# goruck/radar-ml

Measured on AMD Instinct MI355X. Metric: radar frames/s (3D-proj->SVM), higher is better.
Workload: dtype f32 volumes -> u8 codes, i8 MFMA (exact int32 dot), f64 epilogue; 1 GPU; configs[2]: max-projection + RBF-SVM decision_function, 3-class, 2562 SVs, batch 65536 frames/GPU of 64x64x128 f32 resident in HBM; parallelism=single GPU, global_frames=65536

## Files before the change

### include/radarml.h

```cpp
#ifndef RADARML_H
#define RADARML_H

#include <stdint.h>
#include <stddef.h>

#ifdef __cplusplus
extern "C" {
#endif

typedef enum rml_status {
    RML_OK = 0,
    RML_ERR_INVALID = -1,
    RML_ERR_UNSUPPORTED = -2,
    RML_ERR_HIP = -3,
    RML_ERR_NOMEM = -4,
    RML_ERR_STATE = -5
} rml_status;

typedef struct rml_ctx rml_ctx;
typedef struct rml_svm rml_svm;
typedef struct rml_linear rml_linear;

#define RML_MODE_MAX   0
#define RML_MODE_SLICE 1
#define RML_MODE_SUM   2
#define RML_MODE_MAX_NAN 3

#define RML_VOL_F32    0
#define RML_VOL_U8     1

#define RML_MASK_XZ 1u
#define RML_MASK_YZ 2u
#define RML_MASK_XY 4u
#define RML_MASK_ALL 7u

#define RML_KERNEL_RBF    0
#define RML_KERNEL_LINEAR 1

#define RML_PATH_AUTO  0
#define RML_PATH_F32   1
#define RML_PATH_I8    2
#define RML_PATH_F64   3
#define RML_PATH_DIGITS 4

const char* rml_version(void);
const char* rml_last_error(void);

int rml_ctx_create(int device, rml_ctx** out);
int rml_ctx_destroy(rml_ctx* ctx);
int rml_ctx_device(const rml_ctx* ctx);

#define RML_OPT_PROJECT_SHARE_CU 1
#define RML_OPT_WAVEFRAME 2
#define RML_OPT_LINPLANE 3
#define RML_OPT_STAGE_CODES 4
#define RML_OPT_SLICE_WAVE 5
#define RML_OPT_DERIVE_FUSED 6
#define RML_OPT_CODE_RMW 7
#define RML_OPT_GEMM_BIG 8
#define RML_OPT_CHUNK 9
#define RML_OPT_C1_PK 10
#define RML_OPT_SMO_LDS_ROWS 11
#define RML_SMO_LDS_ROWS_MAX 2768
#define RML_OPT_SGD_RESIDENT_D 12
#define RML_SGD_RESIDENT_D_MAX 10240
#define RML_OPT_CONV7 13
#define RML_CONV7_DEFAULT 3
#define RML_OPT_ZOOM_ROWS 14
#define RML_OPT_SPARSE_ROWS 15
int rml_ctx_set_option(rml_ctx* ctx, int option, int value);
int rml_ctx_get_option(const rml_ctx* ctx, int option, int* value);

int rml_ctx_reserve_workspace(rml_ctx* ctx, int64_t bytes);
int64_t rml_ctx_workspace_bytes(const rml_ctx* ctx);

int rml_profile_enable(rml_ctx* ctx, int on);
int rml_profile_read(rml_ctx* ctx, int64_t* launches, double* total_ms, int64_t* frames);
int rml_profile_read_gemm(rml_ctx* ctx, int64_t* launches, double* total_ms, double* ops);

int rml_probe_stream(rml_ctx* ctx, const void* buf, int64_t bytes, int reps, double* gb_per_s, void* stream);

int rml_code_rmw_default(int64_t D, int64_t frame_bytes, int derive, int u8);

int rml_svm_sv_occupancy(rml_ctx* ctx, const rml_svm* m, uint32_t* out, int64_t n_words);
int rml_project_occupancy(rml_ctx* ctx, const void* V, int vdtype, int64_t B, int X, int Y, int Z, int mode, float scale_div,
                          uint32_t mask, uint8_t* feat_q, int64_t ld_q, int32_t* row_isum, int64_t* row_isq, int32_t* row_flags,
                          uint32_t* occ, int occ_words, void* stream);
int64_t rml_ctx_sparse_gemm_launches(const rml_ctx* ctx);

int64_t rml_feature_len(int X, int Y, int Z, uint32_t mask);

int rml_project(rml_ctx* ctx, const void* V, int vdtype, int64_t B, int X, int Y, int Z, int mode,
                const int32_t* ijk, float scale_div, uint32_t mask,
                float* feat, int64_t ld_feat,
                uint8_t* feat_q, int64_t ld_q, int32_t* row_isum, int64_t* row_isq, int32_t* row_flags,
                void* stream);

int rml_project_slices(rml_ctx* ctx, const void* V, int vdtype, int64_t B, int X, int Y, int Z, int T,
                       const int32_t* ijk, float scale_div, uint32_t mask,
                       float* feat, int64_t ld_feat,
                       uint8_t* feat_q, int64_t ld_q, int32_t* row_isum, int64_t* row_isq, int32_t* row_flags,
                       void* stream);

int rml_project_planes(rml_ctx* ctx, const void* V, int vdtype, int64_t B, int X, int Y, int Z, int mode,
                       const int32_t* ijk, float* xz, float* yz, float* xy, void* stream);

int rml_derive_targets(rml_ctx* ctx, const void* V, int vdtype, int64_t B, int X, int Y, int Z,
                       int num_targets, int32_t* ijk, float* profiles, void* stream);

int rml_derive_slice(rml_ctx* ctx, const void* V, int vdtype, int64_t B, int X, int Y, int Z, int num_targets,
                     int32_t* ijk, float* profiles, float scale_div, uint32_t mask,
                     float* feat, int64_t ld_feat,
                     uint8_t* feat_q, int64_t ld_q, int32_t* row_isum, int64_t* row_isq, int32_t* row_flags,
                     void* stream);
int rml_derive_slice_supported(const rml_ctx* ctx, const void* V, int vdtype, int X, int Y, int Z, int num_targets);

int rml_assemble_features(rml_ctx* ctx, const float* xz, const float* yz, const float* xy,
                          int64_t B, int X, int Y, int Z, float scale_div, uint32_t mask,
                          float* feat, int64_t ld_feat, void* stream);

int rml_zoom_features(rml_ctx* ctx, const float* xz, const float* yz, const float* xy,
                      int64_t B, int X, int Y, int Z, const int32_t* out_shape,
                      float scale_div, uint32_t mask, float* feat, int64_t ld_feat, void* stream);

int rml_project_zoom(rml_ctx* ctx, const void* V, int vdtype, int64_t B, int X, int Y, int Z, int mode, const int32_t* ijk, int T,
                     const int32_t* out_shape, float scale_div, uint32_t mask, float* feat, int64_t ld_feat, void* stream);

int rml_quantize_rows(rml_ctx* ctx, const float* feat, int64_t N, int64_t D, int64_t ld_feat,
                      float scale_div, uint8_t* feat_q, int64_t ld_q,
                      int32_t* row_isum, int64_t* row_isq, int32_t* row_flags, void* stream);

int rml_svm_load(rml_ctx* ctx, const double* sv, int64_t M, int64_t D,
                 const double* dual_coef, const double* intercept, const int32_t* n_support,
                 int n_classes, int kernel, double gamma, double code_scale ,
                 const double* calib_a, const double* calib_b, rml_svm** out);
int rml_svm_free(rml_ctx* ctx, rml_svm* m);
int rml_svm_is_exact(const rml_svm* m);
int64_t rml_svm_num_sv(const rml_svm* m);
int64_t rml_svm_dim(const rml_svm* m);

int rml_svm_decision(rml_ctx* ctx, const rml_svm* m, int path,
                     const float* feat, int64_t ld_feat,
                     const uint8_t* feat_q, int64_t ld_q, const int32_t* row_isum, const int64_t* row_isq,
                     const int32_t* row_flags,
                     int64_t N,
                     double* dec_ovo, double* dec_ovr, double* proba,
                     int32_t* label_vote, int32_t* label_calib, void* stream);

int rml_svm_set_platt(rml_ctx* ctx, rml_svm* m, const double* probA, const double* probB);
int rml_svm_pairwise_proba(rml_ctx* ctx, const rml_svm* m, const double* dec_ovo, int64_t N, double* proba, void* stream);

#define RML_AUG_ROTATE 0
#define RML_AUG_ZOOM   1
#define RML_AUG_NOISE  2
int rml_augment(rml_ctx* ctx, int op, const float* src, int64_t B, int H, int W, const double* params, float* dst, void* stream);

#define RML_CHAIN_ROTATE 1
#define RML_CHAIN_ZOOM   2
#define RML_CHAIN_NOISE  4
int rml_augment_chain(rml_ctx* ctx, int stages, const float* src, int64_t in_stride, int64_t B, int H, int W, float sub, float div,
                      float lo, float hi, const double* params, float* dst, void* stream);

int rml_svm_kernel_matrix(rml_ctx* ctx, const rml_svm* m, int path, const float* feat, int64_t ld_feat, int64_t N,
                          double* kmat, int64_t ld_k, void* stream);

#define RML_GRAM_LINEAR 0
#define RML_GRAM_RBF    1
int rml_gram(rml_ctx* ctx, const float* feat, int64_t ld_feat, int64_t N, int64_t D,
             int nk, const int* kinds, const double* gammas,
             double* out, int64_t ld_out, int64_t stride_k, void* stream);

int rml_gram_segments(rml_ctx* ctx, const float* feat, int64_t ld_feat, int64_t N, int nseg, const int64_t* seg_len,
                      double* G, int64_t ld_g, int64_t stride_s, double* nsq, void* stream);
int rml_gram_compose(rml_ctx* ctx, const double* G, int64_t ld_g, int64_t stride_s, const double* nsq, int64_t N, int nseg,
                     int n_out, const int* seg_bits, const int* kinds, const double* gammas,
                     double* out, int64_t ld_out, int64_t stride_k, void* stream);

typedef struct rml_smo_problem {
    int32_t matrix;
    int32_t l;
    int32_t n_pos;
    int32_t shrinking;
    int32_t max_iter;
    int32_t reserved;
    int64_t rows_off;
    int64_t alpha_off;
    double Cp, Cn, eps;
} rml_smo_problem;
typedef struct rml_smo_fit {
    int32_t prob0;
    int32_t n_test;
    int64_t test_off;
} rml_smo_fit;
int rml_smo_solve(rml_ctx* ctx, const double* gram, int64_t N, int64_t ld, int64_t stride_k, int n_mats,
                  const rml_smo_problem* probs, int64_t n_probs, const int32_t* rows, int64_t n_rows_total,
                  double* alpha, int64_t n_alpha_total, double* rho, int32_t* n_iter, int32_t* stopped, void* stream);
int rml_smo_score(rml_ctx* ctx, const double* gram, int64_t N, int64_t ld, int64_t stride_k, int n_mats,
                  const rml_smo_problem* probs, int64_t n_probs, const int32_t* rows, int64_t n_rows_total,
                  const double* alpha, int64_t n_alpha_total, const double* rho, int n_classes,
                  const rml_smo_fit* fits, int64_t n_fits, const int32_t* test_rows, const int32_t* test_y,
                  int64_t n_test_total, double* dec, int32_t* labels, int32_t* correct, void* stream);

#define RML_SGD_L1 1
#define RML_SGD_L2 2
#define RML_SGD_ELASTICNET 3
#define RML_SGD_MAX_ROWS 8192
typedef struct rml_sgd_problem {
    int32_t n;
    int32_t penalty;
    int32_t average;
    int32_t max_iter;
    int32_t n_iter_no_change;
    int32_t shuffle;
    uint32_t seed;
    int32_t warm;
    int64_t rows_off;
    int64_t y_off;
    int64_t out;
    double alpha, l1_ratio, tol, weight_pos, weight_neg, t0;
} rml_sgd_problem;
typedef struct rml_sgd_fit {
    int32_t prob0;
    int32_t n_test;
    int64_t test_off;
} rml_sgd_fit;
int rml_sgd_solve(rml_ctx* ctx, const float* X, int64_t N, int64_t D, int64_t ld, const rml_sgd_problem* probs, int64_t n_probs,
                  const int32_t* rows, int64_t n_rows_total, const int32_t* y, int64_t n_y_total, int64_t n_out, double* coef,
                  double* avg_coef, double* intercept, double* avg_intercept, int32_t* n_iter, double* t, int32_t* status,
                  void* stream);
int rml_sgd_score(rml_ctx* ctx, const float* X, int64_t N, int64_t D, int64_t ld, const rml_sgd_problem* probs, int64_t n_probs,
                  int64_t n_out, const double* coef, const double* avg_coef, const double* intercept, const double* avg_intercept,
                  const double* t, int n_classes, const rml_sgd_fit* fits, int64_t n_fits, const int32_t* test_rows,
                  const int32_t* test_y, int64_t n_test_total, double* dec, int32_t* labels, int32_t* correct, void* stream);
int rml_sgd_shuffle(uint32_t seed, int64_t n, int32_t* perm_inout);

typedef struct rml_sgd_step {
    int64_t off;
    int32_t n;
    int32_t score;
    uint32_t seed[8];
} rml_sgd_step;
// ... 177 lines not shown
```

### radar-ml_amd/_lib.py

```python
import ctypes as C
import os
import threading

HERE = os.path.dirname(os.path.abspath(__file__))
LIB_PATH = os.environ.get("RML_LIB") or os.path.join(HERE, "libradarml_hip.so")


class RadarMLError(RuntimeError):
    pass


_lib = None
_lock = threading.RLock()
_ctx = {}

c_void_p, c_int, c_int64, c_uint32, c_uint64, c_float, c_double = (
    C.c_void_p, C.c_int, C.c_int64, C.c_uint32, C.c_uint64, C.c_float, C.c_double)

SIGNATURES = {
    "rml_version": (C.c_char_p, []),
    "rml_last_error": (C.c_char_p, []),
    "rml_ctx_create": (c_int, [c_int, C.POINTER(c_void_p)]),
    "rml_ctx_destroy": (c_int, [c_void_p]),
    "rml_ctx_device": (c_int, [c_void_p]),
# ... 6 lines not shown
    "rml_profile_read_gemm": (c_int, [c_void_p, C.POINTER(c_int64), C.POINTER(c_double), C.POINTER(c_double)]),
    "rml_feature_len": (c_int64, [c_int, c_int, c_int, c_uint32]),
    "rml_project": (c_int, [c_void_p, c_void_p, c_int, c_int64, c_int, c_int, c_int, c_int, c_void_p, c_float, c_uint32,
                            c_void_p, c_int64, c_void_p, c_int64, c_void_p, c_void_p, c_void_p, c_void_p]),
    "rml_project_slices": (c_int, [c_void_p, c_void_p, c_int, c_int64, c_int, c_int, c_int, c_int, c_void_p, c_float, c_uint32,
                                   c_void_p, c_int64, c_void_p, c_int64, c_void_p, c_void_p, c_void_p, c_void_p]),
    "rml_project_planes": (c_int, [c_void_p, c_void_p, c_int, c_int64, c_int, c_int, c_int, c_int, c_void_p,
                                   c_void_p, c_void_p, c_void_p, c_void_p]),
    "rml_derive_targets": (c_int, [c_void_p, c_void_p, c_int, c_int64, c_int, c_int, c_int, c_int, c_void_p, c_void_p, c_void_p]),
    "rml_derive_slice": (c_int, [c_void_p, c_void_p, c_int, c_int64, c_int, c_int, c_int, c_int, c_void_p, c_void_p, c_float, c_uint32,
                                 c_void_p, c_int64, c_void_p, c_int64, c_void_p, c_void_p, c_void_p, c_void_p]),
    "rml_derive_slice_supported": (c_int, [c_void_p, c_void_p, c_int, c_int, c_int, c_int, c_int]),
    "rml_assemble_features": (c_int, [c_void_p, c_void_p, c_void_p, c_void_p, c_int64, c_int, c_int, c_int, c_float,
                                      c_uint32, c_void_p, c_int64, c_void_p]),
    "rml_zoom_features": (c_int, [c_void_p, c_void_p, c_void_p, c_void_p, c_int64, c_int, c_int, c_int, c_void_p, c_float,
                                  c_uint32, c_void_p, c_int64, c_void_p]),
    "rml_project_zoom": (c_int, [c_void_p, c_void_p, c_int, c_int64, c_int, c_int, c_int, c_int, c_void_p, c_int, c_void_p, c_float,
                                 c_uint32, c_void_p, c_int64, c_void_p]),
    "rml_project_zoom_svm": (c_int, [c_void_p, c_void_p, c_void_p, c_int, c_int64, c_int, c_int, c_int, c_int, c_void_p, c_void_p, c_float,
                                     c_uint32, c_void_p, c_void_p, c_void_p, c_void_p, c_void_p, c_void_p]),
    "rml_quantize_rows": (c_int, [c_void_p, c_void_p, c_int64, c_int64, c_int64, c_float, c_void_p, c_int64,
                                  c_void_p, c_void_p, c_void_p, c_void_p]),
    "rml_svm_load": (c_int, [c_void_p, c_void_p, c_int64, c_int64, c_void_p, c_void_p, c_void_p, c_int, c_int,
                             c_double, c_double, c_void_p, c_void_p, C.POINTER(c_void_p)]),
    "rml_svm_free": (c_int, [c_void_p, c_void_p]),
    "rml_svm_is_exact": (c_int, [c_void_p]),
    "rml_svm_num_sv": (c_int64, [c_void_p]),
    "rml_svm_dim": (c_int64, [c_void_p]),
    "rml_svm_decision": (c_int, [c_void_p, c_void_p, c_int, c_void_p, c_int64, c_void_p, c_int64, c_void_p, c_void_p,
                                 c_void_p, c_int64, c_void_p, c_void_p, c_void_p, c_void_p, c_void_p, c_void_p]),
    "rml_svm_set_platt": (c_int, [c_void_p, c_void_p, c_void_p, c_void_p]),
    "rml_svm_pairwise_proba": (c_int, [c_void_p, c_void_p, c_void_p, c_int64, c_void_p, c_void_p]),
    "rml_svm_kernel_matrix": (c_int, [c_void_p, c_void_p, c_int, c_void_p, c_int64, c_int64, c_void_p, c_int64, c_void_p]),
    "rml_gram": (c_int, [c_void_p, c_void_p, c_int64, c_int64, c_int64, c_int, c_void_p, c_void_p, c_void_p, c_int64, c_int64,
                         c_void_p]),
    "rml_gram_segments": (c_int, [c_void_p, c_void_p, c_int64, c_int64, c_int, c_void_p, c_void_p, c_int64, c_int64, c_void_p, c_void_p]),
    "rml_gram_compose": (c_int, [c_void_p, c_void_p, c_int64, c_int64, c_void_p, c_int64, c_int, c_int, c_void_p, c_void_p, c_void_p,
                                 c_void_p, c_int64, c_int64, c_void_p]),
    "rml_smo_solve": (c_int, [c_void_p, c_void_p, c_int64, c_int64, c_int64, c_int, c_void_p, c_int64, c_void_p, c_int64, c_void_p, c_int64,
                              c_void_p, c_void_p, c_void_p, c_void_p]),
    "rml_smo_score": (c_int, [c_void_p, c_void_p, c_int64, c_int64, c_int64, c_int, c_void_p, c_int64, c_void_p, c_int64, c_void_p, c_int64,
                              c_void_p, c_int, c_void_p, c_int64, c_void_p, c_void_p, c_int64, c_void_p, c_void_p, c_void_p, c_void_p]),
    "rml_sgd_solve": (c_int, [c_void_p, c_void_p, c_int64, c_int64, c_int64, c_void_p, c_int64, c_void_p, c_int64, c_void_p, c_int64, c_int64,
                              c_void_p, c_void_p, c_void_p, c_void_p, c_void_p, c_void_p, c_void_p, c_void_p]),
    "rml_sgd_score": (c_int, [c_void_p, c_void_p, c_int64, c_int64, c_int64, c_void_p, c_int64, c_int64, c_void_p, c_void_p, c_void_p,
                              c_void_p, c_void_p, c_int, c_void_p, c_int64, c_void_p, c_void_p, c_int64, c_void_p, c_void_p, c_void_p,
                              c_void_p]),
    "rml_sgd_shuffle": (c_int, [c_uint32, c_int64, c_void_p]),
    "rml_sgd_online": (c_int, [c_void_p, c_void_p, c_int64, c_int64, c_int64, c_void_p, c_int, c_void_p, c_int64, c_void_p, c_void_p, c_int64,
                               c_void_p, c_void_p, c_int64, c_int64, c_void_p, c_void_p, c_void_p, c_void_p, c_void_p, c_void_p, c_void_p,
                               c_void_p, c_void_p, c_void_p, c_void_p, c_void_p]),
    "rml_libsvm_shuffle": (c_int, [c_uint32, c_int64, c_void_p]),
    "rml_platt_fit": (c_int, [c_void_p, c_void_p, c_int64, C.POINTER(c_double), C.POINTER(c_double), C.POINTER(c_int)]),
    "rml_project_svm": (c_int, [c_void_p, c_void_p, c_void_p, c_int, c_int64, c_int, c_int, c_int, c_int, c_void_p, c_float,
                                c_uint32, c_void_p, c_void_p, c_void_p, c_void_p, c_void_p, c_void_p]),
    "rml_derive_project_svm": (c_int, [c_void_p, c_void_p, c_void_p, c_int, c_int64, c_int, c_int, c_int, c_float, c_uint32, c_void_p,
                                       c_void_p, c_void_p, c_void_p, c_void_p, c_void_p, c_void_p]),
    "rml_linear_load": (c_int, [c_void_p, c_void_p, c_void_p, c_int, c_int64, c_void_p, c_void_p, C.POINTER(c_void_p)]),
    "rml_linear_free": (c_int, [c_void_p, c_void_p]),
    "rml_linear_decision": (c_int, [c_void_p, c_void_p, c_void_p, c_int64, c_int64, c_void_p, c_void_p, c_void_p,
                                    c_void_p, c_void_p]),
    "rml_resize_bicubic": (c_int, [c_void_p, c_void_p, c_int64, c_int64, c_int, c_int, c_int, c_int, c_float, c_float,
                                   c_void_p, c_int, c_void_p]),
    "rml_dnn_preprocess_supported": (c_int, [c_int, c_int, c_int, c_int, c_int]),
    "rml_dnn_preprocess_rows": (c_int, [c_void_p, c_void_p, c_int64, c_void_p, c_int64, c_void_p, c_int64, c_int, c_int, c_int, c_int,
                                        c_int, c_void_p, c_void_p, c_void_p, c_void_p]),
    "rml_dnn_preprocess_volumes": (c_int, [c_void_p, c_void_p, c_int, c_int64, c_int, c_int, c_int, c_int, c_void_p, c_void_p, c_int64,
                                           c_void_p, c_void_p, c_int64, c_int, c_int, c_void_p, c_void_p, c_void_p, c_void_p]),
    "rml_dnn_preprocess_slices": (c_int, [c_void_p, c_void_p, c_int, c_int64, c_int, c_int, c_int, c_void_p, c_int, c_int, c_int,
                                          c_void_p, c_void_p, c_void_p, c_void_p]),
    "rml_dnn_trunk": (c_int, [c_void_p, c_void_p, c_void_p, c_void_p, c_int, c_int64, c_int, c_int, c_void_p, c_void_p, c_void_p,
                              c_void_p, c_void_p, c_void_p]),
    "rml_dnn_trunk_kblock": (c_int, [c_void_p, c_void_p, c_void_p, c_void_p, c_int, c_int64, c_int, c_int, c_void_p, c_void_p, c_void_p,
                                     c_void_p, c_void_p, c_void_p]),
    "rml_dnn_trunk_kblock_supported": (c_int, [c_int, c_int]),
    "rml_dnn_trunk_x3_supported": (c_int, [c_int, c_int]),
    "rml_dnn_trunk_x3": (c_int, [c_void_p, c_void_p, c_void_p, c_void_p, c_int64, c_int, c_int, c_void_p, c_void_p, c_void_p,
                                 c_void_p, c_int, c_void_p, c_void_p]),
    "rml_dnn_exact_features_scratch_bytes": (c_int64, [c_int, c_int64, c_int, c_int, c_int, c_int, c_int, c_int]),
    "rml_dnn_exact_features": (c_int, [c_void_p, c_void_p, c_int, c_void_p, c_int64, c_int, c_int, c_int, c_int, c_int, c_int, c_void_p,
                                       c_void_p, c_void_p, c_void_p, c_int, c_void_p, c_int64, c_void_p, c_void_p]),
    "rml_dnn_top2_gap": (c_int, [c_void_p, c_void_p, c_int64, c_int64, c_int, c_void_p, c_void_p]),
    "rml_dnn_guard_apply": (c_int, [c_void_p, c_void_p, c_int64, c_int, c_void_p, c_int64, c_void_p, c_float, c_void_p, c_void_p, c_void_p,
                                    c_void_p]),
    "rml_dnn_dense_workspace_bytes": (c_int64, [c_void_p, c_int64, c_int64]),
    "rml_dnn_dense_tail": (c_int, [c_void_p, c_void_p, c_int64, c_int, c_int64, c_int64, c_void_p, c_void_p, c_void_p, c_void_p, c_void_p,
                                   c_void_p, c_int, c_void_p, c_int64, c_void_p, c_void_p]),
    "rml_dnn_dense_tail_f32_workspace_bytes": (c_int64, [c_int64, c_int64]),
    "rml_dnn_dense_tail_f32": (c_int, [c_void_p, c_void_p, c_int64, c_int64, c_int64, c_void_p, c_void_p, c_void_p, c_void_p, c_void_p,
                                       c_void_p, c_int, c_void_p, c_int64, c_void_p, c_void_p]),
    "rml_sgan_trunk_supported": (c_int, [c_int, c_int]),
    "rml_sgan_trunk_workspace_bytes": (c_int64, [c_int64, c_int, c_int]),
    "rml_sgan_trunk": (c_int, [c_void_p, c_void_p, c_void_p, c_void_p, c_int, c_int64, c_int, c_int, c_void_p, c_void_p, c_void_p,
                               c_void_p, c_void_p, c_void_p, c_float, c_void_p, c_void_p, c_int64, c_void_p]),
    "rml_dense_tail_lrelu": (c_int, [c_void_p, c_void_p, c_int64, c_int64, c_int64, c_void_p, c_void_p, c_void_p, c_void_p, c_void_p,
                                     c_void_p, c_int, c_float, c_void_p, c_int64, c_void_p, c_void_p]),
    "rml_sgan_trunk_x3_supported": (c_int, [c_int, c_int]),
    "rml_sgan_trunk_x3_workspace_bytes": (c_int64, [c_int64, c_int, c_int]),
    "rml_sgan_trunk_x3": (c_int, [c_void_p, c_void_p, c_void_p, c_void_p, c_int64, c_int, c_int, c_void_p, c_void_p, c_void_p, c_void_p,
                                  c_void_p, c_void_p, c_float, c_int, c_void_p, c_void_p, c_int64, c_void_p]),
    "rml_dense_tail_lrelu_f32": (c_int, [c_void_p, c_void_p, c_int64, c_int64, c_int64, c_void_p, c_void_p, c_void_p, c_void_p, c_void_p,
                                         c_void_p, c_int, c_float, c_void_p, c_int64, c_void_p, c_void_p]),
    "rml_dnn_train_supported":(c_int, [c_int, c_int, c_int]),
    "rml_dnn_train_workspace_bytes": (c_int64, [c_int, c_int, c_int, c_int]),
    "rml_dnn_train_step": (c_int, [c_void_p, c_void_p, c_void_p, c_void_p, c_void_p, c_void_p, c_int, c_int64, c_int, c_int, c_void_p, c_int,
                                   c_void_p, c_void_p, c_int, c_uint64, c_int64, c_float, c_int, c_void_p, c_int64, c_void_p, c_void_p,
                                   c_void_p, c_void_p]),
    "rml_dnn_dropout_mask": (c_int, [c_uint64, c_int64, c_int, c_int, c_int, c_float, c_void_p]),
    "rml_bn_workspace_floats": (c_int64, [c_void_p, c_int]),
    "rml_bn_lrelu_pad_forward": (c_int, [c_void_p, c_void_p, c_int, c_int64, c_int, c_int, c_int, c_int, c_int, c_void_p, c_void_p,
                                         c_float, c_float, c_float, c_void_p, c_void_p, c_void_p, c_void_p, c_void_p, c_void_p, c_void_p]),
    "rml_bn_lrelu_pad_backward": (c_int, [c_void_p, c_void_p, c_void_p, c_int, c_int64, c_int, c_int, c_int, c_int, c_int, c_void_p,
                                          c_void_p, c_void_p, c_void_p, c_float, c_void_p, c_void_p, c_void_p, c_void_p, c_void_p]),
    "rml_conv1_bn_lrelu_pad_forward": (c_int, [c_void_p, c_void_p, c_void_p, c_int, c_int64, c_int, c_int, c_int, c_int, c_int, c_void_p,
                                               c_void_p, c_float, c_float, c_float, c_void_p, c_void_p, c_void_p, c_void_p, c_void_p,
                                               c_void_p, c_void_p, c_void_p]),
    "rml_conv1_bn_lrelu_pad_backward": (c_int, [c_void_p, c_void_p, c_void_p, c_void_p, c_int, c_int64, c_int, c_int, c_int, c_int, c_int,
                                                c_void_p, c_void_p, c_void_p, c_void_p, c_void_p, c_float, c_void_p, c_void_p, c_void_p,
                                                c_void_p, c_void_p]),
    "rml_conv7_tanh_supported": (c_int, [c_int, c_int, c_int]),
    "rml_conv7_workspace_floats": (c_int64, [c_void_p, c_int64, c_int, c_int, c_int]),
    "rml_conv7_tanh_forward": (c_int, [c_void_p, c_void_p, c_int, c_int64, c_int, c_int, c_int, c_void_p, c_void_p, c_void_p, c_void_p]),
    "rml_conv7_tanh_backward": (c_int, [c_void_p, c_void_p, c_void_p, c_void_p, c_int, c_int64, c_int, c_int, c_int, c_void_p, c_void_p,
                                        c_void_p, c_void_p, c_void_p, c_void_p]),
    "rml_gen_up_supported": (c_int, [c_int, c_int, c_int]),
    "rml_gen_up_forward": (c_int, [c_void_p, c_void_p, c_int, c_int64, c_int, c_int, c_int, c_void_p, c_void_p, c_void_p, c_void_p]),
    "rml_sgan_generate_workspace_bytes": (c_int64, [c_int64, c_int, c_int, c_int]),
    "rml_sgan_generate": (c_int, [c_void_p, c_void_p, c_int64, c_int, c_int, c_int, c_int, c_int, c_void_p, c_void_p, c_void_p, c_void_p,
                                  c_void_p, c_void_p, c_void_p, c_void_p, c_void_p, c_void_p, c_int64, c_void_p]),
    "rml_conv3s2_supported": (c_int, [c_int, c_int, c_int, c_int]),
    "rml_conv3s2_workspace_bytes": (c_int64, [c_void_p, c_int64, c_int, c_int, c_int, c_int, c_int]),
    "rml_conv3s2_forward": (c_int, [c_void_p, c_void_p, c_void_p, c_int, c_int64, c_int, c_int, c_int, c_int, c_void_p, c_void_p, c_int64,
                                    c_void_p]),
    "rml_conv3s2_dgrad": (c_int, [c_void_p, c_void_p, c_void_p, c_int, c_int64, c_int, c_int, c_int, c_int, c_void_p, c_void_p, c_int64,
                                  c_void_p]),
    "rml_conv3s2_wgrad": (c_int, [c_void_p, c_void_p, c_void_p, c_int, c_int64, c_int, c_int, c_int, c_int, c_void_p, c_void_p, c_int64,
                                  c_void_p]),
    "rml_convt4s2_supported": (c_int, [c_int, c_int, c_int, c_int]),
    "rml_convt4s2_workspace_bytes": (c_int64, [c_void_p, c_int64, c_int, c_int, c_int, c_int, c_int]),
    "rml_convt4s2_forward": (c_int, [c_void_p, c_void_p, c_void_p, c_int, c_int64, c_int, c_int, c_int, c_int, c_void_p, c_void_p, c_int64,
                                     c_void_p]),
    "rml_convt4s2_dgrad": (c_int, [c_void_p, c_void_p, c_void_p, c_int, c_int64, c_int, c_int, c_int, c_int, c_void_p, c_void_p, c_int64,
                                   c_void_p]),
    "rml_convt4s2_wgrad": (c_int, [c_void_p, c_void_p, c_void_p, c_int, c_int64, c_int, c_int, c_int, c_int, c_void_p, c_void_p, c_int64,
                                   c_void_p]),
    "rml_adam_entry_bytes": (c_int, []),
    "rml_adam_step": (c_int, [c_void_p, c_void_p, c_int, c_int64, c_float, c_float, c_float, c_float, c_void_p, c_void_p, c_void_p,
                              c_void_p, c_int, c_float, c_float, c_int, c_void_p]),
    "rml_augment": (c_int, [c_void_p, c_int, c_void_p, c_int64, c_int, c_int, c_void_p, c_void_p, c_void_p]),
    "rml_augment_chain": (c_int, [c_void_p, c_int, c_void_p, c_int64, c_int64, c_int, c_int, c_float, c_float, c_float, c_float, c_void_p,
                                  c_void_p, c_void_p]),
    "rml_code_rmw_default": (c_int, [c_int64, c_int64, c_int, c_int]),
    "rml_ctx_sparse_gemm_launches": (c_int64, [c_void_p]),
    "rml_svm_sv_occupancy": (c_int, [c_void_p, c_void_p, c_void_p, c_int64]),
    "rml_project_occupancy": (c_int, [c_void_p, c_void_p, c_int, c_int64, c_int, c_int, c_int, c_int, c_float, c_uint32, c_void_p, c_int64,
                                      c_void_p, c_void_p, c_void_p, c_void_p, c_int, c_void_p]),
    "rml_probe_stream": (c_int, [c_void_p, c_void_p, c_int64, c_int, c_void_p, c_void_p]),
    "rml_synth_volumes": (c_int, [c_void_p, c_uint64, c_int64, c_int64, c_int, c_int, c_int, c_int, c_void_p, c_void_p,
                                  c_void_p]),
}

MODE_MAX, MODE_SLICE, MODE_SUM, MODE_MAX_NAN = 0, 1, 2, 3
OPT_PROJECT_SHARE_CU, OPT_WAVEFRAME, OPT_LINPLANE, OPT_STAGE_CODES, OPT_SLICE_WAVE, OPT_DERIVE_FUSED, OPT_CODE_RMW, OPT_GEMM_BIG, OPT_CHUNK, OPT_C1_PK, OPT_SMO_LDS_ROWS, OPT_SGD_RESIDENT_D, OPT_CONV7, OPT_ZOOM_ROWS, OPT_SPARSE_ROWS = range(1, 16)
OPTIONS = {"project_share_cu": OPT_PROJECT_SHARE_CU, "waveframe": OPT_WAVEFRAME, "linplane": OPT_LINPLANE, "stage_codes": OPT_STAGE_CODES,
           "slice_wave": OPT_SLICE_WAVE, "derive_fused": OPT_DERIVE_FUSED, "code_rmw": OPT_CODE_RMW, "gemm_big": OPT_GEMM_BIG,
           "chunk": OPT_CHUNK, "c1_pk": OPT_C1_PK}
SOLVER_OPTIONS = {"smo_lds_rows": OPT_SMO_LDS_ROWS, "sgd_resident_d": OPT_SGD_RESIDENT_D}
NN_OPTIONS = {"conv7": OPT_CONV7}
ZOOM_OPTIONS = {"zoom_rows": OPT_ZOOM_ROWS}
SVM_OPTIONS = {"sparse_rows": OPT_SPARSE_ROWS}
SMO_LDS_ROWS_MAX = 2768
SGD_RESIDENT_D_MAX = 10240
SGD_MAX_ROWS = 8192
SGD_L1, SGD_L2, SGD_ELASTICNET = 1, 2, 3
DNN_TRAIN, DNN_EVAL = 0, 1
DNN_TRAIN_MAX_BATCH = 64
ENV_OPTIONS = {"RML_WAVE_SHARE": "project_share_cu", "RML_WAVEFRAME": "waveframe", "RML_LINPLANE": "linplane", "RML_STAGE_CODES": "stage_codes",
               "RML_SLICE_WAVE": "slice_wave", "RML_DERIVE_FUSED": "derive_fused", "RML_CODE_RMW": "code_rmw", "RML_GEMM_BIG": "gemm_big",
               "RML_CHUNK": "chunk", "RML_C1_PK": "c1_pk", "RML_SMO_LDS_ROWS": "smo_lds_rows", "RML_SGD_RESIDENT_D": "sgd_resident_d",
               "RML_CONV7": "conv7", "RML_SPARSE_ROWS": "sparse_rows"}
AUG_ROTATE, AUG_ZOOM, AUG_NOISE = 0, 1, 2
CHAIN_ROTATE, CHAIN_ZOOM, CHAIN_NOISE = 1, 2, 4
VOL_F32, VOL_U8 = 0, 1
MODES = {"max": MODE_MAX, "slice": MODE_SLICE, "sum": MODE_SUM, "max_nan": MODE_MAX_NAN}
KERNEL_RBF, KERNEL_LINEAR = 0, 1
PATH_AUTO, PATH_F32, PATH_I8, PATH_F64, PATH_DIGITS = 0, 1, 2, 3, 4
GRAM_LINEAR, GRAM_RBF = 0, 1
PATHS = {"auto": PATH_AUTO, "f32": PATH_F32, "i8": PATH_I8, "f64": PATH_F64, "digits": PATH_DIGITS}


def option_id(name):
    name = name.lower()
    for table in (OPTIONS, SOLVER_OPTIONS, ZOOM_OPTIONS, SVM_OPTIONS):
        if name in table:
            return table[name]
    return NN_OPTIONS[name]


def load():
    global _lib
    with _lock:
        if _lib is not None:
            return _lib
        if not os.path.exists(LIB_PATH):
            raise RadarMLError(
                "libradarml_hip.so is not built (%s missing): run `python radar-ml_amd/build.py`; "
                "there is no CPU fallback for the HIP path" % LIB_PATH)
        try:
            import torch
        except Exception:
            pass
        try:
            lib = C.CDLL(LIB_PATH, mode=C.RTLD_GLOBAL)
        except OSError as e:
            raise RadarMLError("cannot load %s: %s" % (LIB_PATH, e))
        for name, (res, args) in SIGNATURES.items():
            try:
                fn = getattr(lib, name)
            except AttributeError:
                raise RadarMLError("libradarml_hip.so does not export %s" % name)
            fn.restype = res
            fn.argtypes = args
        _lib = lib
        return lib


def check(rc, what=""):
    if rc != 0:
        msg = load().rml_last_error()
        raise RadarMLError("%s failed (status %d): %s" % (what or "radarml call", rc, msg.decode() if msg else ""))


def context(device=None):
    import torch
    if not torch.cuda.is_available():
        raise RadarMLError("no HIP device is visible: the radar-ml HIP path needs an MI355X (no CPU fallback)")
    if device is None:
        device = torch.cuda.current_device()
    elif isinstance(device, torch.device):
        device = device.index if device.index is not None else torch.cuda.current_device()
    index = int(device)
    lib = load()
    with _lock:
        h = _ctx.get(device)
    if h is None:
        new = c_void_p()
        check(lib.rml_ctx_create(index, C.byref(new)), "rml_ctx_create")
        for var, name in ENV_OPTIONS.items():
            val = os.environ.get(var)
            if val not in (None, ""):
                check(lib.rml_ctx_set_option(new, option_id(name), int(val)), "rml_ctx_set_option(%s from $%s)" % (name, var))
        with _lock:
            h = _ctx.setdefault(device, new)
        if h is not new:
            lib.rml_ctx_destroy(new)
    return h


def set_option(name, value, device=None):
    lib, ctx = load(), context(device)
    old = C.c_int()
    check(lib.rml_ctx_get_option(ctx, option_id(name), C.byref(old)), "rml_ctx_get_option")
    check(lib.rml_ctx_set_option(ctx, option_id(name), int(value)), "rml_ctx_set_option")
    return old.value


def get_option(name, device=None):
    v = C.c_int()
    check(load().rml_ctx_get_option(context(device), option_id(name), C.byref(v)), "rml_ctx_get_option")
    return v.value


class options:

    def __init__(self, device=None, **kv):
        self.device, self.kv, self.old = device, kv, {}

    def __enter__(self):
        for k, v in self.kv.items():
            self.old[k] = set_option(k, v, self.device)
        return self

    def __exit__(self, *exc):
        for k, v in self.old.items():
            set_option(k, v, self.device)
        return False


def device_of(device=None):
    import torch
    if device is None:
        return torch.device("cuda", torch.cuda.current_device())
    d = torch.device(device) if not isinstance(device, int) else torch.device("cuda", device)
    if d.type != "cuda":
        raise RadarMLError("the radar-ml HIP path runs on a HIP device, not %r" % (device,))
    return d if d.index is not None else torch.device("cuda", torch.cuda.current_device())


def ptr(t):
    if t is None:
        return None
    return c_void_p(t.data_ptr())


def stream_ptr(device=None):
    import torch
    return c_void_p(torch.cuda.current_stream(device).cuda_stream)
```

### radar-ml_amd/csrc/context.hip

```cpp
#include "rml_internal.h"
#include <stdarg.h>
#include <stdio.h>
#include <stdlib.h>
#include <new>

namespace {
thread_local char g_err[512] = "";
}

void rml_set_error(const char* fmt, ...) {
    va_list ap;
    va_start(ap, fmt);
    vsnprintf(g_err, sizeof(g_err), fmt, ap);
    va_end(ap);
}

int rml_hip_fail(hipError_t e, const char* what, const char* file, int line) {
    rml_set_error("HIP error %d (%s) in %s at %s:%d", (int)e, hipGetErrorString(e), what, file, line);
    return RML_ERR_HIP;
}

static void ws_release_retired(rml_ctx* ctx, bool all) {
    size_t k = 0;
    for (size_t i = 0; i < ctx->ws_retired.size(); ++i) {
// ... 114 lines not shown
    RML_REQUIRE(device >= 0 && device < n, RML_ERR_INVALID, "rml_ctx_create: device %d out of range (%d devices)", device, n);
    struct restore_device {
        int prev = -1;
        restore_device() { if (hipGetDevice(&prev) != hipSuccess) { (void)hipGetLastError(); prev = -1; } }
        ~restore_device() { if (prev >= 0) (void)hipSetDevice(prev); }
    } restore;
    RML_HIP(hipSetDevice(device));
    hipDeviceProp_t prop;
    RML_HIP(hipGetDeviceProperties(&prop, device));
    rml_ctx* c = new (std::nothrow) rml_ctx();
    RML_REQUIRE(c != nullptr, RML_ERR_NOMEM, "rml_ctx_create: out of host memory");
    c->device = device;
    c->num_cu = prop.multiProcessorCount;
    hipError_t e = hipStreamCreateWithFlags(&c->aux_stream, hipStreamNonBlocking);
    if (e == hipSuccess) e = hipEventCreateWithFlags(&c->ev_fork, hipEventDisableTiming);
    if (e == hipSuccess) e = hipEventCreateWithFlags(&c->ev_join, hipEventDisableTiming);
    if (e == hipSuccess) e = hipEventCreateWithFlags(&c->ev_last, hipEventDisableTiming);
    for (int i = 0; i < 2 && e == hipSuccess; ++i) {
        e = hipEventCreateWithFlags(&c->ev_proj[i], hipEventDisableTiming);
        if (e == hipSuccess) e = hipEventCreateWithFlags(&c->ev_done[i], hipEventDisableTiming);
    }
    if (e == hipSuccess) e = hipMalloc(reinterpret_cast<void**>(&c->bg_line), 128);
    if (e == hipSuccess) e = hipMemset(c->bg_line, 0x80, 128);
    if (e != hipSuccess) {
        if (c->bg_line) (void)hipFree(c->bg_line);
        delete c;
        return rml_hip_fail(e, "stream/event creation", __FILE__, __LINE__);
    }
    *out = c;
    return RML_OK;
}

extern "C" int rml_ctx_destroy(rml_ctx* ctx) {
    if (!ctx) return RML_OK;
    int prev = -1;
    if (hipGetDevice(&prev) != hipSuccess) { (void)hipGetLastError(); prev = -1; }
    (void)hipSetDevice(ctx->device);
    (void)hipDeviceSynchronize();
    ws_release_retired(ctx, true);
    if (ctx->ws) (void)hipFree(ctx->ws);
    if (ctx->ev_fork) (void)hipEventDestroy(ctx->ev_fork);
    if (ctx->ev_join) (void)hipEventDestroy(ctx->ev_join);
    if (ctx->ev_last) (void)hipEventDestroy(ctx->ev_last);
    if (ctx->ev_stage) (void)hipEventDestroy(ctx->ev_stage);
    if (ctx->stage) (void)hipHostFree(ctx->stage);
    for (int i = 0; i < 2; ++i) {
        if (ctx->ev_proj[i]) (void)hipEventDestroy(ctx->ev_proj[i]);
        if (ctx->ev_done[i]) (void)hipEventDestroy(ctx->ev_done[i]);
    }
    for (hipEvent_t e : ctx->prof_ev) (void)hipEventDestroy(e);
    for (hipEvent_t e : ctx->prof_ev_g) (void)hipEventDestroy(e);
    for (const rml_resize_tab& t : ctx->resize_tabs) (void)hipFree(const_cast<double*>(t.kk));
    for (const rml_pre_tab& t : ctx->pre_tabs) (void)hipFree(t.dev);
    if (ctx->aux_stream) (void)hipStreamDestroy(ctx->aux_stream);
    if (ctx->bg_line) (void)hipFree(ctx->bg_line);
    delete ctx;
    if (prev >= 0) (void)hipSetDevice(prev);
    return RML_OK;
}

static bool stream_is_capturing(hipStream_t st) {
    hipStreamCaptureStatus cs = hipStreamCaptureStatusNone;
    if (hipStreamIsCapturing(st, &cs) != hipSuccess) (void)hipGetLastError();
    return cs != hipStreamCaptureStatusNone;
}

void rml_prof_mark(rml_ctx* ctx, hipStream_t st) {
    if (!ctx->profiling || stream_is_capturing(st)) return;
    if (ctx->prof_used == ctx->prof_ev.size()) {
        hipEvent_t e;
        if (hipEventCreate(&e) != hipSuccess) { (void)hipGetLastError(); return; }
        ctx->prof_ev.push_back(e);
    }
    (void)hipEventRecord(ctx->prof_ev[ctx->prof_used++], st);
}

void rml_prof_mark_gemm(rml_ctx* ctx, hipStream_t st) {
    if (!ctx->profiling || stream_is_capturing(st)) return;
    if (ctx->prof_used_g == ctx->prof_ev_g.size()) {
        hipEvent_t e;
        if (hipEventCreate(&e) != hipSuccess) { (void)hipGetLastError(); return; }
        ctx->prof_ev_g.push_back(e);
    }
    (void)hipEventRecord(ctx->prof_ev_g[ctx->prof_used_g++], st);
}

extern "C" int rml_profile_read_gemm(rml_ctx* ctx, int64_t* launches, double* total_ms, double* ops) {
    RML_REQUIRE(ctx != nullptr, RML_ERR_INVALID, "rml_profile_read_gemm: ctx is NULL");
    std::lock_guard<std::recursive_mutex> lk(ctx->mu);
    RML_HIP(hipSetDevice(ctx->device));
    double tot = 0.0;
    int64_t n = 0;
    for (size_t i = 0; i + 1 < ctx->prof_used_g; i += 2) {
        RML_HIP(hipEventSynchronize(ctx->prof_ev_g[i + 1]));
        float ms = 0.0f;
        RML_HIP(hipEventElapsedTime(&ms, ctx->prof_ev_g[i], ctx->prof_ev_g[i + 1]));
        tot += ms;
        ++n;
    }
    if (launches) *launches = n;
    if (total_ms) *total_ms = tot;
    if (ops) *ops = ctx->prof_ops_g;
    ctx->prof_used_g = 0;
    ctx->prof_ops_g = 0.0;
    return RML_OK;
}

extern "C" int rml_profile_enable(rml_ctx* ctx, int on) {
    RML_REQUIRE(ctx != nullptr, RML_ERR_INVALID, "rml_profile_enable: ctx is NULL");
    std::lock_guard<std::recursive_mutex> lk(ctx->mu);
    ctx->profiling = on != 0;
    ctx->prof_used = 0;
    ctx->prof_frames = 0;
    ctx->prof_used_g = 0;
    ctx->prof_ops_g = 0.0;
    return RML_OK;
}

extern "C" int rml_profile_read(rml_ctx* ctx, int64_t* launches, double* total_ms, int64_t* frames) {
    RML_REQUIRE(ctx != nullptr, RML_ERR_INVALID, "rml_profile_read: ctx is NULL");
    std::lock_guard<std::recursive_mutex> lk(ctx->mu);
    RML_HIP(hipSetDevice(ctx->device));
    double tot = 0.0;
    int64_t n = 0;
    for (size_t i = 0; i + 1 < ctx->prof_used; i += 2) {
        RML_HIP(hipEventSynchronize(ctx->prof_ev[i + 1]));
        float ms = 0.0f;
        RML_HIP(hipEventElapsedTime(&ms, ctx->prof_ev[i], ctx->prof_ev[i + 1]));
        tot += ms;
        ++n;
    }
    if (launches) *launches = n;
    if (total_ms) *total_ms = tot;
    if (frames) *frames = ctx->prof_frames;
    ctx->prof_used = 0;
    ctx->prof_frames = 0;
    return RML_OK;
}

extern "C" int rml_ctx_device(const rml_ctx* ctx) { return ctx ? ctx->device : RML_ERR_INVALID; }

static int* opt_slot(rml_opts& o, int option) {
    switch (option) {
        case RML_OPT_PROJECT_SHARE_CU: return &o.project_share_cu;
        case RML_OPT_WAVEFRAME: return &o.waveframe;
        case RML_OPT_LINPLANE: return &o.linplane;
        case RML_OPT_STAGE_CODES: return &o.stage_codes;
        case RML_OPT_SLICE_WAVE: return &o.slice_wave;
        case RML_OPT_DERIVE_FUSED: return &o.derive_fused;
        case RML_OPT_CODE_RMW: return &o.code_rmw;
        case RML_OPT_GEMM_BIG: return &o.gemm_big;
        case RML_OPT_C1_PK: return &o.c1_pk;
        case RML_OPT_SPARSE_ROWS: return &o.sparse_rows;
        default: return nullptr;
    }
}

extern "C" int rml_ctx_set_option(rml_ctx* ctx, int option, int value) {
    RML_REQUIRE(ctx != nullptr, RML_ERR_INVALID, "rml_ctx_set_option: ctx is NULL");
    std::lock_guard<std::recursive_mutex> lk(ctx->mu);
    if (option == RML_OPT_SMO_LDS_ROWS) {
        RML_REQUIRE(value >= 0 && value <= RML_SMO_LDS_ROWS_MAX, RML_ERR_INVALID, "rml_ctx_set_option: RML_OPT_SMO_LDS_ROWS is 0..%d rows",
                    RML_SMO_LDS_ROWS_MAX);
        ctx->opt.smo_lds_rows = value;
        return RML_OK;
    }
    if (option == RML_OPT_SGD_RESIDENT_D) {
        RML_REQUIRE(value >= 0 && value <= RML_SGD_RESIDENT_D_MAX, RML_ERR_INVALID, "rml_ctx_set_option: RML_OPT_SGD_RESIDENT_D is 0..%d "
                    "features", RML_SGD_RESIDENT_D_MAX);
        ctx->opt.sgd_resident_d = value;
        return RML_OK;
    }
    if (option == RML_OPT_CONV7) {
        RML_REQUIRE(value >= 0 && value <= 3, RML_ERR_INVALID, "rml_ctx_set_option: RML_OPT_CONV7 is 0..3 (bit 0 forward, bit 1 backward)");
        ctx->opt.conv7 = value;
        return RML_OK;
    }
    if (option == RML_OPT_ZOOM_ROWS) {
        RML_REQUIRE(value >= 0 && value <= 2, RML_ERR_INVALID, "rml_ctx_set_option: RML_OPT_ZOOM_ROWS is 0 (by LDS size), 1 (whole row) or 2 (plane by plane)");
        ctx->opt.zoom_rows = value;
        return RML_OK;
    }
    if (option == RML_OPT_CHUNK) {
        RML_REQUIRE(value == 0 || value >= 128, RML_ERR_INVALID, "rml_ctx_set_option: RML_OPT_CHUNK is 0 (automatic) or >= 128 rows");
        ctx->opt.chunk = value;
        return RML_OK;
    }
    int* slot = opt_slot(ctx->opt, option);
    RML_REQUIRE(slot != nullptr, RML_ERR_INVALID, "rml_ctx_set_option: unknown option %d", option);
    switch (option) {
        case RML_OPT_WAVEFRAME: RML_REQUIRE(value >= 0 && value <= 3, RML_ERR_INVALID, "rml_ctx_set_option: RML_OPT_WAVEFRAME is 0..3"); *slot = value; break;
        case RML_OPT_CODE_RMW: case RML_OPT_GEMM_BIG: case RML_OPT_SPARSE_ROWS: *slot = value < 0 ? -1 : (value ? 1 : 0); break;
        default: *slot = value ? 1 : 0;
    }
    return RML_OK;
}

extern "C" int rml_ctx_get_option(const rml_ctx* ctx, int option, int* value) {
    RML_REQUIRE(ctx != nullptr && value != nullptr, RML_ERR_INVALID, "rml_ctx_get_option: NULL argument");
    rml_ctx* c = const_cast<rml_ctx*>(ctx);
    std::lock_guard<std::recursive_mutex> lk(c->mu);
    if (option == RML_OPT_CHUNK) { *value = (int)c->opt.chunk; return RML_OK; }
    if (option == RML_OPT_SMO_LDS_ROWS) { *value = c->opt.smo_lds_rows; return RML_OK; }
    if (option == RML_OPT_SGD_RESIDENT_D) { *value = c->opt.sgd_resident_d; return RML_OK; }
    if (option == RML_OPT_CONV7) { *value = c->opt.conv7; return RML_OK; }
    if (option == RML_OPT_ZOOM_ROWS) { *value = c->opt.zoom_rows; return RML_OK; }
    const int* slot = opt_slot(c->opt, option);
    RML_REQUIRE(slot != nullptr, RML_ERR_INVALID, "rml_ctx_get_option: unknown option %d", option);
    *value = *slot;
    return RML_OK;
}

namespace {
typedef float probe_v4 __attribute__((ext_vector_type(4)));
__global__ __launch_bounds__(256) void k_probe_stream(const probe_v4* __restrict__ src, int64_t n16, float* sink) {
    constexpr int PF = 16;
    const int64_t piece = (int64_t)256 * PF;
    probe_v4 m = {-INFINITY, -INFINITY, -INFINITY, -INFINITY};
    for (int64_t base = (int64_t)blockIdx.x * piece; base < n16; base += (int64_t)gridDim.x * piece) {
        probe_v4 v[PF];
#pragma unroll
        for (int u = 0; u < PF; ++u) {
            int64_t q = base + (int64_t)u * 256 + threadIdx.x;
            q = q < n16 ? q : n16 - 1;
            v[u] = __builtin_nontemporal_load(src + q);
        }
#pragma unroll
        for (int u = 0; u < PF; ++u) {
            m.x = fmaxf(m.x, v[u].x); m.y = fmaxf(m.y, v[u].y); m.z = fmaxf(m.z, v[u].z); m.w = fmaxf(m.w, v[u].w);
        }
    }
    const float r = fmaxf(fmaxf(m.x, m.y), fmaxf(m.z, m.w));
    if (r == 12345.678f) sink[blockIdx.x] = r;
}
}

extern "C" int rml_probe_stream(rml_ctx* ctx, const void* buf, int64_t bytes, int reps, double* gb_per_s, void* stream) {
    RML_REQUIRE(ctx && buf && gb_per_s, RML_ERR_INVALID, "rml_probe_stream: NULL argument");
    RML_REQUIRE(bytes >= (1 << 20) && reps >= 1 && (reinterpret_cast<uintptr_t>(buf) & 15) == 0, RML_ERR_INVALID,
                "rml_probe_stream: needs a 16-byte aligned buffer of at least 1 MiB and reps >= 1");
    RML_HIP(hipSetDevice(ctx->device));
    hipStream_t st = static_cast<hipStream_t>(stream);
    rml_ctx_guard guard(ctx, st);
    void* sink = nullptr;
    int rc = rml_ws_reserve(ctx, (size_t)4 * 2 * ctx->num_cu, &sink, st);
    if (rc) return rc;
    const int64_t n16 = bytes / 16;
    hipEvent_t e0 = nullptr, e1 = nullptr;
    RML_HIP(hipEventCreate(&e0));
    {
        const hipError_t ec = hipEventCreate(&e1);
        if (ec != hipSuccess) { (void)hipEventDestroy(e0); RML_HIP(ec); }
    }
    const dim3 grid((unsigned)(2 * ctx->num_cu)), block(256);
    for (int i = 0; i < 2; ++i)
        hipLaunchKernelGGL(k_probe_stream, grid, block, 0, st, static_cast<const probe_v4*>(buf), n16, static_cast<float*>(sink));
    hipError_t e = hipGetLastError();
    if (e == hipSuccess) e = hipEventRecord(e0, st);
    for (int i = 0; i < reps && e == hipSuccess; ++i)
        hipLaunchKernelGGL(k_probe_stream, grid, block, 0, st, static_cast<const probe_v4*>(buf), n16, static_cast<float*>(sink));
    if (e == hipSuccess) e = hipGetLastError();
    if (e == hipSuccess) e = hipEventRecord(e1, st);
    if (e == hipSuccess) e = hipEventSynchronize(e1);
    float ms = 0.0f;
    if (e == hipSuccess) e = hipEventElapsedTime(&ms, e0, e1);
    (void)hipEventDestroy(e0);
    (void)hipEventDestroy(e1);
    RML_HIP(e);
    RML_HIP(hipGetLastError());
    *gb_per_s = ms > 0.0f ? (double)reps * (double)(n16 * 16) / ((double)ms * 1e-3) / 1e9 : 0.0;
    return RML_OK;
}

extern "C" int rml_code_rmw_default(int64_t D, int64_t frame_bytes, int derive, int u8) {
    return rml_code_rmw(D, frame_bytes, derive != 0, u8 != 0);
}
```

### radar-ml_amd/csrc/project.hip

```cpp
#include "project_shared.h"

namespace {

using namespace rmlproj;

template <typename VT, int MODE, int LPR, int NM, bool FULL, bool PRED>
__global__ __launch_bounds__(kThreads) void k_project_fast(ProjParams a) {
    extern __shared__ __align__(16) float lds[];
    if constexpr (PRED) { if (*a.o.skip_if_set) return; }
    const int X = a.X, Y = a.Y, Z = a.Z, ZQ = a.ZQ;
    float* xz_lds = lds;
    float* xy_lds = lds + (size_t)X * Z;
    int64_t* red = reinterpret_cast<int64_t*>(xy_lds + (((size_t)X * Y + 3) & ~(size_t)3));

    constexpr int RPW = 64 / LPR;
    constexpr int NSLOT = 4 * RPW;
    const int tid = threadIdx.x, lane = tid & 63, wave = tid >> 6;
    const int slot = wave * RPW + lane / LPR;
    const int kq = lane % LPR;
    const bool act = FULL || (kq < ZQ);
    const int64_t b = blockIdx.x;
    typedef typename Quad<VT>::T QT;
    const QT* __restrict__ Vb = reinterpret_cast<const QT*>(static_cast<const VT*>(a.V) + b * (int64_t)X * Y * Z);

// ... 125 lines not shown
#pragma unroll
        for (int m = 0; m < NM; ++m) {
            yz[m] = op4<MODE>(yz[m], cur[m]);
            p = op4<MODE>(p, cur[m]);
            float r = Op<MODE>::f(Op<MODE>::f(cur[m].x, cur[m].y), Op<MODE>::f(cur[m].z, cur[m].w));
#pragma unroll
            for (int s = 0; s < 6; ++s) {
                const float o = __shfl_down(r, 1 << s);
                r = ((same >> s) & 1u) ? Op<MODE>::f(r, o) : r;
            }
            if (head && rv[m]) Op<MODE>::lds_atomic(xy_lds + i * Y + slot + R * m, r);
        }
        float* dst = xz_lds + i * Z + 4 * kq;
        Op<MODE>::lds_atomic(dst + 0, p.x);
        Op<MODE>::lds_atomic(dst + 1, p.y);
        Op<MODE>::lds_atomic(dst + 2, p.z);
        Op<MODE>::lds_atomic(dst + 3, p.w);
    }

    Emitter em(a, b);
    em.rmw = false;
#pragma unroll
    for (int m = 0; m < NM; ++m) {
        const int j = slot + R * m;
        if (rv[m]) em.put4(1, (int64_t)j * Z + 4 * kq, yz[m]);
    }
    __syncthreads();
    auto val4 = [](const float4& q) { return make_float4(Op<MODE>::lds_value(q.x), Op<MODE>::lds_value(q.y), Op<MODE>::lds_value(q.z), Op<MODE>::lds_value(q.w)); };
    const int nxz4 = (X * Z) >> 2;
    for (int idx = tid; idx < nxz4; idx += T)
        em.put4(0, (int64_t)idx * 4, val4(*reinterpret_cast<const float4*>(xz_lds + idx * 4)));
    const int nxy = X * Y;
    const int nxy4 = nxy >> 2;
    for (int idx = tid; idx < nxy4; idx += T)
        em.put4(2, (int64_t)idx * 4, val4(*reinterpret_cast<const float4*>(xy_lds + idx * 4)));
    for (int idx = nxy4 * 4 + tid; idx < nxy; idx += T) em.put1(2, idx, Op<MODE>::lds_value(xy_lds[idx]));
    em.finish(red);
}

template <typename VT, int MODE, int NY, int G, bool PRED>
__global__ __launch_bounds__(256, (NY + 2 * G) * 4 + 40 > 256 ? 1 : 2) void k_project_wave(ProjParams a) {
    if constexpr (PRED) { if (*a.o.skip_if_set) return; }
    constexpr int NG = (NY + G - 1) / G;
    static_assert(NG == 1 || NG % 2 == 0, "the two row buffers must alternate statically");
    constexpr int U = NG == 1 ? 2 : NG;
    const int X = a.X, Yr = a.Y, Zr = a.Z, ZQr = a.ZQ;
    const int RPL = a.rpl;
    const int Y = Yr / RPL, Z = Zr * RPL, ZQ = ZQr * RPL;
    const int lane = threadIdx.x & 63;
    const int wave = __builtin_amdgcn_readfirstlane(threadIdx.x >> 6);
    const int64_t stride = (int64_t)gridDim.x * 4;
    int64_t cf = (int64_t)blockIdx.x * 4 + wave;
    if (cf >= a.B) return;
    typedef typename Quad<VT>::T QT;
    const QT* __restrict__ Vall = reinterpret_cast<const QT*>(a.V);
    const int64_t fq = (int64_t)X * Y * ZQ;
    const int pq = Y * ZQ;
    const bool act = lane < ZQ;
    const uint32_t kqc = (uint32_t)(act ? lane : ZQ - 1);
    const float id = Op<MODE>::ident();
    const float4 id4 = make_float4(id, id, id, id);

    int64_t lf = cf;
    int li = 0;
    const QT* __restrict__ lV = Vall + lf * fq;
    auto next_plane = [&]() {
        ++li;
        lV += pq;
        if (li == X) {
            li = 0;
            const int64_t nf = lf + stride;
            lf = nf < a.B ? nf : lf;
            lV = Vall + lf * fq;
        }
    };
    float4 buf[2][G];
    constexpr int kXyStride = 68;
    __shared__ __align__(16) float xy_stage[4][NY * kXyStride];
    float* xyl = xy_stage[wave];
    const uint32_t rowb = (uint32_t)ZQ * sizeof(QT);
    auto fetch = [&](float4 (&dst)[G], auto gc) {
        constexpr int g = decltype(gc)::value;
        const char* __restrict__ base = reinterpret_cast<const char*>(lV);
        uint32_t rowb_t = rowb;
        asm volatile("" : "+s"(rowb_t));
        static_for<G>([&](auto rc) {
            constexpr int r = decltype(rc)::value;
            constexpr int j = g * G + r;
            if constexpr (j < NY) {
                const uint32_t ro = (uint32_t)(NY == 31 || j < Y ? j : Y - 1) * rowb_t;
                dst[r] = ld_stream(reinterpret_cast<const QT*>(base + ro) + kqc);
            }
        });
    };
    constexpr int PPT = NG == 1 ? 2 : 1;
    Emitter em(a, cf);
    em.rmw = false;
    extern __shared__ __align__(16) unsigned char wave_dyn[];
    if (a.stage_bytes) em.set_stage(wave_dyn + wave * a.stage_bytes, (X * Zr + 15) & ~15);
    fetch(buf[0], std::integral_constant<int, 0>{});
    for (; cf < a.B; cf += stride) {
        em.reset(cf);
        float4 yz[NY];
        static_for<NY>([&](auto jc) { yz[decltype(jc)::value] = id4; });
        float4 xz = id4;
        for (int ci = 0; ci < X; ci += PPT) {
            static_for<U>([&](auto uc) {
                constexpr int u = decltype(uc)::value;
                constexpr int g = NG == 1 ? 0 : u;
                constexpr int gn = NG == 1 ? 0 : (u + 1) % NG;
                if constexpr (gn == 0) next_plane();
                fetch(buf[(u + 1) & 1], std::integral_constant<int, gn>{});
                __builtin_amdgcn_sched_barrier(0);
                static_for<G>([&](auto rc) {
                    constexpr int r = decltype(rc)::value;
                    constexpr int j = g * G + r;
                    if constexpr (j < NY) {
                        float4 v = buf[u & 1][r];
                        if constexpr (MODE == RML_MODE_SUM) v = (act && j < Y) ? v : id4;
                        yz[j] = op4_raw<MODE>(yz[j], v);
                        asm volatile("" : "+v"(yz[j].x), "+v"(yz[j].y), "+v"(yz[j].z), "+v"(yz[j].w));
                        xz = op4_raw<MODE>(xz, v);
                        xyl[j * kXyStride + lane] = op_raw<MODE>(op_raw<MODE>(v.x, v.y), op_raw<MODE>(v.z, v.w));
                    }
                });
                asm volatile("" : "+v"(xz.x), "+v"(xz.y), "+v"(xz.z), "+v"(xz.w));
                __builtin_amdgcn_sched_barrier(0);
                if constexpr (g == NG - 1) {
                    const int i = ci + (NG == 1 ? u : 0);
                    int lane_e = lane;
                    asm volatile("" : "+v"(lane_e));
                    for (int off = ZQr; off < ZQ; off <<= 1) {
                        float4 o;
                        o.x = __shfl_xor(xz.x, off); o.y = __shfl_xor(xz.y, off); o.z = __shfl_xor(xz.z, off); o.w = __shfl_xor(xz.w, off);
                        xz = op4<MODE>(xz, o);
                    }
                    if (lane_e < ZQr) em.put4(0, (int64_t)i * Zr + 4 * lane_e, xz);
                    for (int jr = lane_e; jr < Yr; jr += 64) {
                        const float* rowp = xyl + (jr / RPL) * kXyStride + (jr % RPL) * ZQr;
                        float m = id;
                        for (int q = 0; q < ZQr; q += 4) {
                            const float4 t = *reinterpret_cast<const float4*>(rowp + q);
                            m = Op<MODE>::f(m, Op<MODE>::f(Op<MODE>::f(t.x, t.y), Op<MODE>::f(t.z, t.w)));
                        }
                        em.put1(2, (int64_t)i * Yr + jr, m);
                    }
                    xz = id4;
                }
            });
        }
        int lane_f = lane, Y_f = Y;
        asm volatile("" : "+v"(lane_f), "+s"(Y_f));
        const bool act_f = lane_f < ZQ;
        static_for<NY>([&](auto jc) {
            constexpr int j = decltype(jc)::value;
            if (j < Y_f && act_f) em.put4(1, (int64_t)j * Z + 4 * lane_f, yz[j]);
        });
        em.flush_wave(lane_f);
        em.finish_wave(lane_f);
    }
}

template <typename VT, int MODE, int NY, int G>
void launch_wave(const ProjParams& pp_in, int num_cu, hipStream_t st) {
    ProjParams pp = pp_in;
    constexpr int per_cu_max = (NY + 2 * G) * 4 + 40 > 256 ? 1 : 2;
    const size_t mine = (size_t)4 * NY * 68 * sizeof(float);
    pp.stage_bytes = code_stage_bytes(pp, sizeof(VT));
    if (mine + (size_t)4 * pp.stage_bytes > 160 * 1024) pp.stage_bytes = 0;
    if (!pp.stage_bytes) pp.o.occ = nullptr;
    else if (pp.o.occ && pp.occ_done) *pp.occ_done = 1;
    const size_t stage = (size_t)4 * pp.stage_bytes;
    int per_cu = pp.o.share_cu ? 1 : per_cu_max;
    if (per_cu * (mine + stage) > 160 * 1024) per_cu = 1;
    const int64_t want = (pp.B + 3) / 4;
    const int64_t cap = (int64_t)num_cu * per_cu;
    dim3 grid((unsigned)(want < cap ? want : cap)), block(kThreads);
    size_t pad = stage;
    if (pp.o.share_cu && per_cu == 1 && !pp.o.no_pad && mine + stage < 81 * 1024) pad = 81 * 1024 - mine;
    if (pp.o.skip_if_set) {
        RML_MAX_DYN_LDS(160 * 1024 - (int)mine, &k_project_wave<VT, MODE, NY, G, true>);
        hipLaunchKernelGGL((k_project_wave<VT, MODE, NY, G, true>), grid, block, pad, st, pp);
    } else {
        RML_MAX_DYN_LDS(160 * 1024 - (int)mine, &k_project_wave<VT, MODE, NY, G, false>);
        hipLaunchKernelGGL((k_project_wave<VT, MODE, NY, G, false>), grid, block, pad, st, pp);
    }
}

int wave_kernel_rpl(int ZQ, int Y) {
    if (ZQ > 32 && ZQ <= 64) return Y <= 32 ? 1 : 0;
    if (ZQ == 32 || ZQ == 16) {
        const int rpl = 64 / ZQ;
        return (Y % rpl == 0 && Y / rpl <= 32) ? rpl : 0;
    }
    return 0;
}

bool wave_kernel_wanted(int ZQ, int Y, bool share_cu, int64_t B, int num_cu, int knob) {
    if (B < 2 * (int64_t)num_cu) return false;
    const int rpl = wave_kernel_rpl(ZQ, Y);
    if (knob == 0 || rpl == 0) return false;
    return rpl == 1 || share_cu || knob == 3;
}

template <typename VT, int MODE>
bool try_launch_wave(const ProjParams& pp_in, int num_cu, hipStream_t st) {
    const int knob = pp_in.k_waveframe;
    if (!wave_kernel_wanted(pp_in.ZQ, pp_in.Y, pp_in.o.share_cu != 0, pp_in.B, num_cu, knob)) return false;
    ProjParams pp = pp_in;
    pp.rpl = wave_kernel_rpl(pp.ZQ, pp.Y);
    const int Y = pp.Y / wave_kernel_rpl(pp.ZQ, pp.Y);
    const bool quarter = knob == 2 || (pp.X & 1) || pp.o.share_cu;
#define RML_WAVE_CASE(NYV)                                                                     \
    { if (quarter) launch_wave<VT, MODE, NYV, (NYV + 3) / 4>(pp, num_cu, st);                 \
      else launch_wave<VT, MODE, NYV, NYV>(pp, num_cu, st); return true; }
    if (Y <= 8) RML_WAVE_CASE(8)
    if (Y <= 16) RML_WAVE_CASE(16)
    if (Y <= 24) RML_WAVE_CASE(24)
    if (Y == 31) RML_WAVE_CASE(31)
    RML_WAVE_CASE(32)
#undef RML_WAVE_CASE
}

template <typename VT, int MODE>
__global__ __launch_bounds__(kThreads) void k_project_generic(ProjParams a) {
    __shared__ int64_t red[64];
    if (a.o.skip_if_set && *a.o.skip_if_set) return;
    const int X = a.X, Y = a.Y, Z = a.Z;
    const int64_t b = blockIdx.x;
    const VT* __restrict__ Vb = static_cast<const VT*>(a.V) + b * (int64_t)X * Y * Z;
    const int tid = threadIdx.x, lane = tid & 63, wave = tid >> 6;
    Emitter em(a, b);
    const float id = Op<MODE>::ident();
    for (int idx = tid; idx < X * Z; idx += kThreads) {
        int i = idx / Z, k = idx - i * Z;
        float r = id;
        for (int j = 0; j < Y; ++j) r = Op<MODE>::f(r, (float)Vb[((int64_t)i * Y + j) * Z + k]);
        em.put1(0, idx, r);
    }
    for (int idx = tid; idx < Y * Z; idx += kThreads) {
        float r = id;
        for (int i = 0; i < X; ++i) r = Op<MODE>::f(r, (float)Vb[(int64_t)i * Y * Z + idx]);
        em.put1(1, idx, r);
    }
    for (int row = wave; row < X * Y; row += kThreads / 64) {
        float r = id;
        for (int k = lane; k < Z; k += 64) r = Op<MODE>::f(r, (float)Vb[(int64_t)row * Z + k]);
        r = row_reduce<MODE, 64>(r);
        if (lane == 0) em.put1(2, row, r);
    }
    em.finish(red);
}

template <typename VT>
__global__ __launch_bounds__(kThreads) void k_project_slice(ProjParams a) {
    __shared__ int64_t red[64];
    if (a.o.skip_if_set && *a.o.skip_if_set) return;
    const int X = a.X, Y = a.Y, Z = a.Z;
    const int64_t b = blockIdx.x;
    const VT* __restrict__ Vb = static_cast<const VT*>(a.V) + (b / a.tpf) * (int64_t)X * Y * Z;
    int i = a.ijk[b * 3 + 0], j = a.ijk[b * 3 + 1], k = a.ijk[b * 3 + 2];
    i = i < 0 ? i + X : i; j = j < 0 ? j + Y : j; k = k < 0 ? k + Z : k;
    i = min(max(i, 0), X - 1); j = min(max(j, 0), Y - 1); k = min(max(k, 0), Z - 1);
    const int tid = threadIdx.x;
    Emitter em(a, b);
    for (int idx = tid; idx < X * Z; idx += kThreads) {
        int ii = idx / Z, kk = idx - ii * Z;
        em.put1(0, idx, (float)Vb[((int64_t)ii * Y + j) * Z + kk]);
    }
    for (int idx = tid; idx < Y * Z; idx += kThreads)
        em.put1(1, idx, (float)Vb[(int64_t)i * Y * Z + idx]);
    for (int idx = tid; idx < X * Y; idx += kThreads)
        em.put1(2, idx, (float)Vb[(int64_t)idx * Z + k]);
    em.finish(red);
}

__global__ __launch_bounds__(kThreads) void k_assemble(const float* xz, const float* yz, const float* xy, ProjParams a) {
    __shared__ int64_t red[64];
    const int X = a.X, Y = a.Y, Z = a.Z;
    const int64_t b = blockIdx.x;
    const int tid = threadIdx.x;
    Emitter em(a, b);
    if (xz) for (int idx = tid; idx < X * Z; idx += kThreads) em.put1(0, idx, xz[b * (int64_t)X * Z + idx]);
    if (yz) for (int idx = tid; idx < Y * Z; idx += kThreads) em.put1(1, idx, yz[b * (int64_t)Y * Z + idx]);
    if (xy) for (int idx = tid; idx < X * Y; idx += kThreads) em.put1(2, idx, xy[b * (int64_t)X * Y + idx]);
    em.finish(red);
}

__global__ __launch_bounds__(kThreads) void k_quantize_rows(const float* feat, int64_t D, int64_t ld, float scale_div, ProjParams a) {
    __shared__ int64_t red[64];
    const int64_t b = blockIdx.x;
    Emitter em(a, b);
    const bool scaled = scale_div > 1.0f;
    for (int64_t idx = threadIdx.x; idx < D; idx += kThreads) {
        float v = feat[b * ld + idx];
        float c = rintf(scaled ? v * scale_div : v);
        float back = scaled ? __fdiv_rn(c, scale_div) : c;
        bool good = (back == v) && c >= 0.0f && c <= 255.0f;
        em.put_code1(0, idx, good ? (int)c : 0, good);
    }
    em.finish(red);
}

__global__ __launch_bounds__(64) void k_profiles_topk(const float* xzs, const float* yzs, int X, int Y, int Z,
                                                      int ntgt, int32_t* ijk, float* profiles) {
    extern __shared__ float prof[];
    const int64_t b = blockIdx.x;
    const float* xz = xzs + b * (int64_t)X * Z;
    const float* yz = yzs + b * (int64_t)Y * Z;
// ... 16 lines not shown
                if (best < 0 || v >= bv) { bv = v; best = q; }
            }
            ijk[(b * ntgt + (ntgt - 1 - t)) * 3 + lane] = best;
            s[best] = -INFINITY;
        }
    }
}

int next_pow2(int v) { int p = 1; while (p < v) p <<= 1; return p; }

template <typename VT, int MODE, int LPR, int NM, bool FULL>
void launch_fast_pred(const ProjParams& pp, size_t lds_bytes, hipStream_t st) {
    dim3 grid((unsigned)pp.B), block(kThreads);
    if (pp.o.skip_if_set) {
        RML_MAX_DYN_LDS(160 * 1024, &k_project_fast<VT, MODE, LPR, NM, FULL, true>);
        hipLaunchKernelGGL((k_project_fast<VT, MODE, LPR, NM, FULL, true>), grid, block, lds_bytes, st, pp);
    } else {
        RML_MAX_DYN_LDS(160 * 1024, &k_project_fast<VT, MODE, LPR, NM, FULL, false>);
        hipLaunchKernelGGL((k_project_fast<VT, MODE, LPR, NM, FULL, false>), grid, block, lds_bytes, st, pp);
    }
}

template <typename VT, int MODE, int LPR>
int launch_fast_nm(const ProjParams& pp, int nm, size_t lds_bytes, hipStream_t st) {
    constexpr int NSLOT = 4 * (64 / LPR);
    if (nm > (LPR == 64 ? 16 : 8)) return 1;
    const int NMr = nm <= 4 ? 4 : (nm <= 8 ? 8 : 16);
    const bool full = (pp.ZQ == LPR) && (pp.Y == NMr * NSLOT);
    if (NMr == 4) { if (full) launch_fast_pred<VT, MODE, LPR, 4, true>(pp, lds_bytes, st); else launch_fast_pred<VT, MODE, LPR, 4, false>(pp, lds_bytes, st); }
    else if (NMr == 8) { if (full) launch_fast_pred<VT, MODE, LPR, 8, true>(pp, lds_bytes, st); else launch_fast_pred<VT, MODE, LPR, 8, false>(pp, lds_bytes, st); }
    else if constexpr (LPR == 64) { if (full) launch_fast_pred<VT, MODE, LPR, 16, true>(pp, lds_bytes, st); else launch_fast_pred<VT, MODE, LPR, 16, false>(pp, lds_bytes, st); }
    return 0;
}

template <typename VT, int MODE, int NM>
void launch_rowgroup(const ProjParams& pp, int R, size_t lds_bytes, hipStream_t st) {
    dim3 grid((unsigned)pp.B), block((unsigned)(R * pp.ZQ));
    if (pp.o.skip_if_set) {
        RML_MAX_DYN_LDS(160 * 1024, &k_project_rowgroup<VT, MODE, NM, true>);
        hipLaunchKernelGGL((k_project_rowgroup<VT, MODE, NM, true>), grid, block, lds_bytes, st, pp, R);
    } else {
        RML_MAX_DYN_LDS(160 * 1024, &k_project_rowgroup<VT, MODE, NM, false>);
        hipLaunchKernelGGL((k_project_rowgroup<VT, MODE, NM, false>), grid, block, lds_bytes, st, pp, R);
    }
}

int gcd_int(int a, int b) { while (b) { int t = a % b; a = b; b = t; } return a; }

template <typename VT, int MODE>
int launch_mode(const ProjParams& pp, int num_cu, hipStream_t st, bool* used_fast) {
    const int X = pp.X, Y = pp.Y, Z = pp.Z;
    *used_fast = false;
    if constexpr (sizeof(VT) == 1 && MODE == RML_MODE_MAX) {
        if (try_launch_u8_max(pp, st)) { *used_fast = true; return 0; }
    }
    bool fast_ok = (Z % 4 == 0) && (Z / 4 <= 64) && ((reinterpret_cast<uintptr_t>(pp.V) & (4 * sizeof(VT) - 1)) == 0);
    size_t lds_bytes = ((size_t)X * Z + (((size_t)X * Y + 3) & ~(size_t)3)) * 4 + 64 * 8;
    if (lds_bytes > 150 * 1024) fast_ok = false;
    if constexpr (sizeof(VT) == 4) {
        if (fast_ok && wave_kernel_wanted(pp.ZQ, pp.Y, pp.o.share_cu != 0, pp.B, num_cu, pp.k_waveframe) && try_launch_lin(pp, MODE, num_cu, st)) {
            *used_fast = true;
            return 0;
        }
    }
    if (fast_ok && try_launch_wave<VT, MODE>(pp, num_cu, st)) { *used_fast = true; return 0; }
    if (fast_ok && (Z / 4) != next_pow2(Z / 4) && (Z / 4) >= 8) {
        const int zq = Z / 4;
        int R = 64 / gcd_int(zq, 64);
        while (R * zq < 512 && 2 * R * zq <= 1024 && 2 * R <= Y) R *= 2;
        if (R * zq <= 1024) {
            const int nm = (Y + R - 1) / R;
            if (nm <= 2) { launch_rowgroup<VT, MODE, 2>(pp, R, lds_bytes, st); *used_fast = true; return 0; }
            if (nm <= 4) { launch_rowgroup<VT, MODE, 4>(pp, R, lds_bytes, st); *used_fast = true; return 0; }
            if (nm <= 8) { launch_rowgroup<VT, MODE, 8>(pp, R, lds_bytes, st); *used_fast = true; return 0; }
        }
    }
    if (fast_ok) {
        int zq = Z / 4;
        int lpr = next_pow2(zq); if (lpr < 16) lpr = 16;
        int nslot = 4 * (64 / lpr);
        int nm = (Y + nslot - 1) / nslot;
        int rc = 1;
        if (lpr == 16) rc = launch_fast_nm<VT, MODE, 16>(pp, nm, lds_bytes, st);
        else if (lpr == 32) rc = launch_fast_nm<VT, MODE, 32>(pp, nm, lds_bytes, st);
        else rc = launch_fast_nm<VT, MODE, 64>(pp, nm, lds_bytes, st);
        if (rc == 0) { *used_fast = true; return 0; }
    }
    hipLaunchKernelGGL((k_project_generic<VT, MODE>), dim3((unsigned)pp.B), dim3(kThreads), 0, st, pp);
    return 0;
}

void fill_params(ProjParams& pp, const rml_ctx* ctx, const void* V, int64_t B, int X, int Y, int Z, const int32_t* ijk, const ProjOut& o) {
    pp.V = V; pp.B = B; pp.X = X; pp.Y = Y; pp.Z = Z; pp.ZQ = Z / 4; pp.ijk = ijk; pp.tpf = 1; pp.rpl = 1; pp.o = o;
    pp.ntgt = 1; pp.ijk_out = nullptr; pp.profiles = nullptr; pp.wave_lds = 0; pp.stage_bytes = 0; pp.occ_done = nullptr;
    const rml_opts def;
    const rml_opts& op = ctx ? ctx->opt : def;
    pp.k_waveframe = op.waveframe; pp.k_linplane = op.linplane; pp.k_stage_codes = op.stage_codes; pp.k_slice_wave = op.slice_wave;
    pp.k_derive_fused = op.derive_fused;
    if (op.project_share_cu) pp.o.share_cu = 1;
    for (int pl = 0; pl < 3; ++pl)
        pp.vec_ok[pl] = o.p[pl] && ((reinterpret_cast<uintptr_t>(o.p[pl]) & 15) == 0) && (o.stride[pl] % 4 == 0);
}

}

namespace {
template <typename VT>
int launch_project_t(const ProjParams& pp, int mode, int num_cu, hipStream_t st) {
    bool fast = false;
    if (mode == RML_MODE_MAX) launch_mode<VT, RML_MODE_MAX>(pp, num_cu, st, &fast);
    else if (mode == RML_MODE_SUM) launch_mode<VT, RML_MODE_SUM>(pp, num_cu, st, &fast);
    else if (mode == RML_MODE_SLICE) {
        RML_REQUIRE(pp.ijk != nullptr, RML_ERR_INVALID, "rml_project: mode SLICE needs ijk");
        if (!try_launch_slice(pp, (int)sizeof(VT), st))
            hipLaunchKernelGGL(k_project_slice<VT>, dim3((unsigned)pp.B), dim3(kThreads), 0, st, pp);
    } else {
        RML_REQUIRE(false, RML_ERR_INVALID, "rml_project: unknown mode %d", mode);
    }
    return RML_OK;
}
}

namespace {
__global__ __launch_bounds__(256) void k_fill_u32(uint32_t* p, int64_t n, uint32_t v) {
    const int64_t i = (int64_t)blockIdx.x * 256 + threadIdx.x;
    if (i < n) p[i] = v;
}
}

bool rml_project_uses_wave_kernel(const rml_ctx* ctx, int vdtype, int mode, int X, int Y, int Z, bool share_cu, int64_t B) {
    (void)X;
    const int num_cu = ctx ? ctx->num_cu : 256, knob = ctx ? ctx->opt.waveframe : 1;
    if (mode != RML_MODE_MAX && mode != RML_MODE_SUM) return false;
    if (vdtype == RML_VOL_U8 && mode == RML_MODE_MAX && Z % 16 == 0) return false;
    return Z % 4 == 0 && wave_kernel_wanted(Z / 4, Y, share_cu, B, num_cu, knob);
}

int rml_launch_project(rml_ctx* ctx, const void* V, int vdtype, int64_t B, int X, int Y, int Z, int mode,
                       const int32_t* ijk, const ProjOut& o, hipStream_t st, int targets_per_frame) {
    if (B == 0) return RML_OK;
    RML_REQUIRE(vdtype == RML_VOL_F32 || vdtype == RML_VOL_U8, RML_ERR_INVALID, "rml_project: unknown volume dtype %d", vdtype);
    if (mode == RML_MODE_MAX_NAN) mode = RML_MODE_MAX;
    RML_REQUIRE(targets_per_frame == 1 || mode == RML_MODE_SLICE, RML_ERR_INVALID, "rml_project: several targets per frame only in mode SLICE");
    RML_REQUIRE(!o.occ || (o.qrow && (int64_t)o.occ_words * 32 >= (o.qD + 127) / 128), RML_ERR_INVALID,
                "rml_project: occupancy words need code rows and a bit per 128-byte line");
    ProjParams pp;
    fill_params(pp, ctx, V, B, X, Y, Z, ijk, o);
    pp.tpf = targets_per_frame;
    int occ_done = 0;
    pp.occ_done = &occ_done;
    const int num_cu = !ctx ? 256 : ctx->num_cu;
    const int rc = vdtype == RML_VOL_U8 ? launch_project_t<uint8_t>(pp, mode, num_cu, st) : launch_project_t<float>(pp, mode, num_cu, st);
    if (rc) return rc;
    if (o.occ && !occ_done) {
        const int64_t n = B * o.occ_words;
        hipLaunchKernelGGL(k_fill_u32, dim3((unsigned)((n + 255) / 256)), dim3(256), 0, st, o.occ, n, 0xFFFFFFFFu);
    }
    RML_HIP(hipGetLastError());
    return RML_OK;
}

namespace {
constexpr int kFinalThreads = 1024;
__global__ __launch_bounds__(kFinalThreads) void k_project_finalize(ProjParams a, const float* __restrict__ scr, int S, int Xs, int64_t ldv) {
    __shared__ int64_t red[64];
    const int X = a.X, Y = a.Y, Z = a.Z;
    const int64_t b = blockIdx.x;
    const float* __restrict__ fr = scr + b * S * ldv;
    const int64_t oyz = (int64_t)Xs * Z, oxy = oyz + (int64_t)Y * Z;
    Emitter em(a, b);
    em.rmw = false;
    const int tid = threadIdx.x;
    for (int idx = tid; idx < (X * Z) >> 2; idx += kFinalThreads) {
        const int i = (idx * 4) / Z, k = idx * 4 - i * Z, s = i / Xs;
        em.put4(0, (int64_t)idx * 4, *reinterpret_cast<const float4*>(fr + s * ldv + (int64_t)(i - s * Xs) * Z + k));
    }
    for (int idx = tid; idx < (Y * Z) >> 2; idx += kFinalThreads) {
        const float* __restrict__ q0 = fr + oyz + (int64_t)idx * 4;
        float4 v = *reinterpret_cast<const float4*>(q0);
        for (int s0 = 1; s0 < S; s0 += 8) {
            float4 t[8];
#pragma unroll
            for (int u = 0; u < 8; ++u) t[u] = *reinterpret_cast<const float4*>(q0 + (int64_t)(s0 + u < S ? s0 + u : 0) * ldv);
#pragma unroll
            for (int u = 0; u < 8; ++u) v = op4<RML_MODE_MAX>(v, t[u]);
        }
        em.put4(1, (int64_t)idx * 4, v);
    }
    const int nxy = X * Y;
    if ((Y & 3) == 0) {
        for (int idx = tid; idx < nxy >> 2; idx += kFinalThreads) {
            const int i = (idx * 4) / Y, j = idx * 4 - i * Y, s = i / Xs;
            em.put4(2, (int64_t)idx * 4, *reinterpret_cast<const float4*>(fr + s * ldv + oxy + (int64_t)(i - s * Xs) * Y + j));
        }
    } else {
        for (int idx = tid; idx < nxy >> 2; idx += kFinalThreads) {
            float v[4];
#pragma unroll
            for (int e = 0; e < 4; ++e) {
                const int t = idx * 4 + e, i = t / Y, j = t - i * Y, s = i / Xs;
                v[e] = fr[s * ldv + oxy + (int64_t)(i - s * Xs) * Y + j];
            }
            em.put4(2, (int64_t)idx * 4, make_float4(v[0], v[1], v[2], v[3]));
        }
        for (int t = (nxy & ~3) + tid; t < nxy; t += kFinalThreads) {
            const int i = t / Y, j = t - i * Y, s = i / Xs;
            em.put1(2, t, fr[s * ldv + oxy + (int64_t)(i - s * Xs) * Y + j]);
        }
    }
    em.finish(red);
}
}

int rml_project_split_pieces(int X, int Y, int Z) {
    if (Z % 4 != 0 || X < 2 || Y < 1) return 0;
    int best = 0;
    for (int s = 2; s <= X && s <= 16; ++s)
        if (X % s == 0) best = s;
    return best;
}
int64_t rml_project_split_ld(int X, int Y, int Z, int S) {
    const int Xs = X / S;
    return (((int64_t)Xs * Z + (int64_t)Y * Z + (int64_t)Xs * Y) + 3) & ~(int64_t)3;
}
size_t rml_project_split_scratch_bytes(int64_t B, int X, int Y, int Z, int S) {
    return (size_t)B * S * rml_project_split_ld(X, Y, Z, S) * sizeof(float);
}

int rml_launch_project_split(rml_ctx* ctx, const void* V, int vdtype, int64_t B, int X, int Y, int Z, const ProjOut& o, float* scratch, int S,
                             hipStream_t st) {
    RML_REQUIRE(S >= 2 && X % S == 0 && Z % 4 == 0 && scratch, RML_ERR_INVALID, "rml_launch_project_split: bad split");
    const int Xs = X / S;
    const int64_t ldv = rml_project_split_ld(X, Y, Z, S);
    ProjOut os{};
    os.p[0] = scratch; os.p[1] = scratch + (int64_t)Xs * Z; os.p[2] = os.p[1] + (int64_t)Y * Z;
    os.stride[0] = os.stride[1] = os.stride[2] = ldv;
    os.sel = RML_MASK_ALL;
    int rc = rml_launch_project(ctx, V, vdtype, B * S, Xs, Y, Z, RML_MODE_MAX, nullptr, os, st);
    if (rc) return rc;
    ProjParams pp;
    fill_params(pp, ctx, V, B, X, Y, Z, nullptr, o);
    hipLaunchKernelGGL(k_project_finalize, dim3((unsigned)B), dim3(kFinalThreads), 0, st, pp, (const float*)scratch, S, Xs, ldv);
    RML_HIP(hipGetLastError());
    return RML_OK;
}

int rml_launch_derive_slice(rml_ctx* ctx, const void* V, int vdtype, int64_t B, int X, int Y, int Z, int num_targets,
                            int32_t* ijk_out, float* profiles, const ProjOut& o, hipStream_t st) {
    if (B == 0) return RML_OK;
    ProjParams pp;
    fill_params(pp, ctx, V, B, X, Y, Z, nullptr, o);
    pp.ntgt = num_targets; pp.ijk_out = ijk_out; pp.profiles = profiles;
    const int num_cu = !ctx ? 256 : ctx->num_cu;
    if (!try_launch_derive_slice(pp, vdtype == RML_VOL_U8 ? 1 : 4, num_cu, st)) return RML_ERR_UNSUPPORTED;
    RML_HIP(hipGetLastError());
    return RML_OK;
}

static int plane_len(int pl, int X, int Y, int Z) { return pl == 0 ? X * Z : (pl == 1 ? Y * Z : X * Y); }

extern "C" int64_t rml_feature_len(int X, int Y, int Z, uint32_t mask) {
    int64_t d = 0;
    for (int pl = 0; pl < 3; ++pl) if (mask & (1u << pl)) d += plane_len(pl, X, Y, Z);
    return d;
}

static int project_rows(rml_ctx* ctx, const void* V, int vdtype, int64_t B, int X, int Y, int Z, int mode, int tpf,
                        const int32_t* ijk, float scale_div, uint32_t mask,
                        float* feat, int64_t ld_feat, uint8_t* feat_q, int64_t ld_q,
                        int32_t* row_isum, int64_t* row_isq, int32_t* row_flags, void* stream);

extern "C" int rml_project(rml_ctx* ctx, const void* V, int vdtype, int64_t B, int X, int Y, int Z, int mode,
                           const int32_t* ijk, float scale_div, uint32_t mask,
                           float* feat, int64_t ld_feat, uint8_t* feat_q, int64_t ld_q,
                           int32_t* row_isum, int64_t* row_isq, int32_t* row_flags, void* stream) {
    return project_rows(ctx, V, vdtype, B, X, Y, Z, mode, 1, ijk, scale_div, mask, feat, ld_feat, feat_q, ld_q, row_isum, row_isq,
                        row_flags, stream);
}

extern "C" int rml_project_slices(rml_ctx* ctx, const void* V, int vdtype, int64_t B, int X, int Y, int Z, int T,
                                  const int32_t* ijk, float scale_div, uint32_t mask,
                                  float* feat, int64_t ld_feat, uint8_t* feat_q, int64_t ld_q,
                                  int32_t* row_isum, int64_t* row_isq, int32_t* row_flags, void* stream) {
    RML_REQUIRE(T >= 1 && B >= 0 && B * (int64_t)T < (int64_t)1 << 31, RML_ERR_INVALID, "rml_project_slices: bad target count");
    RML_REQUIRE(B == 0 || ijk != nullptr, RML_ERR_INVALID, "rml_project_slices: ijk is NULL");
    return project_rows(ctx, V, vdtype, B * T, X, Y, Z, RML_MODE_SLICE, T, ijk, scale_div, mask, feat, ld_feat, feat_q, ld_q, row_isum,
                        row_isq, row_flags, stream);
}

static void rows_out(ProjOut& o, int X, int Y, int Z, uint32_t mask, float scale_div, float* feat, int64_t ld_feat, uint8_t* feat_q,
                     int64_t ld_q, int32_t* row_isum, int64_t* row_isq, int32_t* row_flags) {
    int64_t off = 0;
    for (int pl = 0; pl < 3; ++pl) {
        if (mask & (1u << pl)) {
            o.p[pl] = feat ? feat + off : nullptr;
            o.stride[pl] = ld_feat;
            o.q[pl] = feat_q ? feat_q + off : nullptr;
            off += plane_len(pl, X, Y, Z);
        }
    }
    o.sel = mask & RML_MASK_ALL;
    o.qstride = ld_q;
    o.qrow = feat_q; o.qD = rml_feature_len(X, Y, Z, mask);
    o.row_isum = row_isum; o.row_isq = row_isq; o.row_flags = row_flags;
    o.scale_div = scale_div;
}

static int derive_two_kernels(rml_ctx* ctx, const void* V, int vdtype, int64_t B, int X, int Y, int Z, int num_targets, int32_t* ijk,
                              float* profiles, hipStream_t st);
static int derive_two_kernels_at(rml_ctx* ctx, const void* V, int vdtype, int64_t B, int X, int Y, int Z, int num_targets, int32_t* ijk,
                                 float* profiles, float* xzs, hipStream_t st);

int rml_launch_derive(rml_ctx* ctx, const void* V, int vdtype, int64_t B, int X, int Y, int Z, int num_targets, int32_t* ijk,
                      float* sums, hipStream_t st) {
    ProjOut none{};
    const int rc = rml_launch_derive_slice(ctx, V, vdtype, B, X, Y, Z, num_targets, ijk, nullptr, none, st);
    return rc != RML_ERR_UNSUPPORTED ? rc : derive_two_kernels_at(ctx, V, vdtype, B, X, Y, Z, num_targets, ijk, nullptr, sums, st);
}

extern "C" int rml_derive_slice_supported(const rml_ctx* ctx, const void* V, int vdtype, int X, int Y, int Z, int num_targets) {
    if (X <= 0 || Y <= 0 || Z <= 0 || (vdtype != RML_VOL_F32 && vdtype != RML_VOL_U8)) return 0;
    if (ctx && !ctx->opt.derive_fused) return 0;
    const size_t quad = vdtype == RML_VOL_U8 ? 4 : 16;
    if (V && (reinterpret_cast<uintptr_t>(V) & (quad - 1))) return 0;
    return derive_slice_shape_ok(X, Y, Z, num_targets) ? 1 : 0;
}

extern "C" int rml_derive_slice(rml_ctx* ctx, const void* V, int vdtype, int64_t B, int X, int Y, int Z, int num_targets,
                                int32_t* ijk, float* profiles, float scale_div, uint32_t mask,
                                float* feat, int64_t ld_feat, uint8_t* feat_q, int64_t ld_q,
                                int32_t* row_isum, int64_t* row_isq, int32_t* row_flags, void* stream) {
    RML_REQUIRE(ctx && B >= 0 && X > 0 && Y > 0 && Z > 0, RML_ERR_INVALID, "rml_derive_slice: bad arguments");
    if (B == 0) return RML_OK;
    RML_REQUIRE(V != nullptr, RML_ERR_INVALID, "rml_derive_slice: V is NULL");
    RML_REQUIRE(vdtype == RML_VOL_F32 || vdtype == RML_VOL_U8, RML_ERR_INVALID, "rml_derive_slice: unknown volume dtype %d", vdtype);
    RML_REQUIRE((mask & RML_MASK_ALL) != 0, RML_ERR_INVALID, "rml_derive_slice: empty projection mask");
    RML_REQUIRE(num_targets >= 1 && num_targets <= X && num_targets <= Y && num_targets <= Z, RML_ERR_INVALID,
                "rml_derive_slice: num_targets out of range");
    RML_REQUIRE(B * (int64_t)num_targets < (int64_t)1 << 31, RML_ERR_UNSUPPORTED, "rml_derive_slice: too many rows for one launch");
    const int64_t D = rml_feature_len(X, Y, Z, mask);
    RML_REQUIRE(!feat || ld_feat >= D, RML_ERR_INVALID, "rml_derive_slice: ld_feat < D");
    RML_REQUIRE(!feat_q || (ld_q >= D && ld_q % 4 == 0 && (reinterpret_cast<uintptr_t>(feat_q) & 3) == 0),
                RML_ERR_INVALID, "rml_derive_slice: feat_q needs ld_q >= D, ld_q %% 4 == 0 and 4-byte alignment");
    RML_HIP(hipSetDevice(ctx->device));
    hipStream_t st = static_cast<hipStream_t>(stream);
    ProjOut o{};
    rows_out(o, X, Y, Z, mask, scale_div, feat, ld_feat, feat_q, ld_q, row_isum, row_isq, row_flags);
    int rc = rml_launch_derive_slice(ctx, V, vdtype, B, X, Y, Z, num_targets, ijk, profiles, o, st);
    if (rc != RML_ERR_UNSUPPORTED) return rc;
    rml_ctx_guard guard(ctx, st);
    int32_t* ijk_w = ijk;
    if (!ijk_w) {
        const size_t planes = (size_t)B * ((size_t)X * Z + (size_t)Y * Z) * sizeof(float);
        void* ws = nullptr;
        rc = rml_ws_reserve(ctx, planes + (size_t)B * num_targets * 3 * sizeof(int32_t), &ws, st);
        if (rc) return rc;
        ijk_w = reinterpret_cast<int32_t*>(static_cast<unsigned char*>(ws) + planes);
    }
    rc = derive_two_kernels(ctx, V, vdtype, B, X, Y, Z, num_targets, ijk_w, profiles, st);
    if (rc) return rc;
    return rml_launch_project(ctx, V, vdtype, B * num_targets, X, Y, Z, RML_MODE_SLICE, ijk_w, o, st, num_targets);
}

static int project_rows(rml_ctx* ctx, const void* V, int vdtype, int64_t B, int X, int Y, int Z, int mode, int tpf,
                        const int32_t* ijk, float scale_div, uint32_t mask,
                        float* feat, int64_t ld_feat, uint8_t* feat_q, int64_t ld_q,
                        int32_t* row_isum, int64_t* row_isq, int32_t* row_flags, void* stream) {
    RML_REQUIRE(ctx && B >= 0 && X > 0 && Y > 0 && Z > 0, RML_ERR_INVALID, "rml_project: bad arguments");
    if (B == 0) return RML_OK;
    RML_REQUIRE(V != nullptr, RML_ERR_INVALID, "rml_project: V is NULL");
    RML_REQUIRE((mask & RML_MASK_ALL) != 0, RML_ERR_INVALID, "rml_project: empty projection mask");
    RML_REQUIRE(B < (int64_t)1 << 31, RML_ERR_UNSUPPORTED, "rml_project: B too large for one launch");
    const int64_t D = rml_feature_len(X, Y, Z, mask);
    RML_REQUIRE(!feat || ld_feat >= D, RML_ERR_INVALID, "rml_project: ld_feat < D");
    RML_REQUIRE(!feat_q || (ld_q >= D && ld_q % 4 == 0 && (reinterpret_cast<uintptr_t>(feat_q) & 3) == 0),
                RML_ERR_INVALID, "rml_project: feat_q needs ld_q >= D, ld_q %% 4 == 0 and 4-byte alignment");
    RML_HIP(hipSetDevice(ctx->device));
    ProjOut o{};
    int64_t off = 0;
    for (int pl = 0; pl < 3; ++pl) {
        if (mask & (1u << pl)) {
            o.p[pl] = feat ? feat + off : nullptr;
            o.stride[pl] = ld_feat;
            o.q[pl] = feat_q ? feat_q + off : nullptr;
            off += plane_len(pl, X, Y, Z);
        }
    }
    o.sel = mask & RML_MASK_ALL;
    o.qstride = ld_q;
    o.qrow = feat_q; o.qD = D;
    o.row_isum = row_isum; o.row_isq = row_isq; o.row_flags = row_flags;
    o.scale_div = scale_div;
    return rml_launch_project(ctx, V, vdtype, B, X, Y, Z, mode, ijk, o, static_cast<hipStream_t>(stream), tpf);
}

extern "C" int rml_project_occupancy(rml_ctx* ctx, const void* V, int vdtype, int64_t B, int X, int Y, int Z, int mode, float scale_div,
                                     uint32_t mask, uint8_t* feat_q, int64_t ld_q, int32_t* row_isum, int64_t* row_isq, int32_t* row_flags,
                                     uint32_t* occ, int occ_words, void* stream) {
    RML_REQUIRE(ctx && B >= 0 && X > 0 && Y > 0 && Z > 0, RML_ERR_INVALID, "rml_project_occupancy: bad arguments");
    if (B == 0) return RML_OK;
    RML_REQUIRE(V && feat_q && occ, RML_ERR_INVALID, "rml_project_occupancy: NULL argument");
    RML_REQUIRE(mode == RML_MODE_MAX || mode == RML_MODE_SUM || mode == RML_MODE_MAX_NAN, RML_ERR_INVALID, "rml_project_occupancy: mode MAX or SUM");
    RML_REQUIRE((mask & RML_MASK_ALL) != 0, RML_ERR_INVALID, "rml_project_occupancy: empty projection mask");
    RML_REQUIRE(B < (int64_t)1 << 31, RML_ERR_UNSUPPORTED, "rml_project_occupancy: B too large for one launch");
    const int64_t D = rml_feature_len(X, Y, Z, mask);
    RML_REQUIRE(ld_q >= D && ld_q % 128 == 0 && (reinterpret_cast<uintptr_t>(feat_q) & 127) == 0, RML_ERR_INVALID,
                "rml_project_occupancy: code rows need ld_q >= D, ld_q %% 128 == 0 and 128-byte alignment");
    RML_REQUIRE(occ_words == (int)(((D + 127) / 128 + 31) / 32), RML_ERR_INVALID, "rml_project_occupancy: occ_words must be ceil(ceil(D / 128) / 32)");
    RML_HIP(hipSetDevice(ctx->device));
    ProjOut o{};
    rows_out(o, X, Y, Z, mask, scale_div, nullptr, 0, feat_q, ld_q, row_isum, row_isq, row_flags);
    o.occ = occ; o.occ_words = occ_words;
    return rml_launch_project(ctx, V, vdtype, B, X, Y, Z, mode, nullptr, o, static_cast<hipStream_t>(stream));
}

extern "C" int rml_project_planes(rml_ctx* ctx, const void* V, int vdtype, int64_t B, int X, int Y, int Z, int mode,
                                  const int32_t* ijk, float* xz, float* yz, float* xy, void* stream) {
    RML_REQUIRE(ctx && B >= 0 && X > 0 && Y > 0 && Z > 0, RML_ERR_INVALID, "rml_project_planes: bad arguments");
    if (B == 0) return RML_OK;
    RML_REQUIRE(V != nullptr, RML_ERR_INVALID, "rml_project_planes: V is NULL");
    RML_REQUIRE(B < (int64_t)1 << 31, RML_ERR_UNSUPPORTED, "rml_project_planes: B too large for one launch");
    RML_HIP(hipSetDevice(ctx->device));
    ProjOut o{};
    o.p[0] = xz; o.stride[0] = (int64_t)X * Z;
    o.p[1] = yz; o.stride[1] = (int64_t)Y * Z;
    o.p[2] = xy; o.stride[2] = (int64_t)X * Y;
    o.sel = (xz ? 1u : 0u) | (yz ? 2u : 0u) | (xy ? 4u : 0u);
    o.scale_div = 0.0f;
    return rml_launch_project(ctx, V, vdtype, B, X, Y, Z, mode, ijk, o, static_cast<hipStream_t>(stream));
}

extern "C" int rml_derive_targets(rml_ctx* ctx, const void* V, int vdtype, int64_t B, int X, int Y, int Z,
                                  int num_targets, int32_t* ijk, float* profiles, void* stream) {
    RML_REQUIRE(ctx && B >= 0 && X > 0 && Y > 0 && Z > 0, RML_ERR_INVALID, "rml_derive_targets: bad arguments");
    if (B == 0) return RML_OK;
    RML_REQUIRE(V && ijk, RML_ERR_INVALID, "rml_derive_targets: NULL argument");
    RML_REQUIRE(num_targets >= 1 && num_targets <= X && num_targets <= Y && num_targets <= Z, RML_ERR_INVALID,
                "rml_derive_targets: num_targets out of range");
    RML_HIP(hipSetDevice(ctx->device));
    if (B == 0) return RML_OK;
    hipStream_t st = static_cast<hipStream_t>(stream);
    ProjOut none{};
    int rc1 = rml_launch_derive_slice(ctx, V, vdtype, B, X, Y, Z, num_targets, ijk, profiles, none, st);
    if (rc1 != RML_ERR_UNSUPPORTED) return rc1;
    rml_ctx_guard guard(ctx, st);
    return derive_two_kernels(ctx, V, vdtype, B, X, Y, Z, num_targets, ijk, profiles, st);
}

static int derive_two_kernels(rml_ctx* ctx, const void* V, int vdtype, int64_t B, int X, int Y, int Z, int num_targets, int32_t* ijk,
                              float* profiles, hipStream_t st) {
    size_t need = (size_t)B * ((size_t)X * Z + (size_t)Y * Z) * sizeof(float);
    void* ws = nullptr;
    int rc = rml_ws_reserve(ctx, need, &ws, st);
    if (rc) return rc;
    return derive_two_kernels_at(ctx, V, vdtype, B, X, Y, Z, num_targets, ijk, profiles, static_cast<float*>(ws), st);
}

static int derive_two_kernels_at(rml_ctx* ctx, const void* V, int vdtype, int64_t B, int X, int Y, int Z, int num_targets, int32_t* ijk,
                                 float* profiles, float* xzs, hipStream_t st) {
    int rc;
    float* yzs = xzs + (size_t)B * X * Z;
    ProjOut o{};
    o.p[0] = xzs; o.stride[0] = (int64_t)X * Z;
    o.p[1] = yzs; o.stride[1] = (int64_t)Y * Z;
    o.sel = 3u;
    o.scale_div = 0.0f;
    rc = rml_launch_project(ctx, V, vdtype, B, X, Y, Z, RML_MODE_SUM, nullptr, o, st);
    if (rc) return rc;
    hipLaunchKernelGGL(k_profiles_topk, dim3((unsigned)B), dim3(64), (size_t)(X + Y + Z) * sizeof(float), st,
                       xzs, yzs, X, Y, Z, num_targets, ijk, profiles);
    RML_HIP(hipGetLastError());
    return RML_OK;
}

extern "C" int rml_assemble_features(rml_ctx* ctx, const float* xz, const float* yz, const float* xy,
                                     int64_t B, int X, int Y, int Z, float scale_div, uint32_t mask,
                                     float* feat, int64_t ld_feat, void* stream) {
    RML_REQUIRE(ctx && B >= 0 && X > 0 && Y > 0 && Z > 0, RML_ERR_INVALID, "rml_assemble_features: bad arguments");
    if (B == 0) return RML_OK;
    RML_REQUIRE(feat != nullptr, RML_ERR_INVALID, "rml_assemble_features: feat is NULL");
    RML_REQUIRE((mask & RML_MASK_ALL) != 0, RML_ERR_INVALID, "rml_assemble_features: empty mask");
    const float* src[3] = {xz, yz, xy};
    for (int pl = 0; pl < 3; ++pl)
        RML_REQUIRE(!(mask & (1u << pl)) || src[pl], RML_ERR_INVALID, "rml_assemble_features: selected plane %d is NULL", pl);
    const int64_t D = rml_feature_len(X, Y, Z, mask);
    RML_REQUIRE(ld_feat >= D, RML_ERR_INVALID, "rml_assemble_features: ld_feat < D");
    RML_HIP(hipSetDevice(ctx->device));
    if (B == 0) return RML_OK;
    ProjOut o{};
    int64_t off = 0;
    for (int pl = 0; pl < 3; ++pl)
        if (mask & (1u << pl)) { o.p[pl] = feat + off; o.stride[pl] = ld_feat; off += plane_len(pl, X, Y, Z); }
    o.sel = mask & RML_MASK_ALL;
    o.scale_div = scale_div;
    ProjParams pp;
    fill_params(pp, ctx, nullptr, B, X, Y, Z, nullptr, o);
    hipLaunchKernelGGL(k_assemble, dim3((unsigned)B), dim3(kThreads), 0, static_cast<hipStream_t>(stream),
                       (mask & 1u) ? xz : nullptr, (mask & 2u) ? yz : nullptr, (mask & 4u) ? xy : nullptr, pp);
    RML_HIP(hipGetLastError());
    return RML_OK;
}

extern "C" int rml_quantize_rows(rml_ctx* ctx, const float* feat, int64_t N, int64_t D, int64_t ld_feat,
                                 float scale_div, uint8_t* feat_q, int64_t ld_q,
                                 int32_t* row_isum, int64_t* row_isq, int32_t* row_flags, void* stream) {
    RML_REQUIRE(ctx && N >= 0 && D > 0 && ld_feat >= D && ld_q >= D, RML_ERR_INVALID, "rml_quantize_rows: bad arguments");
    if (N == 0) return RML_OK;
    RML_REQUIRE(feat && feat_q, RML_ERR_INVALID, "rml_quantize_rows: NULL argument");
    RML_HIP(hipSetDevice(ctx->device));
    if (N == 0) return RML_OK;
    ProjOut o{};
    o.q[0] = feat_q; o.qstride = ld_q; o.qrow = feat_q; o.qD = D; o.sel = 1u;
    o.row_isum = row_isum; o.row_isq = row_isq; o.row_flags = row_flags;
    o.scale_div = 0.0f;
    ProjParams pp;
    fill_params(pp, ctx, nullptr, N, 1, 1, 1, nullptr, o);
    hipLaunchKernelGGL(k_quantize_rows, dim3((unsigned)N), dim3(kThreads), 0, static_cast<hipStream_t>(stream),
                       feat, D, ld_feat, scale_div, pp);
    RML_HIP(hipGetLastError());
    return RML_OK;
}
```

### radar-ml_amd/csrc/project_shared.h

```cpp
#pragma once
#include "rml_internal.h"
#include <math.h>
#include <stdlib.h>
#include <type_traits>

namespace rmlproj {

constexpr int kThreads = 256;

struct ProjParams {
    const void* V;
    int64_t B;
    int X, Y, Z, ZQ;
    const int32_t* ijk;
    int tpf;
    int rpl;
    ProjOut o;
    int vec_ok[3];
    int ntgt;
    int32_t* ijk_out;
    float* profiles;
    int wave_lds;
    int stage_bytes;
    int k_waveframe, k_linplane, k_stage_codes, k_slice_wave, k_derive_fused;
    int* occ_done;
};

template <int MODE> struct Op;
template <> struct Op<RML_MODE_MAX> {
    static __device__ __forceinline__ float ident() { return -INFINITY; }
    static __device__ __forceinline__ float f(float a, float b) { return __builtin_elementwise_maximum(a, b); }
    static __device__ __forceinline__ uint32_t key(float v) {
        const uint32_t b = __float_as_uint(v);
        const uint32_t k = b ^ ((uint32_t)((int32_t)b >> 31) | 0x80000000u);
        return v != v ? 0xFFFFFFFFu : k;
    }
    static __device__ __forceinline__ float lds_ident() { return __uint_as_float(key(-INFINITY)); }
    static __device__ __forceinline__ float lds_value(float stored) {
        const uint32_t k = __float_as_uint(stored);
        const uint32_t b = (k & 0x80000000u) ? (k ^ 0x80000000u) : ~k;
        return k == 0xFFFFFFFFu ? __uint_as_float(0x7FC00000u) : __uint_as_float(b);
    }
    static __device__ __forceinline__ void lds_atomic(float* p, float v) {
        __hip_atomic_fetch_max(reinterpret_cast<uint32_t*>(p), key(v), __ATOMIC_RELAXED, __HIP_MEMORY_SCOPE_WORKGROUP);
    }
};
template <> struct Op<RML_MODE_SUM> {
    static __device__ __forceinline__ float ident() { return 0.0f; }
    static __device__ __forceinline__ float f(float a, float b) { return a + b; }
    static __device__ __forceinline__ float lds_ident() { return 0.0f; }
    static __device__ __forceinline__ float lds_value(float stored) { return stored; }
    static __device__ __forceinline__ void lds_atomic(float* p, float v) {
        __hip_atomic_fetch_add(p, v, __ATOMIC_RELAXED, __HIP_MEMORY_SCOPE_WORKGROUP);
    }
};

template <int MODE> __device__ __forceinline__ float4 op4(float4 a, float4 b) {
    return make_float4(Op<MODE>::f(a.x, b.x), Op<MODE>::f(a.y, b.y), Op<MODE>::f(a.z, b.z), Op<MODE>::f(a.w, b.w));
}

__device__ __forceinline__ float4 bytes_to_float4(uint32_t w) {
    return make_float4((float)(w & 0xFFu), (float)((w >> 8) & 0xFFu), (float)((w >> 16) & 0xFFu), (float)(w >> 24));
}

struct Emitter {
    const ProjParams& a;
    int64_t b;
    __device__ __forceinline__ int64_t qb() const { return b; }
    int32_t isum = 0;
    uint32_t isq = 0;
    int ok = 1;
    double nsq = 0.0;
    bool want_stats;
    bool rmw;
    typedef __attribute__((address_space(3))) uint8_t lds_u8;
    typedef __attribute__((address_space(3))) uint32_t lds_u32;
    typedef uint32_t u32x4 __attribute__((ext_vector_type(4)));
    typedef __attribute__((address_space(3))) u32x4 lds_u128;
    lds_u8* stage = nullptr;
    int staged = 0;
    int stage_xy = 0;
    int occ_on = 0;
    int occ_off = 0;
    __device__ __forceinline__ void set_stage(unsigned char* p, int xy_off) {
        stage = (lds_u8*)p; staged = 1; stage_xy = xy_off;
        if (a.o.occ) {
            occ_on = 1; occ_off = xy_off + ((a.X * a.Y + 15) & ~15);
            for (int w = threadIdx.x & 63; w < a.o.occ_words; w += 64) *(lds_u32*)(stage + occ_off + 4 * w) = 0u;
        }
    }
    __device__ __forceinline__ void occ_mark(int at) {
        const int k = at >> 7;
        __hip_atomic_fetch_or((lds_u32*)(stage + occ_off + 4 * (k >> 5)), 1u << (k & 31), __ATOMIC_RELAXED, __HIP_MEMORY_SCOPE_WAVEFRONT);
    }
    __device__ __forceinline__ int plane_at(int pl) const { return (int)(a.o.q[pl] - a.o.qrow); }

    __device__ Emitter(const ProjParams& a_, int64_t b_) : a(a_), b(b_) {
        want_stats = a.o.row_isum || a.o.row_isq || a.o.row_flags || a.o.q[0] || a.o.q[1] || a.o.q[2];
        rmw = a.o.q_rmw != 0;
    }
    __device__ __forceinline__ float scaled(float v) const {
        return (a.o.scale_div > 1.0f) ? __fdiv_rn(v, a.o.scale_div) : v;
    }
    __device__ __forceinline__ uint32_t code(float v) {
        int c = (int)v;
        bool good = ((float)c == v) && c >= 0 && c <= 255;
        ok &= good ? 1 : 0;
        c = good ? c : 0;
        isum += c;
        isq += (uint32_t)(c * c);
        return (uint32_t)(c ^ 0x80);
    }
    __device__ __forceinline__ void put_code1(int pl, int64_t idx, int c, bool good) {
        ok &= good ? 1 : 0;
        c = good ? c : 0;
        isum += c;
        isq += (uint32_t)(c * c);
        if (a.o.q[pl]) a.o.q[pl][b * a.o.qstride + idx] = (uint8_t)(c ^ 0x80);
    }
    __device__ __forceinline__ void put1(int pl, int64_t idx, float v) {
        if (!((a.o.sel >> pl) & 1u)) return;
        if (a.o.p[pl]) a.o.p[pl][b * a.o.stride[pl] + idx] = scaled(v);
        if (a.o.row_nsq) { double t = (double)scaled(v); nsq += t * t; }
        if (want_stats) {
            uint32_t c = code(v);
            if (a.o.q[pl]) {
                if (staged && pl != 1) stage[(pl == 2 ? stage_xy : 0) + idx] = (uint8_t)c;
                else {
                    a.o.q[pl][b * a.o.qstride + idx] = (uint8_t)c;
                    if (occ_on && c != 0x80u) occ_mark(plane_at(pl) + (int)idx);
                }
            }
        }
    }
    __device__ __forceinline__ uint32_t old_word(int pl, int64_t idx) const {
        if (!(rmw && a.o.q[pl] && ((a.o.sel >> pl) & 1u))) return 0u;
        return *reinterpret_cast<const uint32_t*>(a.o.q[pl] + qb() * a.o.qstride + idx);
    }
    __device__ __forceinline__ uint32_t old_word_nocheck(int pl, int64_t idx) const {
        return *reinterpret_cast<const uint32_t*>(a.o.q[pl] + qb() * a.o.qstride + idx);
    }
    __device__ __forceinline__ void put_bytes4(int pl, int64_t idx, uint32_t w, bool have_old = false, uint32_t old = 0u) {
        if (!((a.o.sel >> pl) & 1u)) return;
        if (a.o.p[pl] || a.o.row_nsq) { put4(pl, idx, bytes_to_float4(w), have_old, old); return; }
        if (want_stats) {
            isum += (int32_t)__builtin_amdgcn_udot4(w, 0x01010101u, 0u, false);
            isq = __builtin_amdgcn_udot4(w, w, isq, false);
            if (a.o.q[pl]) {
                uint32_t* dq = reinterpret_cast<uint32_t*>(a.o.q[pl] + qb() * a.o.qstride + idx);
                const uint32_t nv = w ^ 0x80808080u;
                if (!rmw || (have_old ? old : *dq) != nv) *dq = nv;
            }
        }
    }
    __device__ __forceinline__ void put4(int pl, int64_t idx, float4 v, bool have_old = false, uint32_t old = 0u) {
        if (!((a.o.sel >> pl) & 1u)) return;
        if (a.o.p[pl]) {
            float* dst = a.o.p[pl] + b * a.o.stride[pl] + idx;
            float4 s = make_float4(scaled(v.x), scaled(v.y), scaled(v.z), scaled(v.w));
            if (a.o.row_nsq) {
                nsq += (double)s.x * (double)s.x + (double)s.y * (double)s.y;
                nsq += (double)s.z * (double)s.z + (double)s.w * (double)s.w;
            }
            if (a.vec_ok[pl]) {
                *reinterpret_cast<float4*>(dst) = s;
            } else {
                typedef float f32x4u __attribute__((ext_vector_type(4), aligned(4)));
                *reinterpret_cast<f32x4u*>(dst) = f32x4u{s.x, s.y, s.z, s.w};
            }
        }
        if (want_stats) {
            uint32_t c0 = code(v.x), c1 = code(v.y), c2 = code(v.z), c3 = code(v.w);
            if (a.o.q[pl]) {
                uint32_t packed = c0 | (c1 << 8) | (c2 << 16) | (c3 << 24);
                if (staged && pl != 1) *(lds_u32*)(stage + (pl == 2 ? stage_xy : 0) + idx) = packed;
                else {
                    uint32_t* dq = reinterpret_cast<uint32_t*>(a.o.q[pl] + qb() * a.o.qstride + idx);
                    if (!rmw || (have_old ? old : *dq) != packed) *dq = packed;
                    if (occ_on && packed != 0x80808080u) occ_mark(plane_at(pl) + (int)idx);
                }
            }
        }
    }
    __device__ __forceinline__ void reset(int64_t b_) { b = b_; isum = 0; isq = 0; ok = 1; nsq = 0.0; }
    __device__ void flush_wave(int lane) {
        if (!staged) return;
        __builtin_amdgcn_fence(__ATOMIC_ACQ_REL, "wavefront");
        const int len[2] = {a.X * a.Z, a.X * a.Y};
        lds_u8* src[2] = {stage, stage + stage_xy};
        uint8_t* dst[2] = {a.o.q[0] + qb() * a.o.qstride, a.o.q[2] + qb() * a.o.qstride};
        const int at[2] = {occ_on ? plane_at(0) : 0, occ_on ? plane_at(2) : 0};
#pragma unroll
        for (int r = 0; r < 2; ++r) {
            int done = 0;
            if ((reinterpret_cast<uintptr_t>(dst[r]) & 15) == 0) {
                for (int i = lane; i < (len[r] >> 4); i += 64) {
                    const u32x4 v = ((lds_u128*)src[r])[i];
                    reinterpret_cast<u32x4*>(dst[r])[i] = v;
                    if (occ_on && ((v.x ^ 0x80808080u) | (v.y ^ 0x80808080u) | (v.z ^ 0x80808080u) | (v.w ^ 0x80808080u))) occ_mark(at[r] + 16 * i);
                }
                done = len[r] & ~15;
            }
            for (int i = done + 4 * lane; i + 4 <= len[r]; i += 256) {
                const uint32_t v = *(lds_u32*)(src[r] + i);
                *reinterpret_cast<uint32_t*>(dst[r] + i) = v;
                if (occ_on && v != 0x80808080u) occ_mark(at[r] + i);
            }
            for (int i = (len[r] & ~3) + lane; i < len[r]; i += 64) {
                const uint8_t v = src[r][i];
                dst[r][i] = v;
                if (occ_on && v != 0x80u) occ_mark(at[r] + i);
            }
        }
        __builtin_amdgcn_fence(__ATOMIC_ACQ_REL, "wavefront");
        if (occ_on) {
            const int kpad = (int)(a.o.qD >> 7);
            for (int w = lane; w < a.o.occ_words; w += 64) {
                lds_u32* lw = (lds_u32*)(stage + occ_off + 4 * w);
                uint32_t v = *lw;
                if ((a.o.qD & 127) && (kpad >> 5) == w) v |= 1u << (kpad & 31);
                a.o.occ[qb() * a.o.occ_words + w] = v;
                *lw = 0u;
            }
            __builtin_amdgcn_fence(__ATOMIC_ACQ_REL, "wavefront");
        }
    }
    __device__ void finish_wave(int lane) {
        if (a.o.qrow) {
            for (int64_t c = a.o.qD + lane; c < a.o.qstride; c += 64) a.o.qrow[b * a.o.qstride + c] = 0;
        }
        if (a.o.prow) {
            for (int64_t c = a.o.pD + lane; c < a.o.pstride; c += 64) a.o.prow[b * a.o.pstride + c] = 0.0f;
        }
        if (!(a.o.row_isum || a.o.row_isq || a.o.row_flags || a.o.row_nsq)) return;
        int64_t s = isum, q = isq;
        int g = ok;
        double nn = nsq;
#pragma unroll
        for (int off = 32; off >= 1; off >>= 1) {
            s += __shfl_xor(s, off);
            q += __shfl_xor(q, off);
            g &= __shfl_xor(g, off);
            nn += __shfl_xor(nn, off);
        }
        if (lane == 0) {
            if (a.o.row_isum) a.o.row_isum[b] = (int32_t)s;
            if (a.o.row_isq) a.o.row_isq[b] = q;
            if (a.o.row_flags) a.o.row_flags[b] = (int32_t)g;
            if (a.o.row_nsq) a.o.row_nsq[b] = nn;
        }
    }
    __device__ void finish(int64_t* red) {
        if (a.o.qrow) {
            for (int64_t c = a.o.qD + threadIdx.x; c < a.o.qstride; c += blockDim.x) a.o.qrow[b * a.o.qstride + c] = 0;
        }
        if (a.o.prow) {
            for (int64_t c = a.o.pD + threadIdx.x; c < a.o.pstride; c += blockDim.x) a.o.prow[b * a.o.pstride + c] = 0.0f;
        }
        if (!(a.o.row_isum || a.o.row_isq || a.o.row_flags || a.o.row_nsq)) return;
        int64_t s = isum, q = isq;
        int g = ok;
        double nn = nsq;
#pragma unroll
        for (int off = 32; off >= 1; off >>= 1) {
            s += __shfl_xor(s, off);
            q += __shfl_xor(q, off);
            g &= __shfl_xor(g, off);
            nn += __shfl_xor(nn, off);
        }
        int lane = threadIdx.x & 63, wave = threadIdx.x >> 6;
        double* redd = reinterpret_cast<double*>(red + 48);
        __syncthreads();
        if (lane == 0) { red[wave * 3 + 0] = s; red[wave * 3 + 1] = q; red[wave * 3 + 2] = g; redd[wave] = nn; }
        __syncthreads();
        if (threadIdx.x == 0) {
            int64_t S = 0, Q = 0, G = 1;
            double NN = 0.0;
            for (int w = 0; w < (int)(blockDim.x + 63) / 64; ++w) { S += red[w * 3]; Q += red[w * 3 + 1]; G &= red[w * 3 + 2]; NN += redd[w]; }
            if (a.o.row_isum) a.o.row_isum[b] = (int32_t)S;
            if (a.o.row_isq) a.o.row_isq[b] = Q;
            if (a.o.row_flags) a.o.row_flags[b] = (int32_t)G;
            if (a.o.row_nsq) a.o.row_nsq[b] = NN;
        }
    }
};

__device__ __forceinline__ float4 ld_stream(const float4* p) {
    typedef float v4f_t __attribute__((ext_vector_type(4)));
    v4f_t v = __builtin_nontemporal_load(reinterpret_cast<const v4f_t*>(p));
    return make_float4(v.x, v.y, v.z, v.w);
}

__device__ __forceinline__ float4 ld_stream(const uint32_t* p) {
    const uint32_t w = __builtin_nontemporal_load(p);
    return make_float4((float)(w & 0xFFu), (float)((w >> 8) & 0xFFu), (float)((w >> 16) & 0xFFu), (float)(w >> 24));
}
template <typename VT> struct Quad;
template <> struct Quad<float> { typedef float4 T; };
template <> struct Quad<uint8_t> { typedef uint32_t T; };

template <int MODE, int LPR> __device__ __forceinline__ float row_reduce(float r) {
#pragma unroll
    for (int off = LPR / 2; off >= 1; off >>= 1) r = Op<MODE>::f(r, __shfl_xor(r, off));
    return r;
}

template <int CTRL, int ROW_MASK, bool BOUND>
__device__ __forceinline__ float dpp_mov(float old, float v) {
    return __int_as_float(__builtin_amdgcn_update_dpp(__float_as_int(old), __float_as_int(v), CTRL, ROW_MASK, 0xF, BOUND));
}
template <int MODE> __device__ __forceinline__ float wave_reduce_uniform(float r) {
    const float id = Op<MODE>::ident();
    r = Op<MODE>::f(r, dpp_mov<0xB1, 0xF, true>(id, r));
    r = Op<MODE>::f(r, dpp_mov<0x4E, 0xF, true>(id, r));
    r = Op<MODE>::f(r, dpp_mov<0x141, 0xF, true>(id, r));
    r = Op<MODE>::f(r, dpp_mov<0x140, 0xF, true>(id, r));
    r = Op<MODE>::f(r, dpp_mov<0x142, 0xA, false>(id, r));
    r = Op<MODE>::f(r, dpp_mov<0x143, 0xC, false>(id, r));
    return __int_as_float(__builtin_amdgcn_readlane(__float_as_int(r), 63));
}

template <int N, typename F> __device__ __forceinline__ void static_for(F&& f) {
    if constexpr (N > 0) {
        static_for<N - 1>(f);
        f(std::integral_constant<int, N - 1>{});
    }
}
template <int J> __device__ __forceinline__ float park_lane(float acc, float uniform_val) {
    asm("v_writelane_b32 %0, %1, %2" : "+v"(acc) : "s"(uniform_val), "n"(J));
    return acc;
}

template <int MODE> __device__ __forceinline__ float op_raw(float a, float b) {
    if constexpr (MODE == RML_MODE_MAX) {
        float r;
        asm("v_maximum3_f32 %0, %1, %2, %2" : "=v"(r) : "v"(a), "v"(b));
        return r;
    } else
    {
        return Op<MODE>::f(a, b);
    }
}
template <int MODE> __device__ __forceinline__ float4 op4_raw(float4 a, float4 b) {
    return make_float4(op_raw<MODE>(a.x, b.x), op_raw<MODE>(a.y, b.y), op_raw<MODE>(a.z, b.z), op_raw<MODE>(a.w, b.w));
}

inline int code_stage_bytes(const ProjParams& pp, size_t voxel_bytes) {
    const ProjOut& o = pp.o;
    if (voxel_bytes != 4 || o.p[0] || o.p[1] || o.p[2] || o.row_nsq || !o.q[0] || !o.q[2] || o.skip_if_set) return 0;
    if (!pp.k_stage_codes) return 0;
    const int bytes = ((pp.X * pp.Z + 15) & ~15) + ((pp.X * pp.Y + 15) & ~15) + (o.occ ? (4 * o.occ_words + 15) & ~15 : 0);
    return bytes <= 16 * 1024 ? bytes : 0;
// ... 12 lines not shown
```

### radar-ml_amd/csrc/rml_internal.h

```cpp
#pragma once
#include <hip/hip_runtime.h>
#include <stdint.h>
#include <cstdlib>
#include <atomic>
#include <mutex>
#include <string>
#include <vector>
#include "../../include/radarml.h"

struct rml_resize_tab {
    int in, out, ksize;
    const int* bounds;
    const double* kk;
};

struct rml_pre_tab {
    int X, Y, Z, OH, OW;
    void* dev;
    size_t off[6];
};

struct rml_opts {
    int project_share_cu = 0;
    int waveframe = 1;
    int linplane = 1;
    int stage_codes = 1;
    int slice_wave = 1;
    int derive_fused = 1;
    int code_rmw = -1;
    int gemm_big = -1;
    int c1_pk = 1;
    int64_t chunk = 0;
    int smo_lds_rows = RML_SMO_LDS_ROWS_MAX;
    int conv7 = RML_CONV7_DEFAULT;
    int sgd_resident_d = RML_SGD_RESIDENT_D_MAX;
    int sparse_rows = -1;
    int zoom_rows = 0;
};

struct rml_ws_retired {
    void* p;
    hipEvent_t ev;
};

struct rml_ctx {
    int device = 0;
    int num_cu = 256;
    void* ws = nullptr;
    size_t ws_bytes = 0;
    std::vector<rml_ws_retired> ws_retired;
    rml_opts opt;
    hipEvent_t ev_fork = nullptr, ev_join = nullptr;
    hipEvent_t ev_proj[2] = {nullptr, nullptr}, ev_done[2] = {nullptr, nullptr};
    hipStream_t aux_stream = nullptr;
    mutable int64_t sparse_gemm_launches = 0;
    uint8_t* bg_line = nullptr;
    bool profiling = false;
    std::vector<hipEvent_t> prof_ev;
    size_t prof_used = 0;
    int64_t prof_frames = 0;
    std::vector<hipEvent_t> prof_ev_g;
    size_t prof_used_g = 0;
    double prof_ops_g = 0.0;
    std::vector<rml_resize_tab> resize_tabs;
    std::vector<rml_pre_tab> pre_tabs;
    std::recursive_mutex mu;
    hipEvent_t ev_last = nullptr;
    bool ev_last_valid = false;
    void* stage = nullptr;
    size_t stage_bytes = 0;
    hipEvent_t ev_stage = nullptr;
    bool ev_stage_valid = false;
};

struct rml_ctx_guard {
    rml_ctx* ctx;
    hipStream_t st;
    bool capturing = false;
    explicit rml_ctx_guard(rml_ctx* c, hipStream_t stream) : ctx(c), st(stream) {
        ctx->mu.lock();
        hipStreamCaptureStatus cs = hipStreamCaptureStatusNone;
        if (hipStreamIsCapturing(st, &cs) != hipSuccess) (void)hipGetLastError();
        capturing = cs != hipStreamCaptureStatusNone;
        if (!capturing && ctx->ev_last_valid) (void)hipStreamWaitEvent(st, ctx->ev_last, 0);
    }
    ~rml_ctx_guard() {
        if (!capturing && ctx->ev_last && hipEventRecord(ctx->ev_last, st) == hipSuccess) ctx->ev_last_valid = true;
        ctx->mu.unlock();
    }
    rml_ctx_guard(const rml_ctx_guard&) = delete;
    rml_ctx_guard& operator=(const rml_ctx_guard&) = delete;
};

void rml_prof_mark(rml_ctx* ctx, hipStream_t st);
void rml_prof_mark_gemm(rml_ctx* ctx, hipStream_t st);

struct rml_once_per_device {
    std::atomic<uint64_t> mask{0};
    bool first(int dev) { const uint64_t bit = 1ull << (dev & 63); return !(mask.fetch_or(bit) & bit); }
};
#define RML_MAX_DYN_LDS(bytes, ...)                                                                                     \
    do {                                                                                                                \
        static rml_once_per_device _once;                                                                               \
        int _dev = 0;                                                                                                   \
        (void)hipGetDevice(&_dev);                                                                                      \
        if (_once.first(_dev))                                                                                          \
            (void)hipFuncSetAttribute(reinterpret_cast<const void*>(__VA_ARGS__), hipFuncAttributeMaxDynamicSharedMemorySize, (bytes)); \
    } while (0)

void rml_set_error(const char* fmt, ...);
int rml_hip_fail(hipError_t e, const char* what, const char* file, int line);

#define RML_HIP(call)                                                        \
    do {                                                                     \
        hipError_t _e = (call);                                              \
        if (_e != hipSuccess) return rml_hip_fail(_e, #call, __FILE__, __LINE__); \
    } while (0)

#define RML_REQUIRE(cond, status, ...)      \
    do {                                    \
        if (!(cond)) {                      \
            rml_set_error(__VA_ARGS__);     \
            return (status);                \
        }                                   \
    } while (0)

int rml_ws_reserve(rml_ctx* ctx, size_t bytes, void** out, hipStream_t st);

int rml_stage_reserve(rml_ctx* ctx, size_t bytes, void** host);
int rml_stage_upload(rml_ctx* ctx, void* dst, size_t bytes, hipStream_t st);

struct ProjOut {
    float* p[3];
    int64_t stride[3];
    uint32_t sel;
    uint8_t* q[3];
    int64_t qstride;
    uint8_t* qrow;
    int64_t qD;
    int32_t* row_isum;
    int64_t* row_isq;
    int32_t* row_flags;
    float scale_div;
    float* prow;
    int64_t pD, pstride;
    double* row_nsq;
    const int32_t* skip_if_set;
    int share_cu;
    int no_pad;
    int q_rmw;
    uint32_t* occ;
    int occ_words;
};
inline int rml_code_rmw(int64_t D, int64_t frame_bytes, bool derive, bool u8) {
    if (derive) return 0;
    return u8 && D * 64 >= frame_bytes && D * 16 <= frame_bytes;
}

inline int rml_sparse_rows(int X, int Y, int Z) {
    return (Z % 128 == 0 || 128 % Z == 0) && ((int64_t)X * Z) % 128 == 0 && ((int64_t)Y * Z) % 128 == 0;
}

bool rml_project_uses_wave_kernel(const rml_ctx* ctx, int vdtype, int mode, int X, int Y, int Z, bool share_cu, int64_t B);

int rml_launch_project(rml_ctx* ctx, const void* V, int vdtype, int64_t B, int X, int Y, int Z, int mode,
                       const int32_t* ijk, const ProjOut& o, hipStream_t st, int targets_per_frame = 1);

constexpr int RML_SMALL_FRAMES = 8;
int rml_project_split_pieces(int X, int Y, int Z);
size_t rml_project_split_scratch_bytes(int64_t B, int X, int Y, int Z, int S);
int rml_launch_project_split(rml_ctx* ctx, const void* V, int vdtype, int64_t B, int X, int Y, int Z, const ProjOut& o, float* scratch, int S,
                             hipStream_t st);

int rml_launch_derive_slice(rml_ctx* ctx, const void* V, int vdtype, int64_t B, int X, int Y, int Z, int num_targets,
                            int32_t* ijk_out, float* profiles, const ProjOut& o, hipStream_t st);

int rml_launch_derive(rml_ctx* ctx, const void* V, int vdtype, int64_t B, int X, int Y, int Z, int num_targets, int32_t* ijk,
                      float* sums, hipStream_t st);

struct rml_zoom_plan {
    int vdtype, X, Y, Z, T; uint32_t mask; int32_t out_shape[6];
    bool codes;
    bool derive;
    int64_t Dsrc, Dout, ld_src;
    size_t lds; int by_plane;
};
int rml_zoom_plan_make(const rml_ctx* ctx, const char* who, int vdtype, int mode, int X, int Y, int Z, int T, bool derive, const int32_t* out_shape,
                       uint32_t mask, rml_zoom_plan* zp);
size_t rml_zoom_stage_bytes(const rml_zoom_plan& zp, int64_t frames);
int rml_zoom_stage_run(rml_ctx* ctx, const rml_zoom_plan& zp, void* scratch, const void* V, int64_t frames, int mode, const int32_t* ijk,
                       float scale_div, float* feat, int64_t ld_feat, int64_t pad_to, double* row_nsq, int32_t* row_flags, hipStream_t st);

struct rml_svm {
    int64_t M = 0, Mpad = 0, D = 0;
    int64_t Kq = 0;
    int64_t Kf = 0;
    int64_t Dq = 0;
    int64_t Df = 0;
    int C = 0, P = 0, PT = 0, kernel = 0;
    double gamma = 0, code_scale = 1;
    bool exact = false, has_calib = false;
    float* sv_f32 = nullptr;
    double* sv_nsq = nullptr;
    uint8_t* sv_q = nullptr;
    double* sv_term_q = nullptr;
    double* W = nullptr;
    double* intercept = nullptr;
    double* calib = nullptr;
    double* platt = nullptr;
    bool dig_ok = false;
    double dig_c0 = 0, dig_s = 1;
    int8_t* sv_dig = nullptr;
    double* sv_dig_nsq = nullptr;
    uint32_t mask_hint = 0;
    uint32_t* sv_occ = nullptr;
    int occ_words = 0;
};

struct rml_svm_pack {
    std::vector<double> W, nsq, term, dnsq;
    std::vector<float> svf;
    std::vector<uint8_t> svq;
    std::vector<int8_t> svd;
    std::vector<uint32_t> occ;
};
int rml_svm_pack_host(const double* sv, int64_t M, int64_t D, const double* dual_coef, const int32_t* n_support,
                      int n_classes, int kernel, double gamma, double code_scale, bool has_calib, rml_svm* m, rml_svm_pack* pk);
size_t rml_svm_ws_bytes(const rml_svm* m, int64_t CH, unsigned needs);

struct rml_linear {
    int64_t D = 0;
    int C = 0;
    bool has_calib = false;
    double* coef = nullptr;
    double* intercept = nullptr;
    double* calib = nullptr;
};
```

### radar-ml_amd/csrc/svm.hip

```cpp
#include "rml_internal.h"
#include "svm_tile.h"
#include "svm_ring.h"
#include "svm_small.h"
#include "svm_rows.h"
#include "svm_finish.h"
#include <math.h>
#include <vector>
#include <stdlib.h>
#include <type_traits>
#include <algorithm>
#include <new>

namespace {

inline bool use_dig_gemm(const rml_svm* m, int policy, int64_t n, int num_cu) {
    if (!m->dig_ok) return false;
    if (policy == RML_PATH_DIGITS) return true;
    if (policy != RML_PATH_AUTO) return false;
    const int64_t wgs = ((n + kBig - 1) / kBig) * ((m->Mpad + kBig - 1) / kBig);
    return wgs * 2 >= (int64_t)num_cu;
}

inline bool use_big_gemm(const rml_svm* m, int64_t n, int num_cu, int knob) {
    if (knob == 0 || m->PT > 6) return false;
    if (knob == 1) return n >= 256;
    const int64_t wgs = ((n + kBig - 1) / kBig) * ((m->Mpad + kBig - 1) / kBig);
    const int64_t rounds = (wgs + num_cu - 1) / num_cu;
    return wgs * 4 >= (int64_t)num_cu * 3 && wgs * 4 >= rounds * num_cu * 3;
}

inline int64_t round_up(int64_t v, int64_t m) { return (v + m - 1) / m * m; }

template <typename T> int dev_upload(T** dst, const std::vector<T>& h) {
    RML_HIP(hipMalloc(reinterpret_cast<void**>(dst), h.size() * sizeof(T)));
    RML_HIP(hipMemcpy(*dst, h.data(), h.size() * sizeof(T), hipMemcpyHostToDevice));
    return RML_OK;
}

RingArgs ring_args_from(const GemmArgs& ga) {
    RingArgs ra{};
    ra.sv = ga.sv; ra.x = ga.x; ra.ld_sv = ga.ld_sv; ra.ld_x = ga.ld_x; ra.KT = ga.KT;
    ra.N = ga.N; ra.Mpad = ga.Mpad; ra.sv_rows = ga.sv_rows; ra.ST = ga.ST; ra.FT = ga.FT;
    ra.tile_exact = ga.tile_exact; ra.want = ga.want; ra.x_isum = ga.x_isum; ra.x_isq = ga.x_isq;
    ra.sv_term = ga.sv_term; ra.W = ga.W; ra.gs = ga.gs; ra.kernel = ga.kernel; ra.partial = ga.partial; ra.Npart = ga.Npart;
    return ra;
}
int launch_gemm_big(const rml_svm* m, const GemmArgs& ga, hipStream_t st) { return launch_gemm_ring<0>(m, ring_args_from(ga), st); }
SmallArgs small_args_from(const GemmArgs& ga, int32_t* G, int64_t g_sm, int64_t g_sn) {
    SmallArgs sa{};
    sa.N = (int)ga.N; sa.Mpad = ga.Mpad; sa.tile_exact = ga.tile_exact; sa.G = G; sa.g_sm = g_sm; sa.g_sn = g_sn;
    sa.x_isum = ga.x_isum; sa.x_isq = ga.x_isq; sa.sv_term = ga.sv_term; sa.W = ga.W; sa.gs = ga.gs; sa.kernel = ga.kernel;
    sa.partial = ga.partial; sa.Npart = ga.Npart;
    return sa;
}
inline bool ring_takes(const rml_ctx* ctx, const rml_svm* m, int64_t n) { return use_big_gemm(m, n, ctx->num_cu, ctx->opt.gemm_big); }

int64_t pick_chunk_opt(const rml_ctx* ctx, int64_t fallback) { return ctx->opt.chunk >= 128 ? round_up(ctx->opt.chunk, kTile) : fallback; }
int64_t pick_chunk(const rml_ctx* ctx, const rml_svm* m, int64_t rows, int64_t fallback, bool dig) {
    const int64_t env = pick_chunk_opt(ctx, 0);
    const int num_cu = ctx->num_cu;
    int64_t ch = fallback;
    if (env) ch = env;
    else if (dig || (m->exact && ring_takes(ctx, m, 32768))) {
        const int64_t st2 = (m->Mpad + kBig - 1) / kBig;
        auto rounds = [&](int64_t n) { return n <= 0 ? (int64_t)0 : (((n + kBig - 1) / kBig) * st2 + num_cu - 1) / num_cu; };
        const int64_t total = round_up(rows, kBig);
        int64_t best = -1;
        const int64_t cmax = dig ? std::max<int64_t>(4096 / 4, std::min<int64_t>(32768, (2048 / st2) * kBig)) : 32768;
        for (int64_t c = std::min<int64_t>(4096, cmax); c <= cmax; c += kBig) {
            const int64_t nfull = total / c, rem = total % c;
            const int64_t cost = 20 * (nfull * rounds(c) + rounds(rem)) + 3 * (nfull + (rem ? 1 : 0));
            if (best < 0 || cost <= best) { best = cost; ch = c; }
            if (c >= total) break;
        }
    }
    return std::min<int64_t>(round_up(rows, kTile), ch);
}

struct ChunkWs {
    uint8_t* q; float* f32; int32_t* isum; int64_t* isq; double* nsq; int32_t* flags;
    int32_t* tile_exact; int32_t* all_exact; double* partial;
    int8_t* dig; int64_t dig_plane; double* dnsq; int32_t* dflags;
    int32_t* stash;
    int32_t* ijk;
    int32_t* gsmall;
    int32_t* gsplit;
    uint32_t* occ;
    size_t bytes;
};

struct ChunkNeeds { bool q, f32, dig, ijk, occ; };
constexpr int64_t kSplitRows = 2048;

ChunkWs carve(const rml_svm* m, int64_t CH, unsigned char* base, const ChunkNeeds& need) {
    ChunkWs w{}; size_t off = 0;
    auto take = [&](size_t bytes) { size_t o = off; off = (off + bytes + 255) & ~(size_t)255; return base && bytes ? base + o : (unsigned char*)nullptr; };
    w.q = (uint8_t*)take(need.q ? (size_t)CH * m->Dq : 0);
    w.f32 = (float*)take(need.f32 ? (size_t)CH * m->Df * 4 : 0);
    w.isum = (int32_t*)take((size_t)CH * 4); w.isq = (int64_t*)take((size_t)CH * 8);
    w.nsq = (double*)take((size_t)CH * 8); w.flags = (int32_t*)take((size_t)CH * 4);
    w.tile_exact = (int32_t*)take((size_t)(CH / kTile + 1) * 4); w.all_exact = (int32_t*)take(256);
    w.partial = (double*)take((size_t)(m->Mpad / kTile) * CH * m->PT * 8);
    w.dig_plane = CH * m->Dq;
    w.dig = (int8_t*)take(need.dig ? (size_t)4 * CH * m->Dq : 0);
    w.dnsq = (double*)take(need.dig ? (size_t)CH * 8 : 0); w.dflags = (int32_t*)take(need.dig ? (size_t)CH * 4 : 0);
    w.stash = (int32_t*)take(need.dig ? (size_t)ring_grid((int)((CH + kBig - 1) / kBig), (int)((m->Mpad + kBig - 1) / kBig)) * 2 * kDigStashBytes : 0);
    w.ijk = (int32_t*)take(need.ijk ? (size_t)CH * 12 : 0);
    w.gsmall = (int32_t*)take(need.q ? (size_t)RML_SMALL_FRAMES * m->Mpad * 4 : 0);
    w.gsplit = (int32_t*)take(need.q && CH <= kSplitRows ? (size_t)m->Mpad * CH * 4 : 0);
    w.occ = (uint32_t*)take(need.q && need.occ ? (size_t)CH * m->occ_words * 4 : 0);
    w.bytes = off;
    return w;
}

int reserve_chunks(rml_ctx* ctx, const rml_svm* m, int64_t CH, const ChunkNeeds& need, hipStream_t st, ChunkWs* w, int nbuf,
                   size_t extra = 0, void** extra_at = nullptr) {
    const size_t each = carve(m, CH, nullptr, need).bytes;
    void* ws = nullptr;
    if (int rc = rml_ws_reserve(ctx, (size_t)nbuf * each + extra, &ws, st)) return rc;
    unsigned char* base = static_cast<unsigned char*>(ws);
    for (int i = 0; i < nbuf; ++i) w[i] = carve(m, CH, base + (size_t)i * each, need);
    if (extra_at) *extra_at = base + (size_t)nbuf * each;
    return RML_OK;
}

struct DecisionOut {
    double* dec_ovo; double* dec_ovr; double* proba; int32_t* label_vote; int32_t* label_calib;
    DecisionOut at(int64_t r0, int C, int P) const {
        auto adv = [r0](auto* p, int64_t per_row) { return p ? p + r0 * per_row : p; };
        return DecisionOut{adv(dec_ovo, P), adv(dec_ovr, C == 2 ? 1 : C), adv(proba, C), adv(label_vote, 1), adv(label_calib, 1)};
    }
};

struct ChunkOps { int64_t n; const uint8_t* q; int64_t ld_q; const int32_t* isum; const int64_t* isq; const int32_t* flags; const float* f32; const double* nsq;
                  const uint32_t* occ; };
ChunkOps ws_rows(const rml_svm* m, const ChunkWs& w, int64_t n) { return ChunkOps{n, w.q, m->Dq, w.isum, w.isq, w.flags, w.f32, w.nsq, nullptr}; }

struct ChunkPlan {
    int policy;
    bool tiles_done;
    bool all_exact_known;
    bool allow_big;
    bool dig_ready;
    double* kmat; int64_t ld_k;
    int FT, ST, group; bool run_i8, run_gen, gen_f32, big, run_dig, small, split, sparse;
};

ChunkPlan plan_chunk(const rml_ctx* ctx, const rml_svm* m, ChunkPlan p, const ChunkOps& x, const ChunkWs& w) {
    p.FT = (int)((x.n + kTile - 1) / kTile); p.ST = (int)(m->Mpad / kTile);
    p.run_i8 = m->exact && x.q && (p.policy == RML_PATH_AUTO || p.policy == RML_PATH_I8);
    p.run_gen = x.f32 && p.policy != RML_PATH_I8; p.gen_f32 = (p.policy == RML_PATH_F32);
    p.big = p.allow_big && p.run_i8 && !p.kmat && ring_takes(ctx, m, x.n);
    p.run_dig = p.dig_ready && w.dig && p.run_gen && !p.gen_f32 && !p.kmat && m->dig_ok;
    p.group = (p.big || p.run_dig) ? 2 : 1;
    p.small = p.run_i8 && !p.kmat && x.n <= RML_SMALL_FRAMES && w.gsmall && (m->Mpad % kSmallSv) == 0;
    p.split = p.run_i8 && !p.kmat && !p.small && !p.big && w.gsplit && x.n <= kSplitRows && (int64_t)p.FT * p.ST < ctx->num_cu &&
              m->Kq / kStepBytes >= 8;
    const bool can_sparse = p.run_i8 && !p.kmat && !p.small && !p.big && x.occ && m->sv_occ && ctx->bg_line && ctx->opt.sparse_rows != 0 &&
                            m->occ_words <= kSparseMaxWords;
    if (can_sparse && ctx->opt.sparse_rows > 0) p.split = false;
    p.sparse = can_sparse && !p.split;
    return p;
}

void launch_tile_flags(const rml_svm* m, const ChunkOps& x, const ChunkPlan& p, const ChunkWs& w, int32_t* all_exact, hipStream_t st) {
    const int blocks = (p.FT + p.group - 1) / p.group + (all_exact ? 1 : 0);
    hipLaunchKernelGGL(k_tile_flags, dim3(blocks), dim3(128 * p.group), 0, st, x.flags, x.n, p.FT, p.run_i8 ? (p.run_gen ? 0 : 2) : 1,
                       (int)m->exact, w.tile_exact, all_exact, p.group);
}
void launch_tile_dig(const ChunkOps& x, const ChunkPlan& p, const ChunkWs& w, hipStream_t st) {
    hipLaunchKernelGGL(k_tile_dig, dim3((p.FT + 1) / 2), dim3(256), 0, st, w.dflags, x.n, p.FT, w.tile_exact, (const int32_t*)nullptr);
}
void launch_digit_rows(const rml_svm* m, const ChunkWs& w, int64_t n, hipStream_t st) {
    hipLaunchKernelGGL(k_digit_rows, dim3((unsigned)n), dim3(256), 0, st, w.f32, m->Df, m->D, m->Dq, w.dig_plane, w.dig, w.dnsq,
                       w.dflags, m->dig_c0, 2147483648.0 / m->dig_s, (const int32_t*)nullptr);
}

int run_finish(const rml_svm* m, const ChunkOps& x, const ChunkPlan& p, const ChunkWs& w, const DecisionOut& out, hipStream_t st) {
    FinishArgs fa{};
    fa.partial = w.partial; fa.Npart = x.n; fa.ST = p.ST; fa.PT = m->PT; fa.N = x.n; fa.C = m->C; fa.P = m->P;
    fa.intercept = m->intercept; fa.calib = m->calib; fa.has_calib = m->has_calib;
    fa.row_flags = p.all_exact_known ? nullptr : x.flags; fa.tile_exact = p.all_exact_known ? nullptr : w.tile_exact;
    fa.forced_i8 = p.run_i8 && !p.run_gen;
    fa.dec_ovo = out.dec_ovo; fa.dec_ovr = out.dec_ovr; fa.proba = out.proba; fa.label_vote = out.label_vote; fa.label_calib = out.label_calib;
    hipLaunchKernelGGL(k_svm_finish, dim3((unsigned)((x.n + 255) / 256)), dim3(256), 0, st, fa);
    RML_HIP(hipGetLastError());
    return RML_OK;
}

int launch_epi(const rml_svm* m, const SmallArgs& sa, int ST, int64_t n, hipStream_t st) {
    const dim3 ge((unsigned)ST, (unsigned)n);
    switch (m->PT) {
        case 1: hipLaunchKernelGGL(k_svm_epi_small<1>, ge, dim3(128), 0, st, sa); break;
        case 3: hipLaunchKernelGGL(k_svm_epi_small<3>, ge, dim3(128), 0, st, sa); break;
        case 6: hipLaunchKernelGGL(k_svm_epi_small<6>, ge, dim3(128), 0, st, sa); break;
        case 10: hipLaunchKernelGGL(k_svm_epi_small<10>, ge, dim3(128), 0, st, sa); break;
        case 15: hipLaunchKernelGGL(k_svm_epi_small<15>, ge, dim3(128), 0, st, sa); break;
        default: RML_REQUIRE(false, RML_ERR_UNSUPPORTED, "svm: unsupported pair count");
    }
    RML_HIP(hipGetLastError());
    return RML_OK;
}

int launch_small(const rml_svm* m, const GemmArgs& ga, int32_t* G, hipStream_t st) {
    SmallArgs sa = small_args_from(ga, G, 1, ga.Mpad);
    sa.sv = ga.sv; sa.ld_sv = ga.ld_sv; sa.x = ga.x; sa.ld_x = ga.ld_x; sa.Kb = (int64_t)ga.KT * kStepBytes;
    const dim3 gd((unsigned)(ga.Mpad / kSmallSv));
    if (ga.N <= 1) hipLaunchKernelGGL(k_svm_dot_small<1>, gd, dim3(256), 0, st, sa);
    else if (ga.N <= 2) hipLaunchKernelGGL(k_svm_dot_small<2>, gd, dim3(256), 0, st, sa);
    else if (ga.N <= 4) hipLaunchKernelGGL(k_svm_dot_small<4>, gd, dim3(256), 0, st, sa);
    else hipLaunchKernelGGL(k_svm_dot_small<8>, gd, dim3(256), 0, st, sa);
    return launch_epi(m, sa, ga.ST, ga.N, st);
}

int launch_split(const rml_svm* m, const GemmArgs& ga, int32_t* G, int num_cu, hipStream_t st) {
    const int64_t ldg = (int64_t)ga.FT * kTile;
    const int64_t n16 = ga.Mpad * ldg / 4;
    hipLaunchKernelGGL(k_zero16, dim3((unsigned)((n16 + 255) / 256)), dim3(256), 0, st, reinterpret_cast<v4i*>(G), n16);
    SplitArgs sp{};
    sp.sv = ga.sv; sp.ld_sv = ga.ld_sv; sp.x = ga.x; sp.ld_x = ga.ld_x; sp.KT = ga.KT; sp.N = ga.N; sp.FT = ga.FT;
    sp.tile_exact = ga.tile_exact; sp.G = G; sp.ldg = ldg;
    const int tiles = ga.FT * ga.ST;
    int KS = (2 * num_cu + tiles - 1) / tiles;
    if (KS > ga.KT / 4) KS = ga.KT / 4;
    if (KS < 1) KS = 1;
    sp.per = (ga.KT + KS - 1) / KS;
    KS = (ga.KT + sp.per - 1) / sp.per;
    hipLaunchKernelGGL(k_svm_gemm_splitk, dim3((unsigned)tiles, (unsigned)KS), dim3(256), 0, st, sp);
    return launch_epi(m, small_args_from(ga, G, ldg, 1), ga.ST, ga.N, st);
}

RingArgs digit_args(const rml_svm* m, const ChunkOps& x, const ChunkPlan& p, const ChunkWs& w) {
    RingArgs ra{};
    ra.sv = reinterpret_cast<const uint8_t*>(m->sv_dig); ra.x = reinterpret_cast<const uint8_t*>(w.dig);
    ra.ld_sv = m->Dq; ra.ld_x = m->Dq; ra.sv_plane = m->Mpad * m->Dq; ra.x_plane = w.dig_plane;
    ra.KT = (int)(m->Kq / kStepBytes); ra.N = x.n; ra.Mpad = m->Mpad; ra.sv_rows = m->Mpad; ra.ST = p.ST; ra.FT = p.FT;
    ra.tile_exact = w.tile_exact; ra.want = 2; ra.x_nsq = w.dnsq; ra.sv_term = m->sv_dig_nsq; ra.W = m->W;
    ra.gs = m->gamma * m->dig_s * m->dig_s; ra.kernel = RML_KERNEL_RBF; ra.partial = w.partial; ra.Npart = x.n; ra.stash = w.stash;
    return ra;
}

int run_chunk(const rml_ctx* ctx, const rml_svm* m, const ChunkOps& x, const ChunkPlan& asked, const ChunkWs& w, const DecisionOut& out,
              hipStream_t st) {
    const ChunkPlan p = plan_chunk(ctx, m, asked, x, w);
    RML_REQUIRE(p.run_i8 || p.run_gen, RML_ERR_STATE, "svm: no usable operand path (model exact=%d)", (int)m->exact);
    if (!p.tiles_done) {
        launch_tile_flags(m, x, p, w, nullptr, st);
        if (p.run_dig) launch_tile_dig(x, p, w, st);
    }
    GemmArgs ga{};
    ga.N = x.n; ga.ST = p.ST; ga.FT = p.FT; ga.tile_exact = p.all_exact_known ? nullptr : w.tile_exact;
    ga.W = m->W; ga.Mpad = m->Mpad; ga.kernel = m->kernel; ga.partial = w.partial; ga.Npart = x.n;
    ga.kmat = p.kmat; ga.ld_k = p.ld_k; ga.M = m->M; ga.sv_rows = m->Mpad;
    int rc = RML_OK;
    if (p.run_i8) {
        ga.sv = m->sv_q; ga.ld_sv = m->Dq; ga.x = x.q; ga.ld_x = x.ld_q; ga.KT = (int)(m->Kq / kStepBytes);
        ga.want = 1; ga.x_isum = x.isum; ga.x_isq = x.isq; ga.sv_term = m->sv_term_q;
        ga.gs = (m->kernel == RML_KERNEL_RBF ? m->gamma : 1.0) / (m->code_scale * m->code_scale);
        if (p.kmat) rc = launch_gemm<PATH_I8, true>(m, ga, st);
        else if (p.small) rc = launch_small(m, ga, w.gsmall, st);
        else if (p.split) rc = launch_split(m, ga, w.gsplit, ctx->num_cu, st);
        else if (p.big) rc = launch_gemm_big(m, ga, st);
        else if (p.sparse) {
            ga.sv_occ = m->sv_occ; ga.x_occ = x.occ; ga.ow = m->occ_words; ga.bg_line = ctx->bg_line;
            ++ctx->sparse_gemm_launches;
            rc = launch_gemm<PATH_I8, false, true>(m, ga, st);
        } else rc = launch_gemm<PATH_I8>(m, ga, st);
        if (rc) return rc;
    }
    if (p.run_dig && (rc = launch_gemm_ring<1>(m, digit_args(m, x, p, w), st))) return rc;
    if (p.run_gen) {
        ga.sv = reinterpret_cast<const uint8_t*>(m->sv_f32); ga.ld_sv = m->Df * 4;
        ga.x = reinterpret_cast<const uint8_t*>(x.f32); ga.ld_x = m->Df * 4; ga.KT = (int)(m->Kf * 4 / kStepBytes);
        ga.want = 0; ga.x_nsq = x.nsq; ga.sv_term = m->sv_nsq; ga.gs = m->gamma;
        rc = p.gen_f32 ? launch_gemm<PATH_F32>(m, ga, st)
                       : (p.kmat ? launch_gemm<PATH_F64, true>(m, ga, st) : launch_gemm<PATH_F64>(m, ga, st));
        if (rc) return rc;
    }
    if (p.kmat) { RML_HIP(hipGetLastError()); return RML_OK; }
    return run_finish(m, x, p, w, out, st);
}
}

int rml_svm_pack_host(const double* sv, int64_t M, int64_t D, const double* dual_coef, const int32_t* n_support,
                      int n_classes, int kernel, double gamma, double code_scale, bool has_calib, rml_svm* m, rml_svm_pack* pk) {
    RML_REQUIRE(sv && dual_coef && n_support && m && pk, RML_ERR_INVALID, "rml_svm_load: NULL argument");
    RML_REQUIRE(M > 0 && D > 0, RML_ERR_INVALID, "rml_svm_load: empty model");
    RML_REQUIRE(n_classes >= 2 && n_classes <= kMaxC, RML_ERR_UNSUPPORTED, "rml_svm_load: %d classes (supported: 2..%d)", n_classes, kMaxC);
    RML_REQUIRE(kernel == RML_KERNEL_RBF || kernel == RML_KERNEL_LINEAR, RML_ERR_UNSUPPORTED, "rml_svm_load: kernel %d", kernel);
    int64_t msum = 0;
    for (int c = 0; c < n_classes; ++c) { RML_REQUIRE(n_support[c] >= 0, RML_ERR_INVALID, "rml_svm_load: negative n_support"); msum += n_support[c]; }
    RML_REQUIRE(msum == M, RML_ERR_INVALID, "rml_svm_load: sum(n_support)=%lld != M=%lld", (long long)msum, (long long)M);
    m->M = M; m->D = D; m->C = n_classes; m->P = n_classes * (n_classes - 1) / 2;
    m->PT = m->P <= 1 ? 1 : (m->P <= 3 ? 3 : (m->P <= 6 ? 6 : (m->P <= 10 ? 10 : 15)));
    m->kernel = kernel; m->gamma = gamma; m->code_scale = code_scale > 1.0 ? code_scale : 1.0;
    m->Mpad = round_up(M, kTile);
    m->Kq = round_up(D, kStepBytes); m->Kf = round_up(D, 32);
    m->Dq = ((m->Kq / 128) & 1) ? m->Kq : m->Kq + 128;
    m->Df = ((m->Kf / 32) & 1) ? m->Kf : m->Kf + 32;
    m->has_calib = has_calib;

    std::vector<double>& W = pk->W;
    W.assign((size_t)m->PT * m->Mpad, 0.0);
    {
        std::vector<int64_t> start(n_classes, 0);
        for (int c = 1; c < n_classes; ++c) start[c] = start[c - 1] + n_support[c - 1];
        int p = 0;
        for (int i = 0; i < n_classes; ++i)
            for (int j = i + 1; j < n_classes; ++j, ++p) {
                for (int64_t k = 0; k < n_support[i]; ++k) W[(size_t)p * m->Mpad + start[i] + k] = dual_coef[(size_t)(j - 1) * M + start[i] + k];
                for (int64_t k = 0; k < n_support[j]; ++k) W[(size_t)p * m->Mpad + start[j] + k] = dual_coef[(size_t)i * M + start[j] + k];
            }
    }
    std::vector<float>& svf = pk->svf;
    std::vector<double>& nsq = pk->nsq;
    svf.assign((size_t)m->Mpad * m->Df, 0.0f);
    nsq.assign(m->Mpad, 0.0);
    std::vector<uint8_t>& svq = pk->svq;
    std::vector<double>& term = pk->term;
    svq.assign((size_t)m->Mpad * m->Dq, 0);
    term.assign(m->Mpad, 0.0);
    bool exact = true;
    const float fscale = (float)m->code_scale;
    for (int64_t r = 0; r < M; ++r) {
        double nn = 0.0; int64_t isum = 0, isq = 0;
        for (int64_t d = 0; d < D; ++d) {
            const double v = sv[(size_t)r * D + d];
            const float vf = (float)v;
            svf[(size_t)r * m->Df + d] = vf;
            nn += (double)vf * (double)vf;
            if (exact) {
                double c = nearbyint(v * m->code_scale);
                bool good = c >= 0.0 && c <= 255.0;
                if (good) {
                    double back = m->code_scale > 1.0 ? (double)((float)c / fscale) : c;
                    good = (back == v);
                }
                if (!good) exact = false;
                else { int ci = (int)c; svq[(size_t)r * m->Dq + d] = (uint8_t)(ci ^ 0x80); isum += ci; isq += (int64_t)ci * ci; }
            }
        }
        nsq[r] = nn;
        term[r] = (kernel == RML_KERNEL_RBF) ? (double)(isq - 256 * isum + 32768 * D) : (double)(128 * isum - 16384 * D);
    }
    m->occ_words = (int)((m->Kq / kStepBytes + 31) / 32);
    std::vector<uint32_t>& occ = pk->occ;
    occ.assign((size_t)m->Mpad * m->occ_words, 0u);
    for (int64_t r = 0; r < m->Mpad; ++r)
        for (int64_t k = 0; k < m->Kq / kStepBytes; ++k) {
            bool bg = r < M && (k + 1) * kStepBytes <= D;
            for (int t = 0; bg && t < kStepBytes; ++t) bg = svq[(size_t)r * m->Dq + k * kStepBytes + t] == 0x80;
            if (!bg) occ[(size_t)r * m->occ_words + (k >> 5)] |= 1u << (k & 31);
        }
    if (m->Kq >= 131072) exact = false;
    m->exact = exact;
    std::vector<int8_t>& svd = pk->svd;
    std::vector<double>& dnsq = pk->dnsq;
    svd.clear(); dnsq.clear();
    m->dig_ok = false;
    if (kernel == RML_KERNEL_RBF && m->Kq < 32768 && m->PT <= 6) {
        double lo = sv[0], hi = sv[0];
        bool finite = true;
        for (size_t i = 0; i < (size_t)M * D; ++i) { const double v = sv[i]; finite &= std::isfinite(v); lo = v < lo ? v : lo; hi = v > hi ? v : hi; }
        if (finite && hi > lo) {
            int e = 0;
            (void)frexp(hi - lo, &e);
            double sd = ldexp(1.0, e);
            if (ldexp(1.0, e - 1) == hi - lo) sd = hi - lo;
            const double c0 = nearbyint(0.5 * (lo + hi) / sd * 256.0) / 256.0 * sd;
            const double k31 = 2147483648.0 / sd;
            svd.assign((size_t)4 * m->Mpad * m->Dq, 0);
            dnsq.assign(m->Mpad, 0.0);
            const size_t plane = (size_t)m->Mpad * m->Dq;
            bool ok = true;
            for (int64_t r = 0; r < M && ok; ++r) {
                double nn = 0.0;
                for (int64_t d = 0; d < D; ++d) {
                    const double t = nearbyint((sv[(size_t)r * D + d] - c0) * k31);
                    if (!(t >= -2147483648.0 && t <= 2139062143.0)) { ok = false; break; }
                    const int32_t I = (int32_t)t;
                    const double u = (double)I * 0x1p-31;
                    nn += u * u;
                    const uint32_t pk4 = ((uint32_t)I + 0x00808080u) ^ 0x00808080u;
                    for (int dg = 0; dg < 4; ++dg) svd[(size_t)dg * plane + (size_t)r * m->Dq + d] = (int8_t)((pk4 >> (8 * (3 - dg))) & 255u);
                }
                dnsq[r] = nn;
            }
            if (ok) { m->dig_ok = true; m->dig_c0 = c0; m->dig_s = sd; }
        }
    }
    return RML_OK;
}

extern "C" int rml_svm_load(rml_ctx* ctx, const double* sv, int64_t M, int64_t D,
                            const double* dual_coef, const double* intercept, const int32_t* n_support,
                            int n_classes, int kernel, double gamma, double code_scale,
                            const double* calib_a, const double* calib_b, rml_svm** out) {
    RML_REQUIRE(ctx && sv && dual_coef && intercept && n_support && out, RML_ERR_INVALID, "rml_svm_load: NULL argument");
    RML_REQUIRE((calib_a == nullptr) == (calib_b == nullptr), RML_ERR_INVALID, "rml_svm_load: calib_a/calib_b must both be given");
    *out = nullptr;
    rml_svm* m = new (std::nothrow) rml_svm();
    RML_REQUIRE(m != nullptr, RML_ERR_NOMEM, "rml_svm_load: out of host memory");
    rml_svm_pack pk;
    int rc = rml_svm_pack_host(sv, M, D, dual_coef, n_support, n_classes, kernel, gamma, code_scale, calib_a != nullptr, m, &pk);
    if (rc) { delete m; return rc; }
    {
        hipError_t e = hipSetDevice(ctx->device);
        if (e != hipSuccess) { delete m; RML_HIP(e); }
    }
    const bool exact = m->exact;
    do {
        if ((rc = dev_upload(&m->W, pk.W))) break;
        if ((rc = dev_upload(&m->sv_f32, pk.svf))) break;
        if ((rc = dev_upload(&m->sv_nsq, pk.nsq))) break;
        if (exact) {
            if ((rc = dev_upload(&m->sv_q, pk.svq))) break;
            if ((rc = dev_upload(&m->sv_term_q, pk.term))) break;
            if ((rc = dev_upload(&m->sv_occ, pk.occ))) break;
        }
        if (m->dig_ok) {
            if ((rc = dev_upload(&m->sv_dig, pk.svd))) break;
            if ((rc = dev_upload(&m->sv_dig_nsq, pk.dnsq))) break;
        }
        std::vector<double> ic(intercept, intercept + m->P);
        if ((rc = dev_upload(&m->intercept, ic))) break;
        if (m->has_calib) {
            std::vector<double> cal(2 * n_classes);
            const int ncal = n_classes == 2 ? 1 : n_classes;
            for (int c = 0; c < n_classes; ++c) { cal[c] = c < ncal ? calib_a[c] : 0.0; cal[n_classes + c] = c < ncal ? calib_b[c] : 0.0; }
            if ((rc = dev_upload(&m->calib, cal))) break;
        }
    } while (0);
    if (rc) { rml_svm_free(ctx, m); return rc; }
    *out = m;
    return RML_OK;
}

extern "C" int rml_svm_free(rml_ctx* ctx, rml_svm* m) {
    if (!m) return RML_OK;
    if (ctx) (void)hipSetDevice(ctx->device);
    (void)hipDeviceSynchronize();
    void* bufs[] = {m->sv_f32, m->sv_nsq, m->sv_q, m->sv_term_q, m->W, m->intercept, m->calib, m->platt, m->sv_dig, m->sv_dig_nsq, m->sv_occ};
    for (void* b : bufs) if (b) (void)hipFree(b);
    delete m;
    return RML_OK;
}

extern "C" int rml_svm_sv_occupancy(rml_ctx* ctx, const rml_svm* m, uint32_t* out, int64_t n_words) {
    RML_REQUIRE(ctx && m && out, RML_ERR_INVALID, "rml_svm_sv_occupancy: NULL argument");
    RML_REQUIRE(m->sv_occ != nullptr, RML_ERR_STATE, "rml_svm_sv_occupancy: the model is not on the code grid");
    RML_REQUIRE(n_words == m->Mpad * m->occ_words, RML_ERR_INVALID, "rml_svm_sv_occupancy: out holds %lld words, the model has %lld",
                (long long)n_words, (long long)(m->Mpad * m->occ_words));
    RML_HIP(hipSetDevice(ctx->device));
    RML_HIP(hipMemcpy(out, m->sv_occ, (size_t)n_words * sizeof(uint32_t), hipMemcpyDeviceToHost));
    return RML_OK;
}
extern "C" int64_t rml_ctx_sparse_gemm_launches(const rml_ctx* ctx) { return ctx ? ctx->sparse_gemm_launches : 0; }
extern "C" int rml_svm_is_exact(const rml_svm* m) { return m && m->exact ? 1 : 0; }
extern "C" int64_t rml_svm_num_sv(const rml_svm* m) { return m ? m->M : 0; }
extern "C" int64_t rml_svm_dim(const rml_svm* m) { return m ? m->D : 0; }

size_t rml_svm_ws_bytes(const rml_svm* m, int64_t CH, unsigned needs) {
    return carve(m, CH, nullptr, ChunkNeeds{(needs & 1u) != 0, (needs & 2u) != 0, (needs & 4u) != 0, (needs & 8u) != 0, (needs & 16u) != 0}).bytes;
}

namespace {
int run_float_rows(const rml_ctx* ctx, const rml_svm* m, const float* feat, int64_t ld_feat, int64_t N, int64_t CH, const ChunkWs& w,
                   const ChunkPlan& plan, const DecisionOut& out, hipStream_t st) {
    for (int64_t r0 = 0; r0 < N; r0 += CH) {
        const int64_t n = std::min(CH, N - r0);
        hipLaunchKernelGGL(k_prepare_rows, dim3((unsigned)n), dim3(256), 0, st, feat + r0 * ld_feat, ld_feat, m->D,
                           (float)m->code_scale, w.f32, m->Df, w.nsq, w.q, m->Dq, w.isum, w.isq, w.flags);
        if (w.dig) launch_digit_rows(m, w, n, st);
        RML_HIP(hipGetLastError());
        ChunkPlan p = plan; if (p.kmat) p.kmat += r0 * p.ld_k;
        if (int rc = run_chunk(ctx, m, ws_rows(m, w, n), p, w, out.at(r0, m->C, m->P), st)) return rc;
    }
    return RML_OK;
}
}

extern "C" int rml_svm_decision(rml_ctx* ctx, const rml_svm* m, int path,
                                const float* feat, int64_t ld_feat,
                                const uint8_t* feat_q, int64_t ld_q, const int32_t* row_isum, const int64_t* row_isq,
                                const int32_t* row_flags, int64_t N,
                                double* dec_ovo, double* dec_ovr, double* proba,
                                int32_t* label_vote, int32_t* label_calib, void* stream) {
    RML_REQUIRE(ctx && m && N >= 0, RML_ERR_INVALID, "rml_svm_decision: bad arguments");
    if (N == 0) return RML_OK;
    RML_REQUIRE(feat || feat_q, RML_ERR_INVALID, "rml_svm_decision: need feat or feat_q");
    RML_REQUIRE(!feat || ld_feat >= m->D, RML_ERR_INVALID, "rml_svm_decision: ld_feat < D");
    RML_REQUIRE(path >= RML_PATH_AUTO && path <= RML_PATH_DIGITS, RML_ERR_INVALID, "rml_svm_decision: bad path %d", path);
    RML_REQUIRE(path != RML_PATH_DIGITS || m->dig_ok, RML_ERR_STATE, "rml_svm_decision: multi-digit path requested but the model has no digit frame "
                "(RBF kernel, D < 32768 and at most 6 class pairs)");
    RML_REQUIRE(!(proba || label_calib) || m->has_calib, RML_ERR_STATE, "rml_svm_decision: model has no calibrators");
    RML_REQUIRE(path != RML_PATH_I8 || m->exact, RML_ERR_STATE, "rml_svm_decision: exact path requested but the model is not on the code grid");
    if (!feat) {
        RML_REQUIRE(m->exact, RML_ERR_STATE, "rml_svm_decision: code rows given but the model is not on the code grid");
        RML_REQUIRE(path == RML_PATH_AUTO || path == RML_PATH_I8, RML_ERR_INVALID, "rml_svm_decision: the float paths need float rows");
        RML_REQUIRE(row_isum && row_isq, RML_ERR_INVALID, "rml_svm_decision: code rows need row_isum/row_isq");
        RML_REQUIRE(ld_q >= m->Kq && ld_q % 16 == 0 && (reinterpret_cast<uintptr_t>(feat_q) & 15) == 0, RML_ERR_INVALID,
                    "rml_svm_decision: code rows need ld_q >= %lld, ld_q %% 16 == 0 and 16-byte alignment", (long long)m->Kq);
    }
    RML_HIP(hipSetDevice(ctx->device));
    hipStream_t st = static_cast<hipStream_t>(stream);
    rml_ctx_guard guard(ctx, st);
    const DecisionOut out{dec_ovo, dec_ovr, proba, label_vote, label_calib};
    ChunkNeeds need{};
    need.q = feat && m->exact && (path == RML_PATH_AUTO || path == RML_PATH_I8); need.f32 = feat != nullptr;
    need.dig = feat && use_dig_gemm(m, path, N, ctx->num_cu);
    const bool dig_rounds = need.dig && !m->exact;
    const int64_t CH = (dig_rounds || m->exact) ? pick_chunk(ctx, m, N, 8192, dig_rounds) : std::min<int64_t>(round_up(N, kTile), 8192);
    ChunkWs w; int rc = reserve_chunks(ctx, m, CH, need, st, &w, 1);
    if (rc) return rc;
    ChunkPlan plan{};
    plan.policy = feat ? path : RML_PATH_I8; plan.allow_big = true; plan.dig_ready = need.dig;
    if (feat) return run_float_rows(ctx, m, feat, ld_feat, N, CH, w, plan, out, st);
    for (int64_t r0 = 0; r0 < N && !rc; r0 += CH) {
        const ChunkOps x{std::min(CH, N - r0), feat_q + r0 * ld_q, ld_q, row_isum + r0, row_isq + r0, row_flags ? row_flags + r0 : nullptr,
                         nullptr, nullptr};
        rc = run_chunk(ctx, m, x, plan, w, out.at(r0, m->C, m->P), st);
    }
    return rc;
}

extern "C" int rml_svm_kernel_matrix(rml_ctx* ctx, const rml_svm* m, int path, const float* feat, int64_t ld_feat, int64_t N,
                                     double* kmat, int64_t ld_k, void* stream) {
    RML_REQUIRE(ctx && m && N >= 0, RML_ERR_INVALID, "rml_svm_kernel_matrix: bad arguments");
    if (N == 0) return RML_OK;
    RML_REQUIRE(feat && kmat, RML_ERR_INVALID, "rml_svm_kernel_matrix: NULL argument");
    RML_REQUIRE(ld_feat >= m->D && ld_k >= m->M, RML_ERR_INVALID, "rml_svm_kernel_matrix: ld_feat < D or ld_k < M");
    RML_REQUIRE(path == RML_PATH_AUTO || path == RML_PATH_I8 || path == RML_PATH_F64, RML_ERR_INVALID,
                "rml_svm_kernel_matrix: path must be AUTO, I8 or F64");
    RML_REQUIRE(path != RML_PATH_I8 || m->exact, RML_ERR_STATE, "rml_svm_kernel_matrix: exact path requested but the model is not on the code grid");
    RML_HIP(hipSetDevice(ctx->device));
    hipStream_t st = static_cast<hipStream_t>(stream);
    rml_ctx_guard guard(ctx, st);
    const int64_t CH = std::min<int64_t>(round_up(N, kTile), 8192);
    ChunkNeeds need{};
    need.q = m->exact && (path == RML_PATH_AUTO || path == RML_PATH_I8); need.f32 = true;
    ChunkWs w; ChunkPlan plan{};
    if (int rc = reserve_chunks(ctx, m, CH, need, st, &w, 1)) return rc;
    plan.policy = path; plan.kmat = kmat; plan.ld_k = ld_k;
    return run_float_rows(ctx, m, feat, ld_feat, N, CH, w, plan, DecisionOut{}, st);
}

namespace {
struct FrontCall {
    rml_ctx* ctx; const rml_svm* m; hipStream_t caller;
    const void* V; int vdtype; int64_t B; int X, Y, Z; int mode; const int32_t* ijk; bool derive; int32_t* ijk_out;
    float scale_div; uint32_t mask; DecisionOut out;
    bool grid_ok;
    int share_cu, q_rmw;
    bool occ;
    bool use_dig; ChunkPlan plan;
    bool u8() const { return vdtype == RML_VOL_U8; }
    int64_t frame_bytes() const { return (int64_t)X * Y * Z * (u8() ? 1 : 4); }
    int64_t plane_len(int pl) const { return pl == 0 ? (int64_t)X * Z : (pl == 1 ? (int64_t)Y * Z : (int64_t)X * Y); }
};

ProjOut code_rows_out(const FrontCall& f, const ChunkWs& w) {
    ProjOut o{}; int64_t off = 0;
    for (int pl = 0; pl < 3; ++pl)
        if (f.mask & (1u << pl)) { o.q[pl] = w.q + off; off += f.plane_len(pl); }
    o.sel = f.mask & RML_MASK_ALL;
    o.qstride = f.m->Dq; o.qrow = w.q; o.qD = f.m->D;
    o.row_isum = w.isum; o.row_isq = w.isq; o.row_flags = f.u8() ? nullptr : w.flags; o.scale_div = f.scale_div;
    o.share_cu = f.share_cu; o.q_rmw = f.q_rmw;
    if (f.occ && w.occ) { o.occ = w.occ; o.occ_words = f.m->occ_words; }
    return o;
}
ProjOut float_rows_out(const FrontCall& f, const ChunkWs& w) {
    ProjOut o{}; int64_t off = 0;
    for (int pl = 0; pl < 3; ++pl)
        if (f.mask & (1u << pl)) { o.p[pl] = w.f32 + off; o.stride[pl] = f.m->Df; off += f.plane_len(pl); }
    o.sel = f.mask & RML_MASK_ALL;
    o.scale_div = f.scale_div; o.prow = w.f32; o.pD = f.m->D; o.pstride = f.m->Df; o.row_nsq = w.nsq;
    o.share_cu = f.share_cu;
    return o;
}

int front_single_tile(const FrontCall& f) {
    rml_ctx* ctx = f.ctx; const rml_svm* m = f.m; hipStream_t st = f.caller;
    const int S = (f.vdtype == RML_VOL_F32 && f.mode == RML_MODE_MAX && f.B <= 64) ? rml_project_split_pieces(f.X, f.Y, f.Z) : 0;
    const size_t sbytes = S ? ((rml_project_split_scratch_bytes(f.B, f.X, f.Y, f.Z, S) + 255) & ~(size_t)255) : 0;
    ChunkNeeds need{};
    need.q = true; need.f32 = !f.u8();
    ChunkWs w; void* scratch = nullptr;
    int rc = reserve_chunks(ctx, m, kTile, need, st, &w, 1, sbytes, &scratch);
    if (rc) return rc;
    const ProjOut o = code_rows_out(f, w);
    rc = S ? rml_launch_project_split(ctx, f.V, f.vdtype, f.B, f.X, f.Y, f.Z, o, static_cast<float*>(scratch), S, st)
           : rml_launch_project(ctx, f.V, f.vdtype, f.B, f.X, f.Y, f.Z, f.mode, f.ijk, o, st);
    if (rc) return rc;
    const ChunkOps x = ws_rows(m, w, f.B);
    ChunkPlan plan{};
    plan.policy = f.u8() ? RML_PATH_I8 : RML_PATH_AUTO; plan.tiles_done = true; plan.all_exact_known = f.u8();
    if (f.u8()) return run_chunk(ctx, m, x, plan, w, f.out, st);
    launch_tile_flags(m, x, plan_chunk(ctx, m, plan, x, w), w, w.all_exact, st);
    ProjOut of = float_rows_out(f, w);
    of.skip_if_set = w.all_exact;
    rc = rml_launch_project(ctx, f.V, f.vdtype, f.B, f.X, f.Y, f.Z, f.mode, f.ijk, of, st);
    return rc ? rc : run_chunk(ctx, m, x, plan, w, f.out, st);
}

struct FrontChunk {
    int64_t r0, n; const ChunkWs& w; hipEvent_t ev_proj; const void* V; const int32_t* ijk; int32_t* ijkd;
};

int caller_stage(const FrontCall& f, const FrontChunk& ck, const ProjOut& po) {
    rml_prof_mark(f.ctx, f.caller);
    const int rc = f.derive ? rml_launch_derive_slice(f.ctx, ck.V, f.vdtype, ck.n, f.X, f.Y, f.Z, 1, ck.ijkd, nullptr, po, f.caller)
                            : rml_launch_project(f.ctx, ck.V, f.vdtype, ck.n, f.X, f.Y, f.Z, f.mode, ck.ijk, po, f.caller);
    rml_prof_mark(f.ctx, f.caller);
    if (f.ctx->profiling) f.ctx->prof_frames += ck.n;
    if (rc) return rc;
    if (f.use_dig) { launch_digit_rows(f.m, ck.w, ck.n, f.caller); RML_HIP(hipGetLastError()); }
    RML_HIP(hipEventRecord(ck.ev_proj, f.caller));
    RML_HIP(hipStreamWaitEvent(f.ctx->aux_stream, ck.ev_proj, 0));
    return RML_OK;
}
int gemm_stage(const FrontCall& f, const FrontChunk& ck) {
    hipStream_t aux = f.ctx->aux_stream;
    rml_prof_mark_gemm(f.ctx, aux);
    ChunkOps x = ws_rows(f.m, ck.w, ck.n);
    if (f.occ) x.occ = ck.w.occ;
    const int rc = run_chunk(f.ctx, f.m, x, f.plan, ck.w, f.out.at(ck.r0, f.m->C, f.m->P), aux);
    rml_prof_mark_gemm(f.ctx, aux);
    if (f.ctx->profiling) f.ctx->prof_ops_g += 2.0 * (double)ck.n * (double)f.m->M * (double)f.m->D;
    return rc;
}

int chunk_u8(const FrontCall& f, const FrontChunk& ck) {
    const int rc = caller_stage(f, ck, code_rows_out(f, ck.w));
    return rc ? rc : gemm_stage(f, ck);
}

int chunk_on_grid(const FrontCall& f, const FrontChunk& ck) {
    int rc = caller_stage(f, ck, code_rows_out(f, ck.w));
    if (rc) return rc;
    const ChunkOps x = ws_rows(f.m, ck.w, ck.n); hipStream_t aux = f.ctx->aux_stream;
    launch_tile_flags(f.m, x, plan_chunk(f.ctx, f.m, f.plan, x, ck.w), ck.w, ck.w.all_exact, aux);
    ProjOut of = float_rows_out(f, ck.w);
    of.no_pad = 1; of.skip_if_set = ck.w.all_exact;
    rc = rml_launch_project(f.ctx, ck.V, f.vdtype, ck.n, f.X, f.Y, f.Z, f.derive ? RML_MODE_SLICE : f.mode, f.derive ? ck.ijkd : ck.ijk, of, aux);
    return rc ? rc : gemm_stage(f, ck);
}

int chunk_off_grid(const FrontCall& f, const FrontChunk& ck) {
    ProjOut of = float_rows_out(f, ck.w);
    of.row_flags = ck.w.flags;
    const int rc = caller_stage(f, ck, of);
    return rc ? rc : gemm_stage(f, ck);
}

int front_chunked(FrontCall f) {
    rml_ctx* ctx = f.ctx; const rml_svm* m = f.m;
    const bool wave_proj = f.derive || rml_project_uses_wave_kernel(ctx, f.vdtype, f.mode, f.X, f.Y, f.Z, true, std::min<int64_t>(f.B, 8192));
    f.use_dig = !f.grid_ok && !f.u8() && use_dig_gemm(m, RML_PATH_AUTO, f.B, ctx->num_cu);
    f.share_cu = 1;
    f.q_rmw = ctx->opt.code_rmw >= 0 ? ctx->opt.code_rmw : rml_code_rmw(m->D, f.frame_bytes(), f.derive, f.u8());
    const bool u8_exact = f.grid_ok && f.u8();
    f.plan.policy = u8_exact ? RML_PATH_I8 : (f.grid_ok ? RML_PATH_AUTO : RML_PATH_F64);
    f.plan.tiles_done = f.grid_ok;
    f.plan.all_exact_known = u8_exact; f.plan.allow_big = !wave_proj; f.plan.dig_ready = f.use_dig;
    const int64_t small_chunk = (f.u8() && (int64_t)f.X * f.Y * f.Z <= 200000) ? 16384
                                : (f.derive && !f.u8() && f.frame_bytes() <= (1 << 20)) ? 12288 : 8192;
    const int64_t CH = (f.grid_ok && !wave_proj) ? pick_chunk(ctx, m, f.B, small_chunk, false)
                       : f.use_dig               ? pick_chunk(ctx, m, f.B, 8192, f.use_dig)
                                                 : std::min<int64_t>(round_up(f.B, kTile), f.grid_ok ? pick_chunk_opt(ctx, small_chunk) : 8192);
    ChunkNeeds need{};
    f.occ = f.grid_ok && !f.derive && f.mode != RML_MODE_SLICE && ctx->opt.sparse_rows != 0 &&
            (ctx->opt.sparse_rows > 0 || (wave_proj && !f.u8() && rml_sparse_rows(f.X, f.Y, f.Z)));
    need.q = f.grid_ok; need.f32 = true; need.dig = f.use_dig; need.ijk = f.derive && !f.ijk_out; need.occ = f.occ;
    constexpr int NBUF = 2;
    ChunkWs w2[NBUF];
    int rc = reserve_chunks(ctx, m, CH, need, f.caller, w2, NBUF);
    if (rc) return rc;
    RML_HIP(hipEventRecord(ctx->ev_fork, f.caller));
    RML_HIP(hipStreamWaitEvent(ctx->aux_stream, ctx->ev_fork, 0));
    int64_t c = 0;
    for (int64_t r0 = 0; r0 < f.B; r0 += CH, ++c) {
        const int b = (int)(c % NBUF);
        if (c >= NBUF) RML_HIP(hipStreamWaitEvent(f.caller, ctx->ev_done[b], 0));
        const FrontChunk ck{r0, std::min(CH, f.B - r0), w2[b], ctx->ev_proj[b], static_cast<const unsigned char*>(f.V) + r0 * f.frame_bytes(),
                            f.ijk ? f.ijk + r0 * 3 : nullptr, f.derive ? (f.ijk_out ? f.ijk_out + r0 * 3 : w2[b].ijk) : nullptr};
        rc = !f.grid_ok ? chunk_off_grid(f, ck) : (f.u8() ? chunk_u8(f, ck) : chunk_on_grid(f, ck));
        if (rc) return rc;
        RML_HIP(hipEventRecord(ctx->ev_done[b], ctx->aux_stream));
    }
    RML_HIP(hipEventRecord(ctx->ev_join, ctx->aux_stream));
    RML_HIP(hipStreamWaitEvent(f.caller, ctx->ev_join, 0));
    return RML_OK;
}

int project_svm_front(rml_ctx* ctx, const rml_svm* m, const void* V, int vdtype, int64_t B, int X, int Y, int Z,
                      int mode, const int32_t* ijk, bool derive, int32_t* ijk_out, float scale_div, uint32_t mask,
                      const DecisionOut& out, void* stream) {
    RML_REQUIRE(ctx && m && B >= 0, RML_ERR_INVALID, "rml_project_svm: bad arguments");
    if (B == 0) return RML_OK;
    RML_REQUIRE(V != nullptr, RML_ERR_INVALID, "rml_project_svm: V is NULL");
    RML_REQUIRE(vdtype == RML_VOL_F32 || vdtype == RML_VOL_U8, RML_ERR_INVALID, "rml_project_svm: unknown volume dtype %d", vdtype);
    RML_REQUIRE(rml_feature_len(X, Y, Z, mask) == m->D, RML_ERR_INVALID, "rml_project_svm: grid/mask give D=%lld, model has D=%lld",
                (long long)rml_feature_len(X, Y, Z, mask), (long long)m->D);
    RML_REQUIRE(!(out.proba || out.label_calib) || m->has_calib, RML_ERR_STATE, "rml_project_svm: model has no calibrators");
    RML_REQUIRE(mode != RML_MODE_SLICE || ijk || derive, RML_ERR_INVALID, "rml_project_svm: mode SLICE needs ijk");
    if (mode == RML_MODE_MAX_NAN) mode = RML_MODE_MAX;
    const bool scaled = scale_div > 1.0f;
    const bool grid_ok = m->exact && ((scaled && (double)scale_div == m->code_scale) || (!scaled && m->code_scale == 1.0));
    RML_HIP(hipSetDevice(ctx->device));
    hipStream_t caller = static_cast<hipStream_t>(stream);
    rml_ctx_guard guard(ctx, caller);
    const FrontCall f{ctx, m, caller, V, vdtype, B, X, Y, Z, mode, ijk, derive, ijk_out, scale_div, mask, out, grid_ok};
    if (B <= kTile && grid_ok && !derive && (mode == RML_MODE_MAX || (mode == RML_MODE_SLICE && ijk))) return front_single_tile(f);
    return front_chunked(f);
}
}

extern "C" int rml_project_svm(rml_ctx* ctx, const rml_svm* m, const void* V, int vdtype, int64_t B, int X, int Y, int Z,
                               int mode, const int32_t* ijk, float scale_div, uint32_t mask,
                               double* dec_ovo, double* dec_ovr, double* proba,
                               int32_t* label_vote, int32_t* label_calib, void* stream) {
    return project_svm_front(ctx, m, V, vdtype, B, X, Y, Z, mode, ijk, false, nullptr, scale_div, mask,
                             DecisionOut{dec_ovo, dec_ovr, proba, label_vote, label_calib}, stream);
}

extern "C" int rml_derive_project_svm(rml_ctx* ctx, const rml_svm* m, const void* V, int vdtype, int64_t B, int X, int Y, int Z,
                                      float scale_div, uint32_t mask, int32_t* ijk_out,
                                      double* dec_ovo, double* dec_ovr, double* proba,
                                      int32_t* label_vote, int32_t* label_calib, void* stream) {
    RML_REQUIRE(rml_derive_slice_supported(ctx, V, vdtype, X, Y, Z, 1) == 1, RML_ERR_UNSUPPORTED,
                "rml_derive_project_svm: no fused derive kernel for %dx%dx%d (rows of whole quads, Z <= 256, odd part of Z/4 <= 15): "
                "use rml_derive_targets + rml_project_svm(mode SLICE)", X, Y, Z);
    return project_svm_front(ctx, m, V, vdtype, B, X, Y, Z, RML_MODE_SLICE, nullptr, true, ijk_out, scale_div, mask,
                             DecisionOut{dec_ovo, dec_ovr, proba, label_vote, label_calib}, stream);
}

namespace {
int chunk_zoom(const FrontCall& f, const FrontChunk& ck, const rml_zoom_plan& zp, void* stage) {
    int rc = rml_zoom_stage_run(f.ctx, zp, stage, ck.V, ck.n, f.mode, ck.ijk, f.scale_div, ck.w.f32, f.m->Df, f.m->Df, ck.w.nsq, ck.w.flags,
                                f.caller);
    if (rc) return rc;
    if (f.use_dig) { launch_digit_rows(f.m, ck.w, ck.n, f.caller); RML_HIP(hipGetLastError()); }
    RML_HIP(hipEventRecord(ck.ev_proj, f.caller));
    RML_HIP(hipStreamWaitEvent(f.ctx->aux_stream, ck.ev_proj, 0));
    return gemm_stage(f, ck);
}

int front_zoom(FrontCall f, const rml_zoom_plan& zp) {
    rml_ctx* ctx = f.ctx; const rml_svm* m = f.m;
    f.use_dig = use_dig_gemm(m, RML_PATH_AUTO, f.B, ctx->num_cu);
    f.plan.policy = RML_PATH_F64; f.plan.dig_ready = f.use_dig;
    ChunkNeeds need{};
    need.f32 = true; need.dig = f.use_dig;
    if (f.B <= kTile) {
        ChunkWs w; void* stage = nullptr;
        int rc = reserve_chunks(ctx, m, kTile, need, f.caller, &w, 1, rml_zoom_stage_bytes(zp, f.B), &stage);
        if (rc) return rc;
        rc = rml_zoom_stage_run(ctx, zp, stage, f.V, f.B, f.mode, f.ijk, f.scale_div, w.f32, m->Df, m->Df, w.nsq, w.flags, f.caller);
        if (rc) return rc;
        if (f.use_dig) { launch_digit_rows(m, w, f.B, f.caller); RML_HIP(hipGetLastError()); }
        return run_chunk(ctx, m, ws_rows(m, w, f.B), f.plan, w, f.out, f.caller);
    }
    const int64_t CH = f.use_dig ? pick_chunk(ctx, m, f.B, 8192, true) : std::min<int64_t>(round_up(f.B, kTile), pick_chunk_opt(ctx, 8192));
    constexpr int NBUF = 2;
    ChunkWs w2[NBUF];
    const size_t sbytes = rml_zoom_stage_bytes(zp, CH);
    void* stages = nullptr;
    int rc = reserve_chunks(ctx, m, CH, need, f.caller, w2, NBUF, NBUF * sbytes, &stages);
    if (rc) return rc;
    RML_HIP(hipEventRecord(ctx->ev_fork, f.caller));
    RML_HIP(hipStreamWaitEvent(ctx->aux_stream, ctx->ev_fork, 0));
    int64_t c = 0;
    for (int64_t r0 = 0; r0 < f.B; r0 += CH, ++c) {
        const int b = (int)(c % NBUF);
        if (c >= NBUF) RML_HIP(hipStreamWaitEvent(f.caller, ctx->ev_done[b], 0));
        const FrontChunk ck{r0, std::min(CH, f.B - r0), w2[b], ctx->ev_proj[b], static_cast<const unsigned char*>(f.V) + r0 * f.frame_bytes(),
                            f.ijk ? f.ijk + r0 * 3 : nullptr, nullptr};
        rc = chunk_zoom(f, ck, zp, static_cast<unsigned char*>(stages) + (size_t)b * sbytes);
        if (rc) return rc;
        RML_HIP(hipEventRecord(ctx->ev_done[b], ctx->aux_stream));
    }
    RML_HIP(hipEventRecord(ctx->ev_join, ctx->aux_stream));
    RML_HIP(hipStreamWaitEvent(f.caller, ctx->ev_join, 0));
    return RML_OK;
}
}

extern "C" int rml_project_zoom_svm(rml_ctx* ctx, const rml_svm* m, const void* V, int vdtype, int64_t B, int X, int Y, int Z,
                                    int mode, const int32_t* ijk, const int32_t* out_shape, float scale_div, uint32_t mask,
                                    double* dec_ovo, double* dec_ovr, double* proba,
                                    int32_t* label_vote, int32_t* label_calib, void* stream) {
    RML_REQUIRE(ctx && m && B >= 0, RML_ERR_INVALID, "rml_project_zoom_svm: bad arguments");
    if (mode == RML_MODE_MAX_NAN) mode = RML_MODE_MAX;
    RML_REQUIRE(mode == RML_MODE_MAX || mode == RML_MODE_SLICE || mode == RML_MODE_SUM, RML_ERR_INVALID, "rml_project_zoom_svm: unknown mode %d", mode);
    rml_zoom_plan zp;
    if (int rc = rml_zoom_plan_make(ctx, "rml_project_zoom_svm", vdtype, mode, X, Y, Z, 1, mode == RML_MODE_SLICE && !ijk, out_shape, mask, &zp)) return rc;
    RML_REQUIRE(zp.Dout == m->D, RML_ERR_INVALID, "rml_project_zoom_svm: the zoomed planes give D=%lld, model has D=%lld",
                (long long)zp.Dout, (long long)m->D);
    if (B == 0) return RML_OK;
    RML_REQUIRE(V != nullptr, RML_ERR_INVALID, "rml_project_zoom_svm: V is NULL");
    RML_REQUIRE(B < (int64_t)1 << 31, RML_ERR_UNSUPPORTED, "rml_project_zoom_svm: B too large");
    RML_REQUIRE(!(proba || label_calib) || m->has_calib, RML_ERR_STATE, "rml_project_zoom_svm: model has no calibrators");
    RML_HIP(hipSetDevice(ctx->device));
    hipStream_t caller = static_cast<hipStream_t>(stream);
    rml_ctx_guard guard(ctx, caller);
    const FrontCall f{ctx, m, caller, V, vdtype, B, X, Y, Z, mode, ijk, false, nullptr, scale_div, mask,
                      DecisionOut{dec_ovo, dec_ovr, proba, label_vote, label_calib}, false};
    return front_zoom(f, zp);
}

extern "C" int rml_svm_set_platt(rml_ctx* ctx, rml_svm* m, const double* probA, const double* probB) {
    RML_REQUIRE(ctx && m && probA && probB, RML_ERR_INVALID, "rml_svm_set_platt: NULL argument");
    RML_HIP(hipSetDevice(ctx->device));
    std::vector<double> ab(2 * kMaxP, 0.0);
    for (int p = 0; p < m->P; ++p) { ab[p] = probA[p]; ab[kMaxP + p] = probB[p]; }
    if (!m->platt) RML_HIP(hipMalloc(reinterpret_cast<void**>(&m->platt), ab.size() * sizeof(double)));
    RML_HIP(hipMemcpy(m->platt, ab.data(), ab.size() * sizeof(double), hipMemcpyHostToDevice));
    return RML_OK;
}

extern "C" int rml_svm_pairwise_proba(rml_ctx* ctx, const rml_svm* m, const double* dec_ovo, int64_t N, double* proba, void* stream) {
    RML_REQUIRE(ctx && m && N >= 0, RML_ERR_INVALID, "rml_svm_pairwise_proba: bad arguments");
    if (N == 0) return RML_OK;
    RML_REQUIRE(dec_ovo && proba, RML_ERR_INVALID, "rml_svm_pairwise_proba: NULL array");
    RML_REQUIRE(m->platt != nullptr, RML_ERR_STATE, "rml_svm_pairwise_proba: the model has no Platt coefficients (rml_svm_set_platt)");
    RML_HIP(hipSetDevice(ctx->device));
    hipStream_t st = static_cast<hipStream_t>(stream);
    hipLaunchKernelGGL(k_pairwise_proba, dim3((unsigned)((N + 255) / 256)), dim3(256), 0, st, dec_ovo, N, m->C, m->platt, m->platt + kMaxP, proba);
    RML_HIP(hipGetLastError());
    return RML_OK;
}

extern "C" int rml_linear_load(rml_ctx* ctx, const double* coef, const double* intercept, int n_classes, int64_t D,
                               const double* calib_a, const double* calib_b, rml_linear** out) {
    RML_REQUIRE(ctx && coef && intercept && out && D > 0, RML_ERR_INVALID, "rml_linear_load: bad arguments");
    RML_REQUIRE(n_classes >= 2 && n_classes <= kMaxC, RML_ERR_UNSUPPORTED, "rml_linear_load: %d classes", n_classes);
    RML_REQUIRE((calib_a == nullptr) == (calib_b == nullptr), RML_ERR_INVALID, "rml_linear_load: calib_a/calib_b must both be given");
    *out = nullptr;
// ... 45 lines not shown
```

Measured before the change: 2.987 million frames/s.

## Skip storing all-background code lines when sparse occupancy GEMM is planned

After: 3.081 million frames/s, median of 6. 3.2% higher.

```diff
diff --git a/include/radarml.h b/include/radarml.h
--- a/include/radarml.h
+++ b/include/radarml.h
@@ -68,6 +68,7 @@
 #define RML_CONV7_DEFAULT 3
 #define RML_OPT_ZOOM_ROWS 14
 #define RML_OPT_SPARSE_ROWS 15
+#define RML_OPT_SPARSE_STORES 16
 int rml_ctx_set_option(rml_ctx* ctx, int option, int value);
 int rml_ctx_get_option(const rml_ctx* ctx, int option, int* value);
 
@@ -86,7 +87,11 @@
 int rml_project_occupancy(rml_ctx* ctx, const void* V, int vdtype, int64_t B, int X, int Y, int Z, int mode, float scale_div,
                           uint32_t mask, uint8_t* feat_q, int64_t ld_q, int32_t* row_isum, int64_t* row_isq, int32_t* row_flags,
                           uint32_t* occ, int occ_words, void* stream);
+int rml_project_sparse_rows(rml_ctx* ctx, const void* V, int vdtype, int64_t B, int X, int Y, int Z, int mode, float scale_div,
+                            uint32_t mask, uint8_t* feat_q, int64_t ld_q, int32_t* row_isum, int64_t* row_isq, int32_t* row_flags,
+                            uint32_t* occ, int occ_words, int skip_clear, void* stream);
 int64_t rml_ctx_sparse_gemm_launches(const rml_ctx* ctx);
+int64_t rml_ctx_sparse_store_launches(const rml_ctx* ctx);
 
 int64_t rml_feature_len(int X, int Y, int Z, uint32_t mask);
 
diff --git a/radar-ml_amd/_lib.py b/radar-ml_amd/_lib.py
--- a/radar-ml_amd/_lib.py
+++ b/radar-ml_amd/_lib.py
@@ -182,23 +182,26 @@
                                   c_void_p, c_void_p]),
     "rml_code_rmw_default": (c_int, [c_int64, c_int64, c_int, c_int]),
     "rml_ctx_sparse_gemm_launches": (c_int64, [c_void_p]),
+    "rml_ctx_sparse_store_launches": (c_int64, [c_void_p]),
     "rml_svm_sv_occupancy": (c_int, [c_void_p, c_void_p, c_void_p, c_int64]),
     "rml_project_occupancy": (c_int, [c_void_p, c_void_p, c_int, c_int64, c_int, c_int, c_int, c_int, c_float, c_uint32, c_void_p, c_int64,
                                       c_void_p, c_void_p, c_void_p, c_void_p, c_int, c_void_p]),
+    "rml_project_sparse_rows": (c_int, [c_void_p, c_void_p, c_int, c_int64, c_int, c_int, c_int, c_int, c_float, c_uint32, c_void_p, c_int64,
+                                        c_void_p, c_void_p, c_void_p, c_void_p, c_int, c_int, c_void_p]),
     "rml_probe_stream": (c_int, [c_void_p, c_void_p, c_int64, c_int, c_void_p, c_void_p]),
     "rml_synth_volumes": (c_int, [c_void_p, c_uint64, c_int64, c_int64, c_int, c_int, c_int, c_int, c_void_p, c_void_p,
                                   c_void_p]),
 }
 
 MODE_MAX, MODE_SLICE, MODE_SUM, MODE_MAX_NAN = 0, 1, 2, 3
-OPT_PROJECT_SHARE_CU, OPT_WAVEFRAME, OPT_LINPLANE, OPT_STAGE_CODES, OPT_SLICE_WAVE, OPT_DERIVE_FUSED, OPT_CODE_RMW, OPT_GEMM_BIG, OPT_CHUNK, OPT_C1_PK, OPT_SMO_LDS_ROWS, OPT_SGD_RESIDENT_D, OPT_CONV7, OPT_ZOOM_ROWS, OPT_SPARSE_ROWS = range(1, 16)
+OPT_PROJECT_SHARE_CU, OPT_WAVEFRAME, OPT_LINPLANE, OPT_STAGE_CODES, OPT_SLICE_WAVE, OPT_DERIVE_FUSED, OPT_CODE_RMW, OPT_GEMM_BIG, OPT_CHUNK, OPT_C1_PK, OPT_SMO_LDS_ROWS, OPT_SGD_RESIDENT_D, OPT_CONV7, OPT_ZOOM_ROWS, OPT_SPARSE_ROWS, OPT_SPARSE_STORES = range(1, 17)
 OPTIONS = {"project_share_cu": OPT_PROJECT_SHARE_CU, "waveframe": OPT_WAVEFRAME, "linplane": OPT_LINPLANE, "stage_codes": OPT_STAGE_CODES,
            "slice_wave": OPT_SLICE_WAVE, "derive_fused": OPT_DERIVE_FUSED, "code_rmw": OPT_CODE_RMW, "gemm_big": OPT_GEMM_BIG,
            "chunk": OPT_CHUNK, "c1_pk": OPT_C1_PK}
 SOLVER_OPTIONS = {"smo_lds_rows": OPT_SMO_LDS_ROWS, "sgd_resident_d": OPT_SGD_RESIDENT_D}
 NN_OPTIONS = {"conv7": OPT_CONV7}
 ZOOM_OPTIONS = {"zoom_rows": OPT_ZOOM_ROWS}
-SVM_OPTIONS = {"sparse_rows": OPT_SPARSE_ROWS}
+SVM_OPTIONS = {"sparse_rows": OPT_SPARSE_ROWS, "sparse_stores": OPT_SPARSE_STORES}
 SMO_LDS_ROWS_MAX = 2768
 SGD_RESIDENT_D_MAX = 10240
 SGD_MAX_ROWS = 8192
@@ -208,7 +211,7 @@
 ENV_OPTIONS = {"RML_WAVE_SHARE": "project_share_cu", "RML_WAVEFRAME": "waveframe", "RML_LINPLANE": "linplane", "RML_STAGE_CODES": "stage_codes",
                "RML_SLICE_WAVE": "slice_wave", "RML_DERIVE_FUSED": "derive_fused", "RML_CODE_RMW": "code_rmw", "RML_GEMM_BIG": "gemm_big",
                "RML_CHUNK": "chunk", "RML_C1_PK": "c1_pk", "RML_SMO_LDS_ROWS": "smo_lds_rows", "RML_SGD_RESIDENT_D": "sgd_resident_d",
-               "RML_CONV7": "conv7", "RML_SPARSE_ROWS": "sparse_rows"}
+               "RML_CONV7": "conv7", "RML_SPARSE_ROWS": "sparse_rows", "RML_SPARSE_STORES": "sparse_stores"}
 AUG_ROTATE, AUG_ZOOM, AUG_NOISE = 0, 1, 2
 CHAIN_ROTATE, CHAIN_ZOOM, CHAIN_NOISE = 1, 2, 4
 VOL_F32, VOL_U8 = 0, 1
diff --git a/radar-ml_amd/csrc/context.hip b/radar-ml_amd/csrc/context.hip
--- a/radar-ml_amd/csrc/context.hip
+++ b/radar-ml_amd/csrc/context.hip
@@ -290,6 +290,7 @@
         case RML_OPT_GEMM_BIG: return &o.gemm_big;
         case RML_OPT_C1_PK: return &o.c1_pk;
         case RML_OPT_SPARSE_ROWS: return &o.sparse_rows;
+        case RML_OPT_SPARSE_STORES: return &o.sparse_stores;
         default: return nullptr;
     }
 }
@@ -328,7 +329,7 @@
     RML_REQUIRE(slot != nullptr, RML_ERR_INVALID, "rml_ctx_set_option: unknown option %d", option);
     switch (option) {
         case RML_OPT_WAVEFRAME: RML_REQUIRE(value >= 0 && value <= 3, RML_ERR_INVALID, "rml_ctx_set_option: RML_OPT_WAVEFRAME is 0..3"); *slot = value; break;
-        case RML_OPT_CODE_RMW: case RML_OPT_GEMM_BIG: case RML_OPT_SPARSE_ROWS: *slot = value < 0 ? -1 : (value ? 1 : 0); break;
+        case RML_OPT_CODE_RMW: case RML_OPT_GEMM_BIG: case RML_OPT_SPARSE_ROWS: case RML_OPT_SPARSE_STORES: *slot = value < 0 ? -1 : (value ? 1 : 0); break;
         default: *slot = value ? 1 : 0;
     }
     return RML_OK;
diff --git a/radar-ml_amd/csrc/project.hip b/radar-ml_amd/csrc/project.hip
--- a/radar-ml_amd/csrc/project.hip
+++ b/radar-ml_amd/csrc/project.hip
@@ -301,9 +301,10 @@
         int lane_f = lane, Y_f = Y;
         asm volatile("" : "+v"(lane_f), "+s"(Y_f));
         const bool act_f = lane_f < ZQ;
+        const bool holes_f = em.line32_ok(1, 4 * ZQ);
         static_for<NY>([&](auto jc) {
             constexpr int j = decltype(jc)::value;
-            if (j < Y_f && act_f) em.put4(1, (int64_t)j * Z + 4 * lane_f, yz[j]);
+            if (j < Y_f && act_f) em.put4_line32(1, (int64_t)j * Z + 4 * lane_f, yz[j], lane_f, holes_f);
         });
         em.flush_wave(lane_f);
         em.finish_wave(lane_f);
@@ -626,6 +627,7 @@
     const int num_cu = !ctx ? 256 : ctx->num_cu;
     const int rc = vdtype == RML_VOL_U8 ? launch_project_t<uint8_t>(pp, mode, num_cu, st) : launch_project_t<float>(pp, mode, num_cu, st);
     if (rc) return rc;
+    if (ctx && o.skip_clear && occ_done) ++ctx->sparse_store_launches;
     if (o.occ && !occ_done) {
         const int64_t n = B * o.occ_words;
         hipLaunchKernelGGL(k_fill_u32, dim3((unsigned)((n + 255) / 256)), dim3(256), 0, st, o.occ, n, 0xFFFFFFFFu);
@@ -868,9 +870,9 @@
     return rml_launch_project(ctx, V, vdtype, B, X, Y, Z, mode, ijk, o, static_cast<hipStream_t>(stream), tpf);
 }
 
-extern "C" int rml_project_occupancy(rml_ctx* ctx, const void* V, int vdtype, int64_t B, int X, int Y, int Z, int mode, float scale_div,
-                                     uint32_t mask, uint8_t* feat_q, int64_t ld_q, int32_t* row_isum, int64_t* row_isq, int32_t* row_flags,
-                                     uint32_t* occ, int occ_words, void* stream) {
+static int project_occupancy(rml_ctx* ctx, const void* V, int vdtype, int64_t B, int X, int Y, int Z, int mode, float scale_div,
+                             uint32_t mask, uint8_t* feat_q, int64_t ld_q, int32_t* row_isum, int64_t* row_isq, int32_t* row_flags,
+                             uint32_t* occ, int occ_words, int skip_clear, void* stream) {
     RML_REQUIRE(ctx && B >= 0 && X > 0 && Y > 0 && Z > 0, RML_ERR_INVALID, "rml_project_occupancy: bad arguments");
     if (B == 0) return RML_OK;
     RML_REQUIRE(V && feat_q && occ, RML_ERR_INVALID, "rml_project_occupancy: NULL argument");
@@ -884,8 +886,19 @@
     RML_HIP(hipSetDevice(ctx->device));
     ProjOut o{};
     rows_out(o, X, Y, Z, mask, scale_div, nullptr, 0, feat_q, ld_q, row_isum, row_isq, row_flags);
-    o.occ = occ; o.occ_words = occ_words;
+    o.occ = occ; o.occ_words = occ_words; o.skip_clear = skip_clear ? 1 : 0;
     return rml_launch_project(ctx, V, vdtype, B, X, Y, Z, mode, nullptr, o, static_cast<hipStream_t>(stream));
+}
+extern "C" int rml_project_occupancy(rml_ctx* ctx, const void* V, int vdtype, int64_t B, int X, int Y, int Z, int mode, float scale_div,
+                                     uint32_t mask, uint8_t* feat_q, int64_t ld_q, int32_t* row_isum, int64_t* row_isq, int32_t* row_flags,
+                                     uint32_t* occ, int occ_words, void* stream) {
+    return project_occupancy(ctx, V, vdtype, B, X, Y, Z, mode, scale_div, mask, feat_q, ld_q, row_isum, row_isq, row_flags, occ, occ_words, 0, stream);
+}
+extern "C" int rml_project_sparse_rows(rml_ctx* ctx, const void* V, int vdtype, int64_t B, int X, int Y, int Z, int mode, float scale_div,
+                                       uint32_t mask, uint8_t* feat_q, int64_t ld_q, int32_t* row_isum, int64_t* row_isq, int32_t* row_flags,
+                                       uint32_t* occ, int occ_words, int skip_clear, void* stream) {
+    return project_occupancy(ctx, V, vdtype, B, X, Y, Z, mode, scale_div, mask, feat_q, ld_q, row_isum, row_isq, row_flags, occ, occ_words,
+                             skip_clear, stream);
 }
 
 extern "C" int rml_project_planes(rml_ctx* ctx, const void* V, int vdtype, int64_t B, int X, int Y, int Z, int mode,
diff --git a/radar-ml_amd/csrc/project_shared.h b/radar-ml_amd/csrc/project_shared.h
--- a/radar-ml_amd/csrc/project_shared.h
+++ b/radar-ml_amd/csrc/project_shared.h
@@ -82,10 +82,12 @@
     int stage_xy = 0;
     int occ_on = 0;
     int occ_off = 0;
+    int skip = 0;
     __device__ __forceinline__ void set_stage(unsigned char* p, int xy_off) {
         stage = (lds_u8*)p; staged = 1; stage_xy = xy_off;
         if (a.o.occ) {
             occ_on = 1; occ_off = xy_off + ((a.X * a.Y + 15) & ~15);
+            skip = a.o.skip_clear;
             for (int w = threadIdx.x & 63; w < a.o.occ_words; w += 64) *(lds_u32*)(stage + occ_off + 4 * w) = 0u;
         }
     }
@@ -182,6 +184,21 @@
             }
         }
     }
+    __device__ __forceinline__ void put4_line32(int pl, int64_t idx, float4 v, int lane, bool holes) {
+        if (!holes) { put4(pl, idx, v); return; }
+        if (!((a.o.sel >> pl) & 1u)) return;
+        uint32_t c0 = code(v.x), c1 = code(v.y), c2 = code(v.z), c3 = code(v.w);
+        if (a.o.q[pl]) {
+            const uint32_t packed = c0 | (c1 << 8) | (c2 << 16) | (c3 << 24);
+            const bool nz = packed != 0x80808080u;
+            const uint64_t line = __ballot(nz) >> (lane & 32);
+            if ((uint32_t)line) *reinterpret_cast<uint32_t*>(a.o.q[pl] + qb() * a.o.qstride + idx) = packed;
+            if (nz) occ_mark(plane_at(pl) + (int)idx);
+        }
+    }
+    __device__ __forceinline__ bool line32_ok(int pl, int bytes) const {
+        return skip && a.o.q[pl] && bytes == 256 && (plane_at(pl) & 127) == 0;
+    }
     __device__ __forceinline__ void reset(int64_t b_) { b = b_; isum = 0; isq = 0; ok = 1; nsq = 0.0; }
     __device__ void flush_wave(int lane) {
         if (!staged) return;
@@ -194,10 +211,21 @@
         for (int r = 0; r < 2; ++r) {
             int done = 0;
             if ((reinterpret_cast<uintptr_t>(dst[r]) & 15) == 0) {
-                for (int i = lane; i < (len[r] >> 4); i += 64) {
-                    const u32x4 v = ((lds_u128*)src[r])[i];
-                    reinterpret_cast<u32x4*>(dst[r])[i] = v;
-                    if (occ_on && ((v.x ^ 0x80808080u) | (v.y ^ 0x80808080u) | (v.z ^ 0x80808080u) | (v.w ^ 0x80808080u))) occ_mark(at[r] + 16 * i);
+                if (skip && (at[r] & 127) == 0) {
+                    const int whole = len[r] & ~127;
+                    for (int i = lane; i < (len[r] >> 4); i += 64) {
+                        const u32x4 v = ((lds_u128*)src[r])[i];
+                        const bool nz = ((v.x ^ 0x80808080u) | (v.y ^ 0x80808080u) | (v.z ^ 0x80808080u) | (v.w ^ 0x80808080u)) != 0u;
+                        const uint32_t line = (uint32_t)(__ballot(nz) >> (lane & 56)) & 0xFFu;
+                        if (line || 16 * i >= whole) reinterpret_cast<u32x4*>(dst[r])[i] = v;
+                        if (nz) occ_mark(at[r] + 16 * i);
+                    }
+                } else {
+                    for (int i = lane; i < (len[r] >> 4); i += 64) {
+                        const u32x4 v = ((lds_u128*)src[r])[i];
+                        reinterpret_cast<u32x4*>(dst[r])[i] = v;
+                        if (occ_on && ((v.x ^ 0x80808080u) | (v.y ^ 0x80808080u) | (v.z ^ 0x80808080u) | (v.w ^ 0x80808080u))) occ_mark(at[r] + 16 * i);
+                    }
                 }
                 done = len[r] & ~15;
             }
diff --git a/radar-ml_amd/csrc/rml_internal.h b/radar-ml_amd/csrc/rml_internal.h
--- a/radar-ml_amd/csrc/rml_internal.h
+++ b/radar-ml_amd/csrc/rml_internal.h
@@ -35,6 +35,7 @@
     int conv7 = RML_CONV7_DEFAULT;
     int sgd_resident_d = RML_SGD_RESIDENT_D_MAX;
     int sparse_rows = -1;
+    int sparse_stores = -1;
     int zoom_rows = 0;
 };
 
@@ -53,6 +54,7 @@
     hipEvent_t ev_fork = nullptr, ev_join = nullptr;
     hipEvent_t ev_proj[2] = {nullptr, nullptr}, ev_done[2] = {nullptr, nullptr};
     hipStream_t aux_stream = nullptr;
+    int64_t sparse_store_launches = 0;
     mutable int64_t sparse_gemm_launches = 0;
     uint8_t* bg_line = nullptr;
     bool profiling = false;
@@ -151,6 +153,7 @@
     int q_rmw;
     uint32_t* occ;
     int occ_words;
+    int skip_clear;
 };
 inline int rml_code_rmw(int64_t D, int64_t frame_bytes, bool derive, bool u8) {
     if (derive) return 0;
@@ -159,6 +162,10 @@
 
 inline int rml_sparse_rows(int X, int Y, int Z) {
     return (Z % 128 == 0 || 128 % Z == 0) && ((int64_t)X * Z) % 128 == 0 && ((int64_t)Y * Z) % 128 == 0;
+}
+
+inline int rml_sparse_stores(int X, int Y, int Z) {
+    return rml_sparse_rows(X, Y, Z);
 }
 
 bool rml_project_uses_wave_kernel(const rml_ctx* ctx, int vdtype, int mode, int X, int Y, int Z, bool share_cu, int64_t B);
diff --git a/radar-ml_amd/csrc/svm.hip b/radar-ml_amd/csrc/svm.hip
--- a/radar-ml_amd/csrc/svm.hip
+++ b/radar-ml_amd/csrc/svm.hip
@@ -133,8 +133,8 @@
 };
 
 struct ChunkOps { int64_t n; const uint8_t* q; int64_t ld_q; const int32_t* isum; const int64_t* isq; const int32_t* flags; const float* f32; const double* nsq;
-                  const uint32_t* occ; };
-ChunkOps ws_rows(const rml_svm* m, const ChunkWs& w, int64_t n) { return ChunkOps{n, w.q, m->Dq, w.isum, w.isq, w.flags, w.f32, w.nsq, nullptr}; }
+                  const uint32_t* occ; bool holes; };
+ChunkOps ws_rows(const rml_svm* m, const ChunkWs& w, int64_t n) { return ChunkOps{n, w.q, m->Dq, w.isum, w.isq, w.flags, w.f32, w.nsq, nullptr, false}; }
 
 struct ChunkPlan {
     int policy;
@@ -244,6 +244,7 @@
               hipStream_t st) {
     const ChunkPlan p = plan_chunk(ctx, m, asked, x, w);
     RML_REQUIRE(p.run_i8 || p.run_gen, RML_ERR_STATE, "svm: no usable operand path (model exact=%d)", (int)m->exact);
+    RML_REQUIRE(!(x.holes && !p.sparse), RML_ERR_STATE, "svm: code rows with unstored background lines reached a dense plan");
     if (!p.tiles_done) {
         launch_tile_flags(m, x, p, w, nullptr, st);
         if (p.run_dig) launch_tile_dig(x, p, w, st);
@@ -456,6 +457,7 @@
     return RML_OK;
 }
 extern "C" int64_t rml_ctx_sparse_gemm_launches(const rml_ctx* ctx) { return ctx ? ctx->sparse_gemm_launches : 0; }
+extern "C" int64_t rml_ctx_sparse_store_launches(const rml_ctx* ctx) { return ctx ? ctx->sparse_store_launches : 0; }
 extern "C" int rml_svm_is_exact(const rml_svm* m) { return m && m->exact ? 1 : 0; }
 extern "C" int64_t rml_svm_num_sv(const rml_svm* m) { return m ? m->M : 0; }
 extern "C" int64_t rml_svm_dim(const rml_svm* m) { return m ? m->D : 0; }
@@ -553,13 +555,14 @@
     bool grid_ok;
     int share_cu, q_rmw;
     bool occ;
+    bool skip_ok;
     bool use_dig; ChunkPlan plan;
     bool u8() const { return vdtype == RML_VOL_U8; }
     int64_t frame_bytes() const { return (int64_t)X * Y * Z * (u8() ? 1 : 4); }
     int64_t plane_len(int pl) const { return pl == 0 ? (int64_t)X * Z : (pl == 1 ? (int64_t)Y * Z : (int64_t)X * Y); }
 };
 
-ProjOut code_rows_out(const FrontCall& f, const ChunkWs& w) {
+ProjOut code_rows_out(const FrontCall& f, const ChunkWs& w, bool holes = false) {
     ProjOut o{}; int64_t off = 0;
     for (int pl = 0; pl < 3; ++pl)
         if (f.mask & (1u << pl)) { o.q[pl] = w.q + off; off += f.plane_len(pl); }
@@ -567,7 +570,7 @@
     o.qstride = f.m->Dq; o.qrow = w.q; o.qD = f.m->D;
     o.row_isum = w.isum; o.row_isq = w.isq; o.row_flags = f.u8() ? nullptr : w.flags; o.scale_div = f.scale_div;
     o.share_cu = f.share_cu; o.q_rmw = f.q_rmw;
-    if (f.occ && w.occ) { o.occ = w.occ; o.occ_words = f.m->occ_words; }
+    if (f.occ && w.occ) { o.occ = w.occ; o.occ_words = f.m->occ_words; o.skip_clear = holes ? 1 : 0; }
     return o;
 }
 ProjOut float_rows_out(const FrontCall& f, const ChunkWs& w) {
@@ -606,7 +609,14 @@
 
 struct FrontChunk {
     int64_t r0, n; const ChunkWs& w; hipEvent_t ev_proj; const void* V; const int32_t* ijk; int32_t* ijkd;
+    bool holes;
 };
+ChunkOps chunk_ops(const FrontCall& f, const FrontChunk& ck) {
+    ChunkOps x = ws_rows(f.m, ck.w, ck.n);
+    if (f.occ) x.occ = ck.w.occ;
+    x.holes = ck.holes;
+    return x;
+}
 
 int caller_stage(const FrontCall& f, const FrontChunk& ck, const ProjOut& po) {
     rml_prof_mark(f.ctx, f.caller);
@@ -623,8 +633,7 @@
 int gemm_stage(const FrontCall& f, const FrontChunk& ck) {
     hipStream_t aux = f.ctx->aux_stream;
     rml_prof_mark_gemm(f.ctx, aux);
-    ChunkOps x = ws_rows(f.m, ck.w, ck.n);
-    if (f.occ) x.occ = ck.w.occ;
+    const ChunkOps x = chunk_ops(f, ck);
     const int rc = run_chunk(f.ctx, f.m, x, f.plan, ck.w, f.out.at(ck.r0, f.m->C, f.m->P), aux);
     rml_prof_mark_gemm(f.ctx, aux);
     if (f.ctx->profiling) f.ctx->prof_ops_g += 2.0 * (double)ck.n * (double)f.m->M * (double)f.m->D;
@@ -632,14 +641,14 @@
 }
 
 int chunk_u8(const FrontCall& f, const FrontChunk& ck) {
-    const int rc = caller_stage(f, ck, code_rows_out(f, ck.w));
+    const int rc = caller_stage(f, ck, code_rows_out(f, ck.w, ck.holes));
     return rc ? rc : gemm_stage(f, ck);
 }
 
 int chunk_on_grid(const FrontCall& f, const FrontChunk& ck) {
-    int rc = caller_stage(f, ck, code_rows_out(f, ck.w));
+    int rc = caller_stage(f, ck, code_rows_out(f, ck.w, ck.holes));
     if (rc) return rc;
-    const ChunkOps x = ws_rows(f.m, ck.w, ck.n); hipStream_t aux = f.ctx->aux_stream;
+    const ChunkOps x = chunk_ops(f, ck); hipStream_t aux = f.ctx->aux_stream;
     launch_tile_flags(f.m, x, plan_chunk(f.ctx, f.m, f.plan, x, ck.w), ck.w, ck.w.all_exact, aux);
     ProjOut of = float_rows_out(f, ck.w);
     of.no_pad = 1; of.skip_if_set = ck.w.all_exact;
@@ -672,6 +681,8 @@
     ChunkNeeds need{};
     f.occ = f.grid_ok && !f.derive && f.mode != RML_MODE_SLICE && ctx->opt.sparse_rows != 0 &&
             (ctx->opt.sparse_rows > 0 || (wave_proj && !f.u8() && rml_sparse_rows(f.X, f.Y, f.Z)));
+    f.skip_ok = f.occ && wave_proj && !f.u8() && ctx->opt.sparse_stores != 0 &&
+                (ctx->opt.sparse_stores > 0 || rml_sparse_stores(f.X, f.Y, f.Z));
     need.q = f.grid_ok; need.f32 = true; need.dig = f.use_dig; need.ijk = f.derive && !f.ijk_out; need.occ = f.occ;
     constexpr int NBUF = 2;
     ChunkWs w2[NBUF];
@@ -683,8 +694,9 @@
     for (int64_t r0 = 0; r0 < f.B; r0 += CH, ++c) {
         const int b = (int)(c % NBUF);
         if (c >= NBUF) RML_HIP(hipStreamWaitEvent(f.caller, ctx->ev_done[b], 0));
-        const FrontChunk ck{r0, std::min(CH, f.B - r0), w2[b], ctx->ev_proj[b], static_cast<const unsigned char*>(f.V) + r0 * f.frame_bytes(),
-                            f.ijk ? f.ijk + r0 * 3 : nullptr, f.derive ? (f.ijk_out ? f.ijk_out + r0 * 3 : w2[b].ijk) : nullptr};
+        FrontChunk ck{r0, std::min(CH, f.B - r0), w2[b], ctx->ev_proj[b], static_cast<const unsigned char*>(f.V) + r0 * f.frame_bytes(),
+                      f.ijk ? f.ijk + r0 * 3 : nullptr, f.derive ? (f.ijk_out ? f.ijk_out + r0 * 3 : w2[b].ijk) : nullptr, false};
+        ck.holes = f.skip_ok && plan_chunk(ctx, m, f.plan, chunk_ops(f, ck), ck.w).sparse;
         rc = !f.grid_ok ? chunk_off_grid(f, ck) : (f.u8() ? chunk_u8(f, ck) : chunk_on_grid(f, ck));
         if (rc) return rc;
         RML_HIP(hipEventRecord(ctx->ev_done[b], ctx->aux_stream));
```
